# AI4Science-WestlakeU/wdno

Hardware: AMD Instinct MI355X
Metric: diffusion train steps/sec, 2D smoke U-Net (8 samples per GPU per step) (higher is better)
Workload: dtype f32

## Files before the change

### include/wdno_hip.h

```cpp
#ifndef WDNO_HIP_H
#define WDNO_HIP_H
#include <stdint.h>
#include <stddef.h>

#ifdef __cplusplus
extern "C" {
#endif

typedef void* wdno_stream_t;

enum { WDNO_OK = 0, WDNO_EINVAL = -1, WDNO_ELAUNCH = -2, WDNO_EUNSUPPORTED = -3, WDNO_EWORKSPACE = -4 };

#define WDNO_AMAX_SLOTS 64
#define WDNO_AMAX_STRIDE 16
#define WDNO_AMAX_FLOATS (WDNO_AMAX_SLOTS * WDNO_AMAX_STRIDE)
const char* wdno_strerror(int code);
int wdno_version(void);
const char* wdno_last_hip_error(void);
int wdno_set_debug(int mode);

typedef struct {
  int nd;
  int mode;
  int L;
  int n_img;
  int in_dims[3];
  int out_dims[3];
  int64_t cs_img, cs_band, cs0, cs1;
} wdno_dwt_desc;
size_t wdno_dwt_ws_bytes(const wdno_dwt_desc* d);
int wdno_dwt_fwd(const float* x, float* coef, const wdno_dwt_desc* d, const float* filters_host, void* ws, size_t ws_bytes, wdno_stream_t s);
int wdno_dwt_inv(const float* coef, float* x, const wdno_dwt_desc* d, const float* filters_host, void* ws, size_t ws_bytes, wdno_stream_t s);
int wdno_dwt_fwd_adjoint(const float* dcoef, float* dx, const wdno_dwt_desc* d, const float* filters_host, void* ws, size_t ws_bytes, wdno_stream_t s);
int wdno_dwt_inv_adjoint(const float* dx, float* dcoef, const wdno_dwt_desc* d, const float* filters_host, void* ws, size_t ws_bytes, wdno_stream_t s);
int wdno_dwt_fwd_packed(const float* x, float* state, const wdno_dwt_desc* d, const float* filters_host, int img_inner, int64_t cs_outer, int row_w,
                        const float* rescaler, wdno_stream_t s);
int wdno_upsample_coef(const float* in, float* out, int64_t outer, int a, int mid, int b, int c, int fa, int fb, int fc, wdno_stream_t s);
int wdno_pack_smoke_state(const float* coef, int64_t coef_sim_stride, const float* init_coef, int64_t init_sim_stride, const float* smokeout,
                          int64_t so_sim_stride, const int64_t* idx, const float* rescaler, float* state, int64_t B, int F, int nt, int nx,
                          int pad_t, int pad_x, wdno_stream_t s);
int wdno_pack_smoke_fields(const float* coef, int64_t coef_sim_stride, const float* rho0, int64_t rho0_sim_stride, const float* curve,
                           int64_t curve_sim_stride, const float* dec_lo_host, const float* dec_hi_host, int L, const float* rescaler,
                           float* state, int64_t B, int F, int nt, int nx, int pad_t, int pad_x, int H0, int W0, int T0, wdno_stream_t s);

int wdno_nc_to_cl(const float* src, float* dst, int64_t N, int C, int64_t S, int Cp, wdno_stream_t s);
int wdno_cl_to_nc(const float* src, float* dst, int64_t N, int C, int64_t S, int Cp, wdno_stream_t s);
int wdno_concat2_cl_planes(const float* a, int Ca, const float* b, int Cb, const float* rec_a, const float* rec_b, void* hi, void* lo,
                           float* scale_out, int64_t P, wdno_stream_t s);
int wdno_concat2_cl(const float* a, int Ca, const float* b, int Cb, float* out, int64_t P, wdno_stream_t s);
int wdno_concat2_cl_amax(const float* a, int Ca, const float* b, int Cb, float* out, float* amax_rec, int64_t P, wdno_stream_t s);
int wdno_split2_cl(const float* in, float* a, int Ca, float* b, int Cb, int64_t P, wdno_stream_t s);
int wdno_upsample2x_cl_fwd(const float* in, float* out, int64_t N, int H, int W, int C, wdno_stream_t s);
int wdno_upsample2x_cl_bwd(const float* dout, float* din, int64_t N, int H, int W, int C, wdno_stream_t s);

typedef struct {
  int N, D, H, W, C;
  int OD, OH, OW, K;
  int kd, kh, kw;
  int sd, sh, sw;
  int pd, ph, pw;
  int YD, YH, YW;
  int osd, osh, osw, ood, ooh, oow;
} wdno_conv_geom;
int wdno_conv_fwd(const float* x, const float* wp, const float* bias, const float* residual, float* y,
                  const wdno_conv_geom* g, wdno_stream_t s);
int wdno_amax(const float* x, int64_t n, float* amax_zeroed, wdno_stream_t s);
int wdno_amax_record(const float* x, int64_t n, float* rec_zeroed, wdno_stream_t s);
int wdno_split_f16(const float* x, const float* amax_rec, void* hi, void* lo, float* scale_out, int64_t rows, int C, int C8, wdno_stream_t s);
size_t wdno_split_colsum_ws_bytes(int64_t rows, int C8);
int wdno_split_f16_colsum(const float* x, const float* amax_rec, void* hi, void* lo, float* scale_out, float* colsum_out,
                          void* ws, size_t ws_bytes, int64_t rows, int C, int C8, wdno_stream_t s);
int wdno_pack_split_weight(const float* w, const float* amax, void* hi, void* lo, float* scale_out, int K, int C, int kd, int kh, int kw,
                           int A, int B, int mode, wdno_stream_t s);
typedef struct { const void* x; int64_t n; void* out; } wdno_amax_item;
typedef struct {
  const void* w; const void* amax; void* hi; void* lo; void* scale_out;
  int K, C, kd, kh, kw, A, B, mode;
} wdno_wsplit_item;
int wdno_amax_multi(const void* table, int n_items, int blocks_per_item, wdno_stream_t s);
int wdno_pack_split_weight_multi(const void* table, int n_items, int blocks_per_item, wdno_stream_t s);
int wdno_conv_fwd_f16x3(const void* xh, const void* xl, const float* sx, const void* wph, const void* wpl, const float* sw,
                        const float* bias, const float* residual, float* y, const wdno_conv_geom* g, wdno_stream_t s);
int wdno_conv_fwd_f16x3_amax(const void* xh, const void* xl, const float* sx, const void* wph, const void* wpl, const float* sw,
                             const float* bias, const float* residual, float* y, float* amax_rec, const wdno_conv_geom* g,
                             wdno_stream_t s);
typedef struct { int channels, d0, h0, w0; } wdno_zero_box;
int wdno_conv_fwd_f16x3_zbox(const void* xh, const void* xl, const float* sx, const void* wph, const void* wpl, const float* sw,
                             const float* bias, const float* residual, float* y, float* amax_rec, const wdno_conv_geom* g,
                             const wdno_zero_box* zb, wdno_stream_t s);
int wdno_conv_fwd_bf16_ex(const void* x16, const void* wp16, const float* bias, const float* residual, void* y, int y_bf16, float* amax_rec,
                          const wdno_conv_geom* g, const wdno_zero_box* zb, wdno_stream_t s);
int wdno_conv_fwd_f16x3_ws(const void* xh, const void* xl, const float* sx, const void* wph, const void* wpl, const float* sw,
                           const float* bias, const float* residual, float* y, float* amax_rec, const wdno_conv_geom* g,
                           void* ws, size_t ws_bytes, wdno_stream_t s);
size_t wdno_conv_fwd_split_ws_bytes(const wdno_conv_geom* g);
size_t wdno_conv_wgrad_f16x3_ws_bytes(const wdno_conv_geom* g);
int wdno_conv_pixel_table(void* table, const wdno_conv_geom* g, wdno_stream_t s);
int wdno_conv_wgrad_f16x3(const void* xh, const void* xl, const float* sx, const void* dyh, const void* dyl, const float* sdy,
                          const void* pixel_table, float* dwp, void* ws, size_t ws_bytes, const wdno_conv_geom* g, wdno_stream_t s);
int wdno_conv_wgrad_f16x3_param(const void* xh, const void* xl, const float* sx, const void* dyh, const void* dyl, const float* sdy,
                                const void* pixel_table, float* dw, int Kn, int Cn, void* ws, size_t ws_bytes,
                                const wdno_conv_geom* g, wdno_stream_t s);
#define WDNO_WGRAD_REDUCE_MAX 40
typedef struct wdno_wgrad_reduce_item {
  const float* ws; float* dw;
  int n, splits;
  int K8, C8, kw, ntap, Kn, Cn;
  int tiled;
  int reserved;
} wdno_wgrad_reduce_item;
int wdno_conv_wgrad_partials(const void* xh, const void* xl, const float* sx, const void* dyh, const void* dyl, const float* sdy,
                             const void* pixel_table, float* dw, int Kn, int Cn, void* ws, size_t ws_bytes,
                             const wdno_conv_geom* g, wdno_wgrad_reduce_item* item, wdno_stream_t s);
int wdno_wgrad_reduce_multi(const wdno_wgrad_reduce_item* items, int n_items, wdno_stream_t s);
size_t wdno_conv_wgrad_ws_bytes(const wdno_conv_geom* g);
int wdno_conv_wgrad(const float* x, const float* dy, float* dwp, void* ws, size_t ws_bytes,
                    const wdno_conv_geom* g, wdno_stream_t s);
#define WDNO_ROWS_SUM_MAX 64
typedef struct wdno_rows_sum_item {
  const void* part; float* out;
  int rows, stride, col0, ncols;
  int is_double, reserved;
} wdno_rows_sum_item;
int wdno_rows_sum_multi(const wdno_rows_sum_item* items, int n_items, wdno_stream_t s);
size_t wdno_colsum_ws_bytes(int64_t P, int C);
int wdno_colsum(const float* in, float* out, int64_t P, int C, void* ws, size_t ws_bytes, wdno_stream_t s);

int wdno_cast_bf16(const float* x, void* out16, int64_t rows, int C, int C8, wdno_stream_t s);
int wdno_cast_bf16_colsum(const float* x, void* out16, float* colsum_out, void* ws, size_t ws_bytes, int64_t rows, int C, int C8, wdno_stream_t s);
int wdno_conv_fwd_bf16(const void* x16, const void* wp16, const float* bias, const float* residual, float* y, float* amax_rec,
                       const wdno_conv_geom* g, wdno_stream_t s);
int wdno_conv_wgrad_bf16_param(const void* x16, const void* dy16, const void* pixel_table, float* dw, int Kn, int Cn, void* ws,
                               size_t ws_bytes, const wdno_conv_geom* g, wdno_stream_t s);

size_t wdno_groupnorm_ws_bytes(int64_t N, int64_t S, int C, int G);
size_t wdno_groupnorm_stats_floats(int64_t N, int C, int G);
int wdno_groupnorm_act_fwd(const float* x, const float* gamma, const float* beta, const float* ss, float* y,
                           float* stats, int64_t N, int64_t S, int C, int G, float eps, int silu,
                           void* ws, size_t ws_bytes, wdno_stream_t s);
int wdno_groupnorm_act_fwd_amax(const float* x, const float* gamma, const float* beta, const float* ss, float* y,
                                float* stats, float* amax_rec, int64_t N, int64_t S, int C, int G, float eps, int silu,
                                void* ws, size_t ws_bytes, wdno_stream_t s);
int wdno_groupnorm_act_bwd(const float* x, const float* dy, const float* gamma, const float* beta, const float* ss,
                           const float* stats, float* dx, float* dgb_partial, float* dss,
                           int64_t N, int64_t S, int C, int G, int silu, void* ws, size_t ws_bytes, wdno_stream_t s);
int wdno_groupnorm_act_bwd_amax(const float* x, const float* dy, const float* gamma, const float* beta, const float* ss,
                                const float* stats, float* dx, float* dgb_partial, float* dss, float* amax_rec,
                                int64_t N, int64_t S, int C, int G, int silu, void* ws, size_t ws_bytes, wdno_stream_t s);
size_t wdno_groupnorm_bwd_planes_ws_bytes(int64_t N, int64_t S, int C, int G);
size_t wdno_groupnorm_fwd_planes_ws_bytes(int64_t N, int64_t S, int C, int G);
int wdno_groupnorm_act_fwd_planes(const float* x, const float* gamma, const float* beta, const float* ss, void* y_hi, void* y_lo,
                                  float* y_scale, float* stats, float* bound_rec, int64_t N, int64_t S, int C, int G, float eps, int silu,
                                  void* ws, size_t ws_bytes, wdno_stream_t s);
int wdno_groupnorm_act_add_fwd_planes(const float* x, const float* gamma, const float* beta, const float* ss, const float* residual,
                                      const float* res_rec, float* y, void* y_hi, void* y_lo, float* y_scale, float* stats,
                                      float* bound_rec, float* y_amax_rec, int64_t N, int64_t S, int C, int G, float eps, int silu,
                                      void* ws, size_t ws_bytes, wdno_stream_t s);
int wdno_groupnorm_act_bwd_planes(const float* x, const float* dy, const float* gamma, const float* beta, const float* ss,
                                  const float* stats, void* dx_hi, void* dx_lo, float* dx_scale, float* dx_colsum,
                                  float* dgb_partial, float* dgb_sum, float* dss, float* bound_rec, int64_t N, int64_t S, int C, int G, int silu,
                                  void* ws, size_t ws_bytes, wdno_stream_t s);
int wdno_groupnorm_bwd_planes_tail(int64_t N, int64_t S, int C, int G, size_t* csp_offset, int* rows);
int wdno_groupnorm_act_fwd_amax_t(const void* x, int x_bf16, const float* gamma, const float* beta, const float* ss, float* y,
                                  float* stats, float* amax_rec, int64_t N, int64_t S, int C, int G, float eps, int silu,
                                  void* ws, size_t ws_bytes, wdno_stream_t s);
int wdno_groupnorm_act_fwd_planes_t(const void* x, int x_bf16, const float* gamma, const float* beta, const float* ss, void* y_hi, void* y_lo,
                                    float* y_scale, float* stats, float* bound_rec, int64_t N, int64_t S, int C, int G, float eps,
                                    int silu, void* ws, size_t ws_bytes, wdno_stream_t s);
int wdno_groupnorm_act_add_fwd_planes_t(const void* x, int x_bf16, const float* gamma, const float* beta, const float* ss, const float* residual,
                                        const float* res_rec, float* y, void* y_hi, void* y_lo, float* y_scale, float* stats,
                                        float* bound_rec, float* y_amax_rec, int64_t N, int64_t S, int C, int G, float eps, int silu,
                                        void* ws, size_t ws_bytes, wdno_stream_t s);
int wdno_groupnorm_act_bwd_planes_t(const void* x, int x_bf16, const void* dy, int dy_bf16, const float* gamma, const float* beta, const float* ss,
                                    const float* stats, void* dx_hi, void* dx_lo, float* dx_scale, float* dx_colsum,
                                    float* dgb_partial, float* dgb_sum, float* dss, float* bound_rec, int64_t N, int64_t S, int C, int G, int silu,
                                    void* ws, size_t ws_bytes, wdno_stream_t s);
int wdno_layernorm_fwd(const float* x, const float* g, float* y, int64_t P, int C, float eps, wdno_stream_t s);
int wdno_layernorm_fwd_amax(const float* x, const float* g, float* y, float* amax_rec, int64_t P, int C, float eps, wdno_stream_t s);
int wdno_layernorm_fwd_planes(const float* x, const float* g, void* y_hi, void* y_lo, float* y_scale, int64_t P, int C, float eps,
                              wdno_stream_t s);
size_t wdno_layernorm_bwd_ws_bytes(int64_t P, int C);
int wdno_layernorm_bwd(const float* x, const float* g, const float* dy, float* dx, float* dg, int64_t P, int C,
                       float eps, void* ws, size_t ws_bytes, wdno_stream_t s);
int wdno_layernorm_bwd_add(const float* x, const float* g, const float* dy, const float* add_to, float* dx, float* dg, int64_t P, int C,
                           float eps, void* ws, size_t ws_bytes, wdno_stream_t s);
int wdno_layernorm_bwd_add_amax(const float* x, const float* g, const float* dy, const float* add_to, float* dx, float* dg, float* amax_rec,
                                int64_t P, int C, float eps, void* ws, size_t ws_bytes, wdno_stream_t s);

typedef struct {
  int n_uo, n_ui, n_tok, heads;
  int64_t so, si, st;
} wdno_attn_desc;
int wdno_attn_fwd(const float* qkv, const float* rot_cos, const float* rot_sin, const float* bias, float* out,
                  const wdno_attn_desc* d, float scale, wdno_stream_t s);
size_t wdno_attn_bwd_ws_bytes(const wdno_attn_desc* d);
int wdno_attn_bwd(const float* qkv, const float* rot_cos, const float* rot_sin, const float* bias, const float* out,
                  const float* dout, float* dqkv, float* dbias, const wdno_attn_desc* d, float scale, void* ws, size_t ws_bytes,
                  wdno_stream_t s);
int wdno_attn_fwd_amax(const float* qkv, const float* rot_cos, const float* rot_sin, const float* bias, float* out, float* amax_rec,
                       const wdno_attn_desc* d, float scale, wdno_stream_t s);
int wdno_attn_bwd_amax(const float* qkv, const float* rot_cos, const float* rot_sin, const float* bias, const float* out,
                       const float* dout, float* dqkv, float* dbias, float* amax_rec, const wdno_attn_desc* d, float scale,
                       void* ws, size_t ws_bytes, wdno_stream_t s);
int wdno_attn_bwd_planes(const float* qkv, const float* rot_cos, const float* rot_sin, const float* bias, const float* out,
                         const float* dout, void* dqkv_hi, void* dqkv_lo, float* dqkv_scale, float* dbias,
                         const float* rec_qkv, const float* rec_dout, const wdno_attn_desc* d, float scale, void* ws, size_t ws_bytes,
                         wdno_stream_t s);
int wdno_attn_fwd_planes(const float* qkv, const float* rot_cos, const float* rot_sin, const float* bias, float* out, void* out_hi,
                         void* out_lo, float* out_scale, float* amax_rec, const float* rec_qkv, const wdno_attn_desc* d, float scale,
                         wdno_stream_t s);
size_t wdno_linattn_ws_bytes(int64_t units, int heads);
int wdno_linattn_fwd(const float* qkv, float* out, float* kstats , float* ctx ,
                     int64_t units, int n_tok, int heads, float scale, wdno_stream_t s);
int wdno_linattn_bwd(const float* qkv, const float* dout, const float* kstats, const float* ctx, float* dqkv,
                     void* ws, size_t ws_bytes, int64_t units, int n_tok, int heads, float scale, wdno_stream_t s);
int wdno_linattn_fwd_amax(const float* qkv, float* out, float* kstats, float* ctx, float* amax_rec, int64_t units, int n_tok, int heads,
                          float scale, wdno_stream_t s);
int wdno_linattn_bwd_amax(const float* qkv, const float* dout, const float* kstats, const float* ctx, float* dqkv, float* amax_rec,
                          void* ws, size_t ws_bytes, int64_t units, int n_tok, int heads, float scale, wdno_stream_t s);
int wdno_linattn_bwd_planes(const float* qkv, const float* dout, const float* kstats, const float* ctx, void* dqkv_hi, void* dqkv_lo,
                            float* dqkv_scale, const float* rec_qkv, const float* rec_dout, float* rec_dctx, void* ws, size_t ws_bytes,
                            int64_t units, int n_tok, int heads, float scale, wdno_stream_t s);
int wdno_linattn_fwd_planes(const float* qkv, void* out_hi, void* out_lo, float* out_scale, float* kstats, float* ctx,
                            const float* rec_qkv, int64_t units, int n_tok, int heads, float scale, wdno_stream_t s);

int wdno_tattn_fused_takes(int C, int n_tok, int heads);
int wdno_tattn_fused_fwd(const float* x, const float* gamma, float eps, const void* wq_hi, const void* wq_lo, const float* wq_scale,
                         const void* wo_hi, const void* wo_lo, const float* wo_scale, const float* rot_cos, const float* rot_sin,
                         const float* bias, float* y, float* amax_rec, float* qkv_out, float* rec_v,
                         int64_t n_batch, int n_tok, int64_t hw, int C, int heads, float scale, wdno_stream_t s);
size_t wdno_tattn_fused_bwd_ws_bytes(void);
int wdno_tattn_fused_bwd_grads(void);
int wdno_tattn_fused_bwd(const float* x, const float* dy, const float* gamma, float eps, const void* wq_hi, const void* wq_lo,
                         const float* wq_scale, const void* wo_hi, const void* wo_lo, const float* wo_scale, const float* rot_cos,
                         const float* rot_sin, const float* bias, const float* rec_dy, const float* rec_v, float* dx, float* amax_rec,
                         float* grads, void* ws, size_t ws_bytes,
                         int64_t n_batch, int n_tok, int64_t hw, int C, int heads, float scale, wdno_stream_t s);

int wdno_lattn_fused_takes(int C, int heads, int n_tok);
size_t wdno_lattn_fused_ws_bytes(int64_t units, int n_tok);
int wdno_lattn_fused_fwd(const float* x, const float* gamma, float eps, const void* wq_hi, const void* wq_lo, const float* wq_scale,
                         const void* wo_hi, const void* wo_lo, const float* wo_scale, const float* bias_out, float* y, float* amax_rec,
                         float* ctx_out, float* kstat_out, void* ws, size_t ws_bytes, int64_t units, int n_tok, int C, int heads, float scale,
                         wdno_stream_t s);

int wdno_lattn_fused_bwd_grads(void);
size_t wdno_lattn_fused_bwd_ws_bytes(int64_t units, int n_tok);
int wdno_lattn_fused_bwd(const float* x, const float* dy, const float* gamma, float eps, const void* wq_hi, const void* wq_lo,
                         const float* wq_scale, const void* wot_hi, const void* wot_lo, const float* wot_scale, const float* ctx,
                         const float* kstat, const float* rec_dy, float* dx, float* amax_rec, float* grads, void* ws, size_t ws_bytes,
                         int64_t units, int n_tok, int C, int heads, float scale, wdno_stream_t s);

int wdno_relpos_bias_fwd(const float* w, const int64_t* bucket, float* out, int n, int heads, wdno_stream_t s);
int wdno_relpos_bias_bwd(const float* dbias, const int64_t* bucket, float* dw, int n, int heads, int num_buckets, wdno_stream_t s);

int wdno_linear_rows_fwd(const float* x, int x_stride, const float* w, int w_stride, const float* bias, float* y, int P, int C, int K,
                         int Kp, wdno_stream_t s);
int wdno_linear_rows_wgrad(const float* x, int x_stride, const float* dy, int dy_stride, float* dw, float* db, int P, int C, int K,
                           wdno_stream_t s);

typedef struct wdno_linear_item {
  const void* w;
  const void* bias;
  int K, k_start;
} wdno_linear_item;
int wdno_linear_multi_fwd(const void* table, int n_items, int F, const float* x, float* y, int P, int C, wdno_stream_t s);
int wdno_linear_multi_wgrad(const void* table, int n_items, int F, const float* x, const float* dy, float* dw, float* db, int P, int C,
                            wdno_stream_t s);
size_t wdno_linear_multi_dgrad_ws_bytes(int F, int P, int C);
int wdno_linear_multi_dgrad(const void* table, int n_items, int F, const float* dy, float* dx, int P, int C, void* ws, size_t ws_bytes,
                            wdno_stream_t s);

int wdno_act_fwd(const float* x, float* y, int64_t n, int act, wdno_stream_t s);
int wdno_act_bwd(const float* x, const float* dy, float* dx, int64_t n, int act, wdno_stream_t s);
int wdno_add(const float* a, const float* b, float* out, int64_t n, wdno_stream_t s);
int wdno_add_amax(const float* a, const float* b, float* out, float* amax_rec, int64_t n, wdno_stream_t s);
int wdno_sinusoidal_emb(const int64_t* t, const float* freqs, float* out, int B, int dim, wdno_stream_t s);

typedef struct {
  int tree;
  int B, F, C, H, W;
  int cT, cH, cW;
  int cond_pad, cond_a, cond_b, cond_c, cond_low;
  int u_rows, uT_rows;
} wdno_cond_desc;
int wdno_q_sample_cond(const float* x0, const float* noise, const int64_t* t, const float* sqrt_ac, const float* sqrt_1mac,
// ... 39 lines not shown
```

### wdno_amd/_lib.py

```python
import contextlib
import ctypes as C
import os

import torch

HERE = os.path.dirname(os.path.abspath(__file__))
LIB_PATH = os.path.join(HERE, 'libwdno_hip.so')

P = C.c_void_p
I = C.c_int
L = C.c_int64
F = C.c_float
Z = C.c_size_t


class DwtDesc(C.Structure):
    _fields_ = [('nd', I), ('mode', I), ('L', I), ('n_img', I), ('in_dims', I * 3), ('out_dims', I * 3),
                ('cs_img', L), ('cs_band', L), ('cs0', L), ('cs1', L)]


class ConvGeom(C.Structure):
    _fields_ = [(k, I) for k in ('N', 'D', 'H', 'W', 'C', 'OD', 'OH', 'OW', 'K', 'kd', 'kh', 'kw', 'sd', 'sh', 'sw',
                                 'pd', 'ph', 'pw', 'YD', 'YH', 'YW', 'osd', 'osh', 'osw', 'ood', 'ooh', 'oow')]


class AttnDesc(C.Structure):
    _fields_ = [('n_uo', I), ('n_ui', I), ('n_tok', I), ('heads', I), ('so', L), ('si', L), ('st', L)]


class CondDesc(C.Structure):
    _fields_ = [(k, I) for k in ('tree', 'B', 'F', 'C', 'H', 'W', 'cT', 'cH', 'cW', 'cond_pad', 'cond_a', 'cond_b',
                                 'cond_c', 'cond_low', 'u_rows', 'uT_rows')]


class WgradReduceItem(C.Structure):
    _fields_ = [('ws', C.c_void_p), ('dw', C.c_void_p), ('n', I), ('splits', I), ('K8', I), ('C8', I), ('kw', I), ('ntap', I), ('Kn', I), ('Cn', I),
                ('tiled', I), ('reserved', I)]


class RowsSumItem(C.Structure):
    _fields_ = [('part', C.c_void_p), ('out', C.c_void_p), ('rows', I), ('stride', I), ('col0', I), ('ncols', I), ('is_double', I), ('reserved', I)]


class BurgersDesc(C.Structure):
    _fields_ = [(k, I) for k in ('N', 's', 'nx0', 'nt_f', 'nxf', 'steps', 'record_time', 'f_time', 'num_t', 'sub_s', 'out_cols', 'waves',
                                 'points')] + [(k, F) for k in ('c', 'd', 'dm', 'dt')]


PD, PG, PA, PC = C.POINTER(DwtDesc), C.POINTER(ConvGeom), C.POINTER(AttnDesc), C.POINTER(CondDesc)
PF = C.POINTER(C.c_float)

PROTOTYPES = {
    'wdno_strerror': (C.c_char_p, [I]),
    'wdno_version': (I, []),
    'wdno_last_hip_error': (C.c_char_p, []),
    'wdno_set_debug': (I, [I]),
    'wdno_dwt_ws_bytes': (Z, [PD]),
    'wdno_dwt_fwd': (I, [P, P, PD, PF, P, Z, P]),
    'wdno_dwt_fwd_packed': (I, [P, P, PD, PF, I, L, I, P, P]),
    'wdno_dwt_inv': (I, [P, P, PD, PF, P, Z, P]),
    'wdno_dwt_fwd_adjoint': (I, [P, P, PD, PF, P, Z, P]),
    'wdno_dwt_inv_adjoint': (I, [P, P, PD, PF, P, Z, P]),
    'wdno_upsample_coef': (I, [P, P, L, I, I, I, I, I, I, I, P]),
    'wdno_pack_smoke_state': (I, [P, L, P, L, P, L, P, P, P, L, I, I, I, I, I, P]),
    'wdno_pack_smoke_fields': (I, [P, L, P, L, P, L, PF, PF, I, P, P, L, I, I, I, I, I, I, I, I, P]),
    'wdno_nc_to_cl': (I, [P, P, L, I, L, I, P]),
    'wdno_cl_to_nc': (I, [P, P, L, I, L, I, P]),
    'wdno_concat2_cl': (I, [P, I, P, I, P, L, P]),
    'wdno_concat2_cl_planes': (I, [P, I, P, I, P, P, P, P, P, L, P]),
    'wdno_concat2_cl_amax': (I, [P, I, P, I, P, P, L, P]),
    'wdno_split2_cl': (I, [P, P, I, P, I, L, P]),
    'wdno_upsample2x_cl_fwd': (I, [P, P, L, I, I, I, P]),
    'wdno_upsample2x_cl_bwd': (I, [P, P, L, I, I, I, P]),
    'wdno_conv_fwd': (I, [P, P, P, P, P, PG, P]),
    'wdno_amax': (I, [P, L, P, P]),
    'wdno_amax_record': (I, [P, L, P, P]),
    'wdno_split_f16': (I, [P, P, P, P, P, L, I, I, P]),
    'wdno_split_colsum_ws_bytes': (Z, [L, I]),
    'wdno_split_f16_colsum': (I, [P, P, P, P, P, P, P, Z, L, I, I, P]),
    'wdno_pack_split_weight': (I, [P, P, P, P, P, I, I, I, I, I, I, I, I, P]),
    'wdno_amax_multi': (I, [P, I, I, P]),
    'wdno_pack_split_weight_multi': (I, [P, I, I, P]),
    'wdno_conv_fwd_f16x3': (I, [P, P, P, P, P, P, P, P, P, PG, P]),
    'wdno_conv_fwd_f16x3_amax': (I, [P, P, P, P, P, P, P, P, P, P, PG, P]),
    'wdno_conv_fwd_f16x3_ws': (I, [P, P, P, P, P, P, P, P, P, P, PG, P, Z, P]),
    'wdno_conv_fwd_split_ws_bytes': (Z, [PG]),
    'wdno_conv_wgrad_f16x3_ws_bytes': (Z, [PG]),
    'wdno_conv_pixel_table': (I, [P, PG, P]),
    'wdno_conv_wgrad_f16x3': (I, [P, P, P, P, P, P, P, P, P, Z, PG, P]),
    'wdno_conv_wgrad_f16x3_param': (I, [P, P, P, P, P, P, P, P, I, I, P, Z, PG, P]),
    'wdno_conv_wgrad_partials': (I, [P, P, P, P, P, P, P, P, I, I, P, Z, PG, P, P]),
    'wdno_wgrad_reduce_multi': (I, [P, I, P]),
    'wdno_rows_sum_multi': (I, [P, I, P]),
    'wdno_cast_bf16': (I, [P, P, L, I, I, P]),
    'wdno_cast_bf16_colsum': (I, [P, P, P, P, Z, L, I, I, P]),
    'wdno_conv_fwd_bf16': (I, [P, P, P, P, P, P, PG, P]),
    'wdno_conv_fwd_f16x3_zbox': (I, [P, P, P, P, P, P, P, P, P, P, PG, P, P]),
    'wdno_conv_fwd_bf16_ex': (I, [P, P, P, P, P, I, P, PG, P, P]),
    'wdno_conv_wgrad_bf16_param': (I, [P, P, P, P, I, I, P, Z, PG, P]),
    'wdno_conv_wgrad_ws_bytes': (Z, [PG]),
    'wdno_conv_wgrad': (I, [P, P, P, P, Z, PG, P]),
    'wdno_colsum_ws_bytes': (Z, [L, I]),
    'wdno_colsum': (I, [P, P, L, I, P, Z, P]),
    'wdno_groupnorm_ws_bytes': (Z, [L, L, I, I]),
    'wdno_groupnorm_stats_floats': (Z, [L, I, I]),
    'wdno_groupnorm_act_fwd': (I, [P, P, P, P, P, P, L, L, I, I, F, I, P, Z, P]),
    'wdno_groupnorm_act_fwd_amax': (I, [P, P, P, P, P, P, P, L, L, I, I, F, I, P, Z, P]),
    'wdno_groupnorm_act_bwd': (I, [P, P, P, P, P, P, P, P, P, L, L, I, I, I, P, Z, P]),
    'wdno_groupnorm_act_bwd_amax': (I, [P, P, P, P, P, P, P, P, P, P, L, L, I, I, I, P, Z, P]),
    'wdno_groupnorm_bwd_planes_ws_bytes': (Z, [L, L, I, I]),
    'wdno_groupnorm_bwd_planes_tail': (I, [L, L, I, I, C.POINTER(Z), C.POINTER(I)]),
    'wdno_groupnorm_fwd_planes_ws_bytes': (Z, [L, L, I, I]),
    'wdno_groupnorm_act_fwd_planes': (I, [P, P, P, P, P, P, P, P, P, L, L, I, I, F, I, P, Z, P]),
    'wdno_groupnorm_act_add_fwd_planes': (I, [P, P, P, P, P, P, P, P, P, P, P, P, P, L, L, I, I, F, I, P, Z, P]),
    'wdno_layernorm_fwd_planes': (I, [P, P, P, P, P, L, I, F, P]),
    'wdno_groupnorm_act_bwd_planes': (I, [P, P, P, P, P, P, P, P, P, P, P, P, P, P, L, L, I, I, I, P, Z, P]),
    'wdno_groupnorm_act_fwd_amax_t': (I, [P, I, P, P, P, P, P, P, L, L, I, I, F, I, P, Z, P]),
    'wdno_groupnorm_act_fwd_planes_t': (I, [P, I, P, P, P, P, P, P, P, P, L, L, I, I, F, I, P, Z, P]),
    'wdno_groupnorm_act_add_fwd_planes_t': (I, [P, I, P, P, P, P, P, P, P, P, P, P, P, P, L, L, I, I, F, I, P, Z, P]),
    'wdno_groupnorm_act_bwd_planes_t': (I, [P, I, P, I, P, P, P, P, P, P, P, P, P, P, P, P, L, L, I, I, I, P, Z, P]),
    'wdno_layernorm_fwd': (I, [P, P, P, L, I, F, P]),
    'wdno_layernorm_fwd_amax': (I, [P, P, P, P, L, I, F, P]),
    'wdno_layernorm_bwd_ws_bytes': (Z, [L, I]),
    'wdno_layernorm_bwd': (I, [P, P, P, P, P, L, I, F, P, Z, P]),
    'wdno_layernorm_bwd_add': (I, [P, P, P, P, P, P, L, I, F, P, Z, P]),
    'wdno_layernorm_bwd_add_amax': (I, [P, P, P, P, P, P, P, L, I, F, P, Z, P]),
    'wdno_attn_fwd': (I, [P, P, P, P, P, PA, F, P]),
    'wdno_attn_bwd_ws_bytes': (Z, [PA]),
    'wdno_attn_bwd': (I, [P, P, P, P, P, P, P, P, PA, F, P, Z, P]),
    'wdno_attn_fwd_amax': (I, [P, P, P, P, P, P, PA, F, P]),
    'wdno_attn_bwd_amax': (I, [P, P, P, P, P, P, P, P, P, PA, F, P, Z, P]),
    'wdno_attn_fwd_planes': (I, [P, P, P, P, P, P, P, P, P, P, PA, F, P]),
    'wdno_linattn_fwd_planes': (I, [P, P, P, P, P, P, P, L, I, I, F, P]),
    'wdno_attn_bwd_planes': (I, [P, P, P, P, P, P, P, P, P, P, P, P, PA, F, P, Z, P]),
    'wdno_tattn_fused_takes': (I, [I, I, I]),
    'wdno_tattn_fused_fwd': (I, [P, P, F, P, P, P, P, P, P, P, P, P, P, P, P, P, L, I, L, I, I, F, P]),
    'wdno_lattn_fused_takes': (I, [I, I, I]),
    'wdno_lattn_fused_ws_bytes': (Z, [L, I]),
    'wdno_lattn_fused_fwd': (I, [P, P, F, P, P, P, P, P, P, P, P, P, P, P, P, Z, L, I, I, I, F, P]),
    'wdno_lattn_fused_bwd_grads': (I, []),
    'wdno_lattn_fused_bwd_ws_bytes': (Z, [L, I]),
    'wdno_lattn_fused_bwd': (I, [P, P, P, F, P, P, P, P, P, P, P, P, P, P, P, P, P, Z, L, I, I, I, F, P]),
    'wdno_tattn_fused_bwd_ws_bytes': (Z, []),
    'wdno_tattn_fused_bwd_grads': (I, []),
    'wdno_tattn_fused_bwd': (I, [P, P, P, F, P, P, P, P, P, P, P, P, P, P, P, P, P, P, P, Z, L, I, L, I, I, F, P]),
    'wdno_linattn_ws_bytes': (Z, [L, I]),
    'wdno_linattn_fwd': (I, [P, P, P, P, L, I, I, F, P]),
    'wdno_linattn_bwd': (I, [P, P, P, P, P, P, Z, L, I, I, F, P]),
    'wdno_linattn_fwd_amax': (I, [P, P, P, P, P, L, I, I, F, P]),
    'wdno_linattn_bwd_amax': (I, [P, P, P, P, P, P, P, Z, L, I, I, F, P]),
    'wdno_linattn_bwd_planes': (I, [P, P, P, P, P, P, P, P, P, P, P, Z, L, I, I, F, P]),
    'wdno_act_fwd': (I, [P, P, L, I, P]),
    'wdno_act_bwd': (I, [P, P, P, L, I, P]),
    'wdno_linear_rows_fwd': (I, [P, I, P, I, P, P, I, I, I, I, P]),
    'wdno_linear_rows_wgrad': (I, [P, I, P, I, P, P, I, I, I, P]),
    'wdno_linear_multi_fwd': (I, [P, I, I, P, P, I, I, P]),
    'wdno_linear_multi_wgrad': (I, [P, I, I, P, P, P, P, I, I, P]),
    'wdno_linear_multi_dgrad_ws_bytes': (Z, [I, I, I]),
    'wdno_linear_multi_dgrad': (I, [P, I, I, P, P, I, I, P, Z, P]),
    'wdno_add': (I, [P, P, P, L, P]),
    'wdno_add_amax': (I, [P, P, P, P, L, P]),
    'wdno_sinusoidal_emb': (I, [P, P, P, I, I, P]),
    'wdno_q_sample_cond': (I, [P, P, P, P, P, P, P, PC, P]),
    'wdno_apply_cond': (I, [P, P, PC, P]),
    'wdno_weighted_mse_ws_bytes': (Z, [L]),
    'wdno_weighted_mse': (I, [P, P, P, P, F, P, P, L, L, I, L, P, Z, P]),
    'wdno_weighted_mse_bwd': (I, [P, P, P, P, F, P, P, L, L, I, L, P]),
    'wdno_p_sample_update': (I, [P, P, P, P, P, P, P, P, P, P, P, L, L, I, P]),
    'wdno_ddim_update': (I, [P, P, P, P, P, P, F, F, F, P, P, L, L, P]),
    'wdno_ddim_update_dev': (I, [P, P, P, P, P, P, P, P, P, L, L, P]),
    'wdno_sumsq_ws_bytes': (Z, [L]),
    'wdno_sumsq': (I, [P, L, P, P, Z, P]),
    'wdno_adam_clip_step': (I, [P, P, P, P, L, P, F, F, F, F, F, F, I, P]),
    'wdno_ema_update': (I, [P, P, L, F, P]),
    'wdno_gather_items': (I, [P, I, I, P]),
    'wdno_relpos_bias_fwd': (I, [P, P, P, I, I, P]),
    'wdno_relpos_bias_bwd': (I, [P, P, P, I, I, I, P]),
    'wdno_burgers_solve': (I, [P, P, P, C.POINTER(BurgersDesc), P]),
}

_lib = None


def load():
    global _lib
    if _lib is not None:
        return _lib
    if not os.path.exists(LIB_PATH):
        raise RuntimeError(f'{LIB_PATH} is missing: run `python -c "import __graft_entry__ as g; g.build()"` '
                           '(there is no CPU / eager fallback for the wdno_amd hot path)')
    lib = C.CDLL(LIB_PATH)
    for name, (res, args) in PROTOTYPES.items():
        fn = getattr(lib, name)
        fn.restype = res
        fn.argtypes = args
    _lib = lib
    if os.environ.get('WDNO_DEBUG'):
        try:
            check(lib.wdno_set_debug(int(os.environ['WDNO_DEBUG'])), f"WDNO_DEBUG={os.environ['WDNO_DEBUG']}")
        except RuntimeError:
            _lib = None
            raise
    return lib


def check(code, what):
    if code != 0:
        lib = load()
        msg = lib.wdno_strerror(code).decode()
        hip = lib.wdno_last_hip_error().decode() if code == -2 else ''
        raise RuntimeError(f'{what} failed: {msg} ({code}) {hip}')


@contextlib.contextmanager
def debug_mode(mode):
    lib = load()
    check(lib.wdno_set_debug(mode), f'wdno_set_debug({mode})')
    try:
        yield
    finally:
        lib.wdno_set_debug(0)
```

### wdno_amd/csrc/conv_common.h

```cpp
#pragma once
#include "common.h"

typedef float f32x16 __attribute__((ext_vector_type(16)));

#define BK 32
#define LDS_STRIDE 36

struct ConvP {
  wdno_conv_geom g;
  int R;
  int nchunk;
  int nsteps;
  int64_t P;
  int identity_out;
  int debug;
  int tiles_n;
  int ntiles;
  int ksplit;
  float* amax_rec;
  int tsplit;
  float* split_ws;
  size_t split_ws_bytes;
  int zb_blocks, zb_d, zb_h;
  int out_bf16;
};

__device__ __forceinline__ int xcd_swizzle(int bid, int nwg) {
  int q = nwg >> 3, r = nwg & 7;
  int xcd = bid & 7, idx = bid >> 3;
  int start = xcd < r ? xcd * (q + 1) : r * (q + 1) + (xcd - r) * q;
  return start + idx;
}

__device__ __forceinline__ int64_t out_row(const wdno_conv_geom& g, int64_t p) {
  int ow = (int)(p % g.OW); int64_t t = p / g.OW;
  int oh = (int)(t % g.OH); t /= g.OH;
  int od = (int)(t % g.OD);
  int64_t n = t / g.OD;
  return ((n * g.YD + (od * g.osd + g.ood)) * g.YH + (oh * g.osh + g.ooh)) * g.YW + (ow * g.osw + g.oow);
}

static inline int check_geom(const wdno_conv_geom* g) {
  if (!g) return WDNO_EINVAL;
  if (g->N <= 0 || g->D <= 0 || g->H <= 0 || g->W <= 0 || g->C <= 0 || g->K <= 0) return WDNO_EINVAL;
  if (g->OD <= 0 || g->OH <= 0 || g->OW <= 0 || g->kd <= 0 || g->kh <= 0 || g->kw <= 0) return WDNO_EINVAL;
  if (g->sd <= 0 || g->sh <= 0 || g->sw <= 0 || g->osd <= 0 || g->osh <= 0 || g->osw <= 0) return WDNO_EINVAL;
  if ((g->C & 3) || (g->K & 3)) return WDNO_EUNSUPPORTED;
  if ((g->OD - 1) * g->osd + g->ood >= g->YD || (g->OH - 1) * g->osh + g->ooh >= g->YH || (g->OW - 1) * g->osw + g->oow >= g->YW)
    return WDNO_EINVAL;
  return WDNO_OK;
}
#include "debug_modes.h"
void wdno_wgrad_h3d_plan(const wdno_conv_geom* g, int* bm, int* bn, int* splits, int* pix_per_split, int* splitpair = nullptr);
int wdno_conv_wgrad_h3_dma(const void* xh, const void* xl, const void* dyh, const void* dyl, const float* sx, const float* sdy,
                           const void* table, float* wsf, const wdno_conv_geom* g, hipStream_t st);
int wdno_conv_fwd_h3_dma(const void* xh, const void* xl, const void* wh, const void* wl, const float* sx, const float* sw,
                         const float* bias, const float* residual, float* y, ConvP& p, hipStream_t st, int stages);
bool wdno_conv_h3t_takes(const wdno_conv_geom& g);
int wdno_conv_h3t_split(const wdno_conv_geom& g, int64_t P, int cus);
int wdno_conv_fwd_h3_tap(int shape, const void* xh, const void* xl, const void* wh, const void* wl, const float* sx, const float* sw,
                         const float* bias, const float* residual, float* y, ConvP& p, hipStream_t st);
#ifdef __HIPCC__
__device__ __forceinline__ uint4 bf16x8_from_runs(float4 va, float4 vb) {
  const uint2 A = bf16x4_pack(va), B = bf16x4_pack(vb);
  const auto sx = __builtin_amdgcn_permlane32_swap(A.x, B.x, false, false);
  const auto sy = __builtin_amdgcn_permlane32_swap(A.y, B.y, false, false);
  return make_uint4(sx[0], sy[0], sx[1], sy[1]);
}
__device__ __forceinline__ void lgkm0_barrier() {
  __builtin_amdgcn_s_waitcnt(0xc07f);
  asm volatile("s_barrier" : : : "memory");
}
#endif
static inline void fill_params(ConvP& p, const wdno_conv_geom* g) {
  p.g = *g;
  p.amax_rec = nullptr;
  p.ksplit = 1;
  p.tsplit = 1;
  p.split_ws = nullptr;
  p.split_ws_bytes = 0;
  p.zb_blocks = 0; p.zb_d = 0; p.zb_h = 0;
  p.out_bf16 = 0;
  p.debug = wdno_debug_mode;
  p.R = g->kw * g->C;
  p.nchunk = cdiv(p.R, BK);
  p.nsteps = g->kd * g->kh * p.nchunk;
  p.P = (int64_t)g->N * g->OD * g->OH * g->OW;
  p.identity_out = (g->YD == g->OD && g->YH == g->OH && g->YW == g->OW && g->osd == 1 && g->osh == 1 && g->osw == 1 &&
                    g->ood == 0 && g->ooh == 0 && g->oow == 0) ? 1 : 0;
}
```

### wdno_amd/csrc/conv_h3.hip

```cpp
#include "conv_common.h"
#include <type_traits>
#include <algorithm>

typedef _Float16 half8 __attribute__((ext_vector_type(8)));
typedef __bf16 bf16x8 __attribute__((ext_vector_type(8)));
template <bool LP>
__device__ __forceinline__ f32x16 mfma_16(half8 a, half8 b, f32x16 c) {
  if constexpr (LP) return __builtin_amdgcn_mfma_f32_32x32x16_bf16(__builtin_bit_cast(bf16x8, a), __builtin_bit_cast(bf16x8, b), c, 0, 0, 0);
  else return __builtin_amdgcn_mfma_f32_32x32x16_f16(a, b, c, 0, 0, 0);
}

#define HBK 32
#define HST 40

template <bool RECORD>
__global__ __launch_bounds__(256) void amax_kernel(const float* __restrict__ x, int64_t n, unsigned* __restrict__ out) {
  __shared__ float red[4];
  const int64_t n4 = n >> 2;
  const float4* x4 = reinterpret_cast<const float4*>(x);
  float m = 0.f;
  const int64_t stride = (int64_t)gridDim.x * 1024;
  for (int64_t k0 = (int64_t)blockIdx.x * 1024 + threadIdx.x; k0 < n4; k0 += stride) {
    float4 v[4];
#pragma unroll
// ... 703 lines not shown
  const int wave = tid >> 6, lane = tid & 63;
  const int wm = wave / WN, wn = wave - wm * WN;
  const int li = lane & 31, hh = lane >> 5;
  const int m_base = wm * (TM * 32), n_base = wn * (TN * 32);
  f32x16 acc[TM][TN];
#pragma unroll
  for (int a = 0; a < TM; ++a)
#pragma unroll
    for (int bb = 0; bb < TN; ++bb)
#pragma unroll
      for (int e = 0; e < 16; ++e) acc[a][bb][e] = 0.f;

  if (nsteps > 0) {
    put_rec(0, fetch_rec(0));
    put_rec(1, fetch_rec(1));
    put_rec(2, fetch_rec(2));
    int4v rec = fetch_rec(3);
    __syncthreads();
    load_tile(0);
    store_tile(0);
    __syncthreads();
    if (nsteps > 1) load_tile(1);
    for (int step = 0; step < nsteps; ++step) {
      const _Float16* Ah = hsm + (step & 1) * STAGE;
      const _Float16* Al = Ah + WH_BKP * SA;
      const _Float16* Bh = Ah + NPL * WH_BKP * SA;
      const _Float16* Bl = Bh + WH_BKP * SB;
      put_rec(step + 3, rec);
      rec = fetch_rec(step + 4);
#pragma unroll
      for (int ks = 0; ks < WH_BKP / 16; ++ks) {
        half8 fah[TM], fal[TM], fbh[TN], fbl[TN];
#pragma unroll
        for (int a = 0; a < TM; ++a) {
          fah[a] = tr_frag(Ah, SA, ks * 16, m_base + a * 32, lane);
          if (!LP) fal[a] = tr_frag(Al, SA, ks * 16, m_base + a * 32, lane);
        }
#pragma unroll
        for (int bb = 0; bb < TN; ++bb) {
          fbh[bb] = tr_frag(Bh, SB, ks * 16, n_base + bb * 32, lane);
          if (!LP) fbl[bb] = tr_frag(Bl, SB, ks * 16, n_base + bb * 32, lane);
        }
        if constexpr (!LP) {
#pragma unroll
          for (int a = 0; a < TM; ++a)
#pragma unroll
            for (int bb = 0; bb < TN; ++bb) acc[a][bb] = mfma_16<false>(fal[a], fbh[bb], acc[a][bb]);
#pragma unroll
          for (int a = 0; a < TM; ++a)
#pragma unroll
            for (int bb = 0; bb < TN; ++bb) acc[a][bb] = mfma_16<false>(fah[a], fbl[bb], acc[a][bb]);
        }
#pragma unroll
        for (int a = 0; a < TM; ++a)
#pragma unroll
          for (int bb = 0; bb < TN; ++bb) acc[a][bb] = mfma_16<LP>(fah[a], fbh[bb], acc[a][bb]);
      }
      if (step + 1 < nsteps) store_tile((step + 1) & 1);
      __syncthreads();
      if (step + 2 < nsteps) load_tile(step + 2);
    }
  }

  const float inv = LP ? 1.0f : 1.0f / (sx[0] * sdy[0]);
  float* out = ws + ((int64_t)split * (g.kd * g.kh) + tap) * (int64_t)g.K * p.R;
#pragma unroll
  for (int a = 0; a < TM; ++a)
#pragma unroll
    for (int e = 0; e < 16; ++e) {
      int kk = k0 + m_base + a * 32 + (e & 3) + 8 * (e >> 2) + 4 * hh;
      if (kk >= g.K) continue;
#pragma unroll
      for (int bb = 0; bb < TN; ++bb) {
        int rr = r0 + n_base + bb * 32 + li;
        if (rr < p.R) out[(int64_t)kk * p.R + rr] = acc[a][bb][e] * inv;
      }
    }
}

__global__ __launch_bounds__(256) void wgrad_h3_reduce_kernel(const float* __restrict__ ws, float* __restrict__ out, int64_t n, int splits) {
  const int64_t n4 = n >> 2;
  const int64_t stride = (int64_t)gridDim.x * 256;
  for (int64_t i = (int64_t)blockIdx.x * 256 + threadIdx.x; i < n4; i += stride) {
    float4 a[4];
#pragma unroll
    for (int u = 0; u < 4; ++u) a[u] = make_float4(0.f, 0.f, 0.f, 0.f);
    int s = 0;
    for (; s + 3 < splits; s += 4) {
#pragma unroll
      for (int u = 0; u < 4; ++u) {
        const float4 v = *reinterpret_cast<const float4*>(ws + (int64_t)(s + u) * n + 4 * i);
        a[u].x += v.x; a[u].y += v.y; a[u].z += v.z; a[u].w += v.w;
      }
    }
    for (; s < splits; ++s) {
      const float4 v = *reinterpret_cast<const float4*>(ws + (int64_t)s * n + 4 * i);
      a[0].x += v.x; a[0].y += v.y; a[0].z += v.z; a[0].w += v.w;
    }
    *reinterpret_cast<float4*>(out + 4 * i) = make_float4((a[0].x + a[1].x) + (a[2].x + a[3].x), (a[0].y + a[1].y) + (a[2].y + a[3].y),
                                                          (a[0].z + a[1].z) + (a[2].z + a[3].z), (a[0].w + a[1].w) + (a[2].w + a[3].w));
  }
  if (blockIdx.x == 0)
    for (int64_t i = (n4 << 2) + threadIdx.x; i < n; i += 256) {
      float acc = 0.f;
      for (int s = 0; s < splits; ++s) acc += ws[(int64_t)s * n + i];
      out[i] = acc;
    }
}

static void wgrad_h3_plan(WgradHP& w, const wdno_conv_geom* g) {
  fill_params(w.c, g);
  w.xcd_group = wdno_debug_mode != WDNO_DBG_WGRAD_NO_XCD_GROUPING;
  const int BM = g->K > 64 ? 128 : 64;
  w.tiles_k = cdiv(g->K, BM);
  w.bn = (g->K > 64 || (w.c.R % 128 != 0 && w.c.R % 192 == 0)) ? 192 : 128;
  w.tiles_r = cdiv(w.c.R, w.bn);
  int64_t tiles = (int64_t)w.tiles_k * w.tiles_r * g->kd * g->kh;
  int64_t want = 512 / tiles;
  if (want < 1) want = 1;
  int64_t max_splits = cdiv64(w.c.P, 16 * WH_BKP);
  if (want > max_splits) want = max_splits;
  if (want < 1) want = 1;
  if (want > 4096) want = 4096;
  int64_t pps = cdiv64(cdiv64(w.c.P, want), WH_BKP) * WH_BKP;
  w.pix_per_split = pps;
  w.splits = (int)cdiv64(w.c.P, pps);
}
extern "C" size_t wdno_conv_wgrad_f16x3_ws_bytes(const wdno_conv_geom* g) {
  if (check_geom(g) != WDNO_OK) return 0;
  WgradHP w;
  wgrad_h3_plan(w, g);
  int bm, bn, splits, pps, sp_mode;
  wdno_wgrad_h3d_plan(g, &bm, &bn, &splits, &pps, &sp_mode);
  if (splits > w.splits) w.splits = splits;
  return (size_t)w.splits * g->kd * g->kh * (size_t)g->K * w.c.R * sizeof(float);
}
template <int BM, int BN, int WM, int WN, bool LP>
static void launch_wgrad_h3(const void* xh, const void* xl, const void* dyh, const void* dyl, const float* sx, const float* sdy,
                            const void* table, float* wsf, const WgradHP& w, dim3 grid, hipStream_t st) {
  const wdno_conv_geom& g = w.c.g;
  const unsigned x_bytes = (unsigned)((int64_t)g.N * g.D * g.H * g.W * g.C * 2);
  const unsigned dy_bytes = (unsigned)((int64_t)g.N * g.YD * g.YH * g.YW * g.K * 2);
  size_t lds = (size_t)2 * (LP ? 1 : 2) * WH_BKP * (BM + WH_PAD + BN + WH_PAD) * sizeof(_Float16) + WH_RING * WH_BKP * sizeof(int4v);
  static bool attr_done = false;
  if (!attr_done) {
    (void)hipFuncSetAttribute((const void*)conv_wgrad_h3_kernel<BM, BN, WM, WN, LP>, hipFuncAttributeMaxDynamicSharedMemorySize, (int)lds);
    attr_done = true;
  }
  conv_wgrad_h3_kernel<BM, BN, WM, WN, LP><<<grid, 256, lds, st>>>((const _Float16*)xh, (const _Float16*)xl, (const _Float16*)dyh,
                                                            (const _Float16*)dyl, sx, sdy, (const int4v*)table, wsf, w, x_bytes, dy_bytes);
}
static int wgrad_h3_partials(const void* xh, const void* xl, const float* sx, const void* dyh, const void* dyl, const float* sdy,
                             const void* pixel_table, float* single, void* ws, size_t ws_bytes, const wdno_conv_geom* g, hipStream_t st,
                             int* splits_out) {
  int rc = check_geom(g);
  if (rc) return rc;
  if ((g->C & 7) || (g->K & 7) || !pixel_table) return WDNO_EUNSUPPORTED;
  if ((int64_t)g->N * g->D * g->H * g->W * g->C * 2 >= OOB_OFFSET || (int64_t)g->N * g->YD * g->YH * g->YW * g->K * 2 >= OOB_OFFSET)
    return WDNO_EUNSUPPORTED;
  WgradHP w;
  wgrad_h3_plan(w, g);
  if (wdno_debug_mode != WDNO_DBG_ROW_ATTN_AND_REG_STAGED_CONV) {
    int bm, bn, splits, pps, sp_mode;
    wdno_wgrad_h3d_plan(g, &bm, &bn, &splits, &pps, &sp_mode);
    size_t need_d = (size_t)splits * g->kd * g->kh * (size_t)g->K * w.c.R * sizeof(float);
    float* dst = (splits == 1 && single) ? single : (float*)ws;
    if (dst == (float*)ws && ws_bytes < need_d) return WDNO_EWORKSPACE;
    rc = wdno_conv_wgrad_h3_dma(xh, xl, dyh, dyl, sx, sdy, pixel_table, dst, g, st);
    if (rc == WDNO_OK) { *splits_out = splits; return WDNO_OK; }
    if (rc != WDNO_EUNSUPPORTED) return rc;
  }
  size_t need = (size_t)w.splits * g->kd * g->kh * (size_t)g->K * w.c.R * sizeof(float);
  float* wsf = (w.splits == 1 && single) ? single : (float*)ws;
  if (wsf == (float*)ws && ws_bytes < need) return WDNO_EWORKSPACE;
  if (w.splits > 65535) return WDNO_EUNSUPPORTED;
  dim3 grid((unsigned)(w.tiles_k * g->kd * g->kh * w.tiles_r), (unsigned)w.splits);
  if (xl == nullptr) {
    if (g->K > 64) launch_wgrad_h3<128, 192, 2, 2, true>(xh, xh, dyh, dyh, sx, sdy, pixel_table, wsf, w, grid, st);
    else if (w.bn == 192) launch_wgrad_h3<64, 192, 2, 2, true>(xh, xh, dyh, dyh, sx, sdy, pixel_table, wsf, w, grid, st);
    else launch_wgrad_h3<64, 128, 1, 4, true>(xh, xh, dyh, dyh, sx, sdy, pixel_table, wsf, w, grid, st);
  } else if (g->K > 64) launch_wgrad_h3<128, 192, 2, 2, false>(xh, xl, dyh, dyl, sx, sdy, pixel_table, wsf, w, grid, st);
  else if (w.bn == 192) launch_wgrad_h3<64, 192, 2, 2, false>(xh, xl, dyh, dyl, sx, sdy, pixel_table, wsf, w, grid, st);
  else launch_wgrad_h3<64, 128, 1, 4, false>(xh, xl, dyh, dyl, sx, sdy, pixel_table, wsf, w, grid, st);
  *splits_out = w.splits;
  return WDNO_OK;
}
extern "C" int wdno_conv_wgrad_f16x3(const void* xh, const void* xl, const float* sx, const void* dyh, const void* dyl, const float* sdy,
                                     const void* pixel_table, float* dwp, void* ws, size_t ws_bytes, const wdno_conv_geom* g, wdno_stream_t s) {
  hipStream_t st = as_stream(s);
  int splits = 0;
  int rc = wgrad_h3_partials(xh, xl, sx, dyh, dyl, sdy, pixel_table, dwp, ws, ws_bytes, g, st, &splits);
  if (rc) return rc;
  if (splits > 1) {
    int64_t n = (int64_t)g->kd * g->kh * g->K * (int64_t)g->kw * g->C;
    wgrad_h3_reduce_kernel<<<stream_grid(n / 4 + 1, 256), 256, 0, st>>>((const float*)ws, dwp, n, splits);
  }
  return wdno_check_launch();
}
__device__ __forceinline__ void wgrad_h3_reduce_nat_body(const float* __restrict__ ws, float* __restrict__ dw, int64_t n, int splits,
                                                         int K8, int C8, int kw, int ntap, int Kn, int Cn, float4 (*part)[33], int bid, int nb) {
  const int R = kw * C8;
  const int j = threadIdx.x & 31, q = threadIdx.x >> 5;
  const int64_t n4 = n >> 2;
  for (int64_t i4 = (int64_t)bid * 32 + j; i4 - j < n4; i4 += (int64_t)nb * 32) {
    float4 a = make_float4(0.f, 0.f, 0.f, 0.f), b = a;
    if (i4 < n4) {
      const float4* src = reinterpret_cast<const float4*>(ws) + i4;
      int sidx = q;
      for (; sidx + 8 < splits; sidx += 16) {
        const float4 u = src[(int64_t)sidx * n4], v = src[(int64_t)(sidx + 8) * n4];
        a.x += u.x; a.y += u.y; a.z += u.z; a.w += u.w;
        b.x += v.x; b.y += v.y; b.z += v.z; b.w += v.w;
      }
      if (sidx < splits) {
        const float4 u = src[(int64_t)sidx * n4];
        a.x += u.x; a.y += u.y; a.z += u.z; a.w += u.w;
      }
    }
    part[q][j] = make_float4(a.x + b.x, a.y + b.y, a.z + b.z, a.w + b.w);
    __syncthreads();
    if (q < 4 && i4 < n4) {
      float t = 0.f;
#pragma unroll
      for (int g = 0; g < 8; ++g) {
        const float4 v = part[g][j];
        t += q == 0 ? v.x : q == 1 ? v.y : q == 2 ? v.z : v.w;
      }
      const int64_t i = i4 * 4 + q;
      const int r = (int)(i % R);
      int64_t tt = i / R;
      const int k = (int)(tt % K8);
      const int tap = (int)(tt / K8);
      const int dx = r / C8, c = r - dx * C8;
      if (k < Kn && c < Cn) dw[(((int64_t)k * Cn + c) * ntap + tap) * kw + dx] = t;
    }
    __syncthreads();
  }
}
__global__ __launch_bounds__(256) void wgrad_h3_reduce_nat_kernel(const float* __restrict__ ws, float* __restrict__ dw, int64_t n, int splits,
                                                                   int K8, int C8, int kw, int ntap, int Kn, int Cn) {
  __shared__ float4 part[8][33];
  wgrad_h3_reduce_nat_body(ws, dw, n, splits, K8, C8, kw, ntap, Kn, Cn, part, (int)blockIdx.x, (int)gridDim.x);
}
__device__ __forceinline__ void wgrad_h3_reduce_tile_body(const float* __restrict__ ws, float* __restrict__ dw, int64_t n, int splits,
                                                          int K8, int C8, int kw, int ntap, int Kn, int Cn, float (*tile)[65], int bx, int by) {
  const int T = ntap * kw, R = kw * C8;
  const int k = by, c0 = bx * 64;
  const int wave = threadIdx.x >> 6, lane = threadIdx.x & 63;
  for (int sgm = wave; sgm < T; sgm += 4) {
    const int t = sgm / kw, dx = sgm - t * kw;
    float a = 0.f, b = 0.f;
    if (c0 + lane < C8) {
      const float* src = ws + ((int64_t)t * K8 + k) * R + dx * C8 + c0 + lane;
      int sp = 0;
      for (; sp + 1 < splits; sp += 2) { a += src[(int64_t)sp * n]; b += src[(int64_t)(sp + 1) * n]; }
      if (sp < splits) a += src[(int64_t)sp * n];
    }
    tile[lane][sgm] = a + b;
  }
  __syncthreads();
  const int cn = min(64, Cn - c0);
  float* out = dw + ((int64_t)k * Cn + c0) * T;
  for (int e = threadIdx.x; e < cn * T; e += 256) {
    const int c = e / T, sgm = e - c * T;
    out[e] = tile[c][sgm];
  }
}
__global__ __launch_bounds__(256) void wgrad_h3_reduce_tile_kernel(const float* __restrict__ ws, float* __restrict__ dw, int64_t n, int splits,
                                                                    int K8, int C8, int kw, int ntap, int Kn, int Cn) {
  __shared__ float tile[64][65];
  wgrad_h3_reduce_tile_body(ws, dw, n, splits, K8, C8, kw, ntap, Kn, Cn, tile, (int)blockIdx.x, (int)blockIdx.y);
}
static bool wgrad_h3_reduce_tiled(int splits, const wdno_conv_geom* g, int Kn, int Cn) {
  const int T = g->kd * g->kh * g->kw;
  const bool big = (int64_t)Kn * cdiv(Cn, 64) >= 512 && splits <= 8;
  return T <= 64 && (splits <= 2 || big);
}

struct WgradReduceArgs {
  wdno_wgrad_reduce_item it[WDNO_WGRAD_REDUCE_MAX];
  int first[WDNO_WGRAD_REDUCE_MAX + 1];
  int n;
};
__global__ __launch_bounds__(256) void wgrad_h3_reduce_multi_kernel(const WgradReduceArgs a) {
  __shared__ __attribute__((aligned(16))) float smem[64 * 65];
  int lo = 0, hi = a.n - 1;
  while (lo < hi) {
    const int mid = (lo + hi + 1) >> 1;
    if (a.first[mid] <= (int)blockIdx.x) lo = mid; else hi = mid - 1;
  }
  const wdno_wgrad_reduce_item& w = a.it[lo];
  const int bid = (int)blockIdx.x - a.first[lo], nb = a.first[lo + 1] - a.first[lo];
  if (w.tiled) {
    const int bxn = (w.Cn + 63) >> 6;
    wgrad_h3_reduce_tile_body(w.ws, w.dw, w.n, w.splits, w.K8, w.C8, w.kw, w.ntap, w.Kn, w.Cn, reinterpret_cast<float (*)[65]>(smem), bid % bxn, bid / bxn);
  } else {
    wgrad_h3_reduce_nat_body(w.ws, w.dw, w.n, w.splits, w.K8, w.C8, w.kw, w.ntap, w.Kn, w.Cn, reinterpret_cast<float4 (*)[33]>(smem), bid, nb);
  }
}
extern "C" int wdno_wgrad_reduce_multi(const wdno_wgrad_reduce_item* items, int n_items, wdno_stream_t s) {
  WDNO_REQUIRE(items && n_items >= 0);
  hipStream_t st = as_stream(s);
  for (int base = 0; base < n_items; base += WDNO_WGRAD_REDUCE_MAX) {
    WgradReduceArgs a;
    a.n = n_items - base < WDNO_WGRAD_REDUCE_MAX ? n_items - base : WDNO_WGRAD_REDUCE_MAX;
    int grid = 0;
    for (int i = 0; i < a.n; ++i) {
      a.it[i] = items[base + i];
      const wdno_wgrad_reduce_item& w = a.it[i];
      WDNO_REQUIRE(w.ws && w.dw && w.n > 0 && w.splits >= 1 && w.Kn > 0 && w.Cn > 0 && w.Kn <= w.K8 && w.Cn <= w.C8);
      a.first[i] = grid;
      grid += w.tiled ? cdiv(w.Cn, 64) * w.Kn : stream_grid(w.n / 4, 32);
    }
    a.first[a.n] = grid;
    if (grid > 0) wgrad_h3_reduce_multi_kernel<<<grid, 256, 0, st>>>(a);
  }
  return wdno_check_launch();
}

static void wgrad_h3_reduce_launch(const float* ws, float* dw, int64_t n, int splits, const wdno_conv_geom* g, int Kn, int Cn, hipStream_t st) {
  if (wgrad_h3_reduce_tiled(splits, g, Kn, Cn)) {
    wgrad_h3_reduce_tile_kernel<<<dim3(cdiv(Cn, 64), Kn), 256, 0, st>>>(ws, dw, n, splits, g->K, g->C, g->kw, g->kd * g->kh, Kn, Cn);
    return;
  }
  wgrad_h3_reduce_nat_kernel<<<stream_grid(n / 4, 32), 256, 0, st>>>(ws, dw, n, splits, g->K, g->C, g->kw, g->kd * g->kh, Kn, Cn);
}
extern "C" int wdno_conv_wgrad_f16x3_param(const void* xh, const void* xl, const float* sx, const void* dyh, const void* dyl, const float* sdy,
                                           const void* pixel_table, float* dw, int Kn, int Cn, void* ws, size_t ws_bytes,
                                           const wdno_conv_geom* g, wdno_stream_t s) {
  WDNO_REQUIRE(g && Kn > 0 && Cn > 0 && Kn <= g->K && Cn <= g->C);
  hipStream_t st = as_stream(s);
  int splits = 0;
  int rc = wgrad_h3_partials(xh, xl, sx, dyh, dyl, sdy, pixel_table, nullptr, ws, ws_bytes, g, st, &splits);
  if (rc) return rc;
  const int64_t n = (int64_t)g->kd * g->kh * g->K * (int64_t)g->kw * g->C;
  wgrad_h3_reduce_launch((const float*)ws, dw, n, splits, g, Kn, Cn, st);
  return wdno_check_launch();
}

extern "C" int wdno_conv_wgrad_partials(const void* xh, const void* xl, const float* sx, const void* dyh, const void* dyl, const float* sdy,
                                        const void* pixel_table, float* dw, int Kn, int Cn, void* ws, size_t ws_bytes,
                                        const wdno_conv_geom* g, wdno_wgrad_reduce_item* item, wdno_stream_t s) {
  WDNO_REQUIRE(g && item && dw && Kn > 0 && Cn > 0 && Kn <= g->K && Cn <= g->C);
  int splits = 0;
  int rc = wgrad_h3_partials(xh, xl, sx, dyh, dyl, sdy, pixel_table, nullptr, ws, ws_bytes, g, as_stream(s), &splits);
  if (rc) return rc;
  const int64_t n = (int64_t)g->kd * g->kh * g->K * (int64_t)g->kw * g->C;
  if (n >= 0x7fffffff) return WDNO_EUNSUPPORTED;
  item->ws = (const float*)ws; item->dw = dw; item->n = (int)n; item->splits = splits; item->K8 = g->K; item->C8 = g->C; item->kw = g->kw;
  item->ntap = g->kd * g->kh; item->Kn = Kn; item->Cn = Cn; item->tiled = wgrad_h3_reduce_tiled(splits, g, Kn, Cn) ? 1 : 0;
  return wdno_check_launch();
}

extern "C" int wdno_conv_wgrad_bf16_param(const void* x16, const void* dy16, const void* pixel_table, float* dw, int Kn, int Cn, void* ws,
                                          size_t ws_bytes, const wdno_conv_geom* g, wdno_stream_t s) {
  WDNO_REQUIRE(g && Kn > 0 && Cn > 0 && Kn <= g->K && Cn <= g->C);
  hipStream_t st = as_stream(s);
  int splits = 0;
  int rc = wgrad_h3_partials(x16, nullptr, nullptr, dy16, nullptr, nullptr, pixel_table, nullptr, ws, ws_bytes, g, st, &splits);
  if (rc) return rc;
  const int64_t n = (int64_t)g->kd * g->kh * g->K * (int64_t)g->kw * g->C;
  wgrad_h3_reduce_launch((const float*)ws, dw, n, splits, g, Kn, Cn, st);
  return wdno_check_launch();
}

#define PS_LDS_FLOATS 10240
struct PackTile { int KT, CT, CTp, tiles_k, tiles_c; };
__host__ __device__ static inline PackTile pack_tile(int T, int A, int B, int mode) {
  PackTile t;
  auto need = [&](int longd, int shortd) { return (int64_t)T * (mode ? (int64_t)longd * (shortd + 1) : (int64_t)shortd * (longd + 1)); };
  int longd = 128, shortd = 8;
  while (longd > 8 && need(longd, shortd) > PS_LDS_FLOATS) longd >>= 1;
  while (shortd > 1 && need(longd, shortd) > PS_LDS_FLOATS) shortd >>= 1;
  t.KT = mode ? longd : shortd;
  t.CT = mode ? shortd : longd;
  t.CTp = t.CT + 1;
  const int kext = mode ? B : A, cext = mode ? A : B;
  t.tiles_k = (kext + t.KT - 1) / t.KT;
  t.tiles_c = (cext + t.CT - 1) / t.CT;
  return t;
}
__device__ __forceinline__ unsigned ps_magic(unsigned d) { return d > 1 ? (unsigned)((1ull << 32) / d) + 1u : 0u; }
__device__ __forceinline__ int ps_div(int n, int d, unsigned m) { return d == 1 ? n : (int)__umulhi((unsigned)n, m); }
__device__ __forceinline__ void pack_split_body(const float* __restrict__ w, const float* __restrict__ amax,
                                                _Float16* __restrict__ hi, _Float16* __restrict__ lo,
                                                float* __restrict__ scale_out, int K, int C, int kd, int kh, int kw,
                                                int A, int B, int mode_in, int block, int nblocks) {
  __shared__ float tile[PS_LDS_FLOATS + 16];
  const int frag = mode_in >= 10 ? mode_in - 9 : 0;
  const int parity = mode_in >= 2 && mode_in < 6 ? mode_in - 2 : -1;
  const int patch = mode_in >= 6 && mode_in < 10 ? mode_in - 6 : -1;
  const int mode = mode_in == 1 || patch >= 0 ? 1 : 0;
  const bool lp = lo == nullptr;
  const float s = lp ? 1.0f : scale_from_amax(amax[0]);
  if (!lp && block == 0 && threadIdx.x == 0) scale_out[0] = s;
  const int b8 = B >> 3;
  const int T = kd * kh * kw, khw = kh * kw;
  const PackTile pt = pack_tile(T, A, B, mode);
  if ((int64_t)T * pt.KT * pt.CTp > PS_LDS_FLOATS + 16) return;
  const int ntiles = pt.tiles_k * pt.tiles_c;
  const int run = pt.CT * T;
  const int bt8 = (mode ? pt.KT : pt.CT) >> 3;
  const int at = mode ? pt.CT : pt.KT;
  const unsigned m_run = ps_magic(run), m_T = ps_magic(T), m_bt8 = ps_magic(bt8), m_at = ps_magic(at), m_khw = ps_magic(khw), m_kw = ps_magic(kw);
  for (int tl = block; tl < ntiles; tl += nblocks) {
    const int tk = ps_div(tl, pt.tiles_c, ps_magic(pt.tiles_c)), tc = tl - tk * pt.tiles_c;
    const int k0 = tk * pt.KT, c0 = tc * pt.CT;
    __syncthreads();
    const int cvalid = min(pt.CT, C - c0);
    const int nload = pt.KT * run;
    for (int idx0 = threadIdx.x; idx0 < nload; idx0 += 256 * 8) {
      float v[8];
      int dst[8];
#pragma unroll
      for (int u = 0; u < 8; ++u) {
        const int idx = min(idx0 + 256 * u, nload - 1);
        const int kk = ps_div(idx, run, m_run), r = idx - kk * run;
        const int cl = ps_div(r, T, m_T), tap = r - cl * T;
        const bool ok = k0 + kk < K && cl < cvalid;
        const int64_t off = !ok ? 0 : patch >= 0 ? (((int64_t)(k0 + kk) * C + c0 + cl) * 4 + patch) : parity < 0 ? ((int64_t)(k0 + kk) * C + c0) * T + r
                            : ((int64_t)(c0 + cl) * K + (k0 + kk)) * 16 + (3 - (parity >> 1) - 2 * (tap >> 1)) * 4 + (3 - (parity & 1) - 2 * (tap & 1));
        v[u] = w[off];
        if (!ok) v[u] = 0.f;
        dst[u] = idx0 + 256 * u < nload ? (tap * pt.KT + kk) * pt.CTp + cl : -1;
      }
#pragma unroll
      for (int u = 0; u < 8; ++u)
        if (dst[u] >= 0) tile[dst[u]] = v[u];
    }
    __syncthreads();
    const int nitems = T * at * bt8;
    for (int idx = threadIdx.x; idx < nitems; idx += 256) {
      int q = ps_div(idx, bt8, m_bt8);
      const int g = idx - q * bt8;
      const int tap = ps_div(q, at, m_at), al = q - tap * at;
      const int dz = ps_div(tap, khw, m_khw), rr = tap - dz * khw;
      const int dy = ps_div(rr, kw, m_kw), dx = rr - dy * kw;
      const int ts = mode ? T - 1 - tap : tap;
      const int a = (mode ? c0 : k0) + al;
      const int bg = ((mode ? k0 : c0) >> 3) + g;
      if (a >= A || bg >= b8) continue;
      const float* src = mode ? tile + (ts * pt.KT + g * 8) * pt.CTp + al : tile + (ts * pt.KT + al) * pt.CTp + g * 8;
      const int step = mode ? pt.CTp : 1;
      half8 h, l;
      typedef unsigned short us8 __attribute__((ext_vector_type(8)));
      us8 bq;
#pragma unroll
      for (int e = 0; e < 8; ++e) {
        const float v = src[e * step];
        const float tv = v * s;
        const _Float16 th = (_Float16)tv;
        h[e] = th;
        l[e] = (_Float16)(tv - (float)th);
        bq[e] = bf16_rne(v);
      }
      int64_t i = ((((int64_t)dz * kh + dy) * A + a) * kw + dx) * b8 + bg;
      if (frag) {
        const int li = a & 31, t = bg >> 2, hh2 = (bg >> 1) & 1, s2 = bg & 1;
        if (frag == 1) { const int ti = a >> 7, hd = (a >> 5) & 3; i = ((((hd * 3 + ti) * (B >> 5) + t) * 2 + s2) * 64 + hh2 * 32 + li); }
        else { const int q4 = A >> 2, wv = a / q4, mt = (a - wv * q4) >> 5; i = ((((wv * (A >> 7) + mt) * 4 + t) * 2 + s2) * 64 + hh2 * 32 + li); }
      }
      if (lp) { *reinterpret_cast<us8*>(hi + i * 8) = bq; continue; }
      *reinterpret_cast<half8*>(hi + i * 8) = h;
      *reinterpret_cast<half8*>(lo + i * 8) = l;
    }
  }
}
__global__ __launch_bounds__(256) void pack_split_weight_kernel(const float* __restrict__ w, const float* __restrict__ amax,
                                                                 _Float16* __restrict__ hi, _Float16* __restrict__ lo,
                                                                 float* __restrict__ scale_out, int K, int C, int kd, int kh, int kw,
                                                                 int A, int B, int mode) {
  pack_split_body(w, amax, hi, lo, scale_out, K, C, kd, kh, kw, A, B, mode, (int)blockIdx.x, (int)gridDim.x);
}
__global__ __launch_bounds__(256) void amax_multi_kernel(const wdno_amax_item* __restrict__ tab) {
  __shared__ float red[4];
  const wdno_amax_item it = tab[blockIdx.y];
  const float* x = (const float*)it.x;
  const int64_t n = it.n;
  float m = 0.f;
  int64_t head = (int64_t)(((16 - (reinterpret_cast<uintptr_t>(x) & 15)) & 15) >> 2);
  if (head > n) head = n;
  const int64_t n4 = (n - head) >> 2, tail0 = head + 4 * n4;
  if (blockIdx.x == 0) {
    if ((int64_t)threadIdx.x < head) m = fabsf(x[threadIdx.x]);
    if (tail0 + (int64_t)threadIdx.x < n) m = fmaxf(m, fabsf(x[tail0 + threadIdx.x]));
  }
  const float4* x4 = reinterpret_cast<const float4*>(x + head);
  const int64_t stride = (int64_t)gridDim.x * 256;
  int64_t k = (int64_t)blockIdx.x * 256 + threadIdx.x;
  for (; k + 3 * stride < n4; k += 4 * stride) {
    const float4 a = x4[k], b = x4[k + stride], c = x4[k + 2 * stride], d = x4[k + 3 * stride];
    m = amax4(amax4(m, a), b);
    m = amax4(amax4(m, c), d);
  }
  for (; k < n4; k += stride) m = amax4(m, x4[k]);
  m = wave_max(m);
  if ((threadIdx.x & 63) == 0) red[threadIdx.x >> 6] = m;
  __syncthreads();
  if (threadIdx.x == 0) {
    m = fmaxf(fmaxf(red[0], red[1]), fmaxf(red[2], red[3]));
    if (m > 0.f) atomicMax((unsigned*)it.out, __float_as_uint(m));
  }
}
extern "C" int wdno_amax_multi(const void* table, int n_items, int blocks_per_item, wdno_stream_t s) {
  WDNO_REQUIRE(table && n_items > 0 && n_items <= 65535 && blocks_per_item > 0);
  amax_multi_kernel<<<dim3((unsigned)blocks_per_item, (unsigned)n_items), 256, 0, as_stream(s)>>>((const wdno_amax_item*)table);
  return wdno_check_launch();
}
__global__ __launch_bounds__(256) void pack_split_weight_multi_kernel(const wdno_wsplit_item* __restrict__ tab) {
  const wdno_wsplit_item it = tab[blockIdx.y];
  pack_split_body((const float*)it.w, (const float*)it.amax, (_Float16*)it.hi, (_Float16*)it.lo, (float*)it.scale_out, it.K, it.C, it.kd, it.kh,
                  it.kw, it.A, it.B, it.mode, (int)blockIdx.x, (int)gridDim.x);
}
extern "C" int wdno_pack_split_weight_multi(const void* table, int n_items, int blocks_per_item, wdno_stream_t s) {
  WDNO_REQUIRE(table && n_items > 0 && n_items <= 65535 && blocks_per_item > 0);
  pack_split_weight_multi_kernel<<<dim3((unsigned)blocks_per_item, (unsigned)n_items), 256, 0, as_stream(s)>>>((const wdno_wsplit_item*)table);
// ... 20 lines not shown
```

### wdno_amd/csrc/conv_wgrad_h3d.hip

```cpp
#include "conv_common.h"
#include <type_traits>

typedef _Float16 half8 __attribute__((ext_vector_type(8)));
typedef __bf16 bf16x8 __attribute__((ext_vector_type(8)));
typedef int int4v __attribute__((ext_vector_type(4)));
#define WD_OOB 0x7ffffff0
template <bool LP>
__device__ __forceinline__ f32x16 mfma_16(half8 a, half8 b, f32x16 c) {
  if constexpr (LP) return __builtin_amdgcn_mfma_f32_32x32x16_bf16(__builtin_bit_cast(bf16x8, a), __builtin_bit_cast(bf16x8, b), c, 0, 0, 0);
  else return __builtin_amdgcn_mfma_f32_32x32x16_f16(a, b, c, 0, 0, 0);
}

struct WgradDP {
  ConvP c;
  int tiles_k, tiles_r, splits, nsteps;
  int items;
  int pix_per_split;
  int xcd_chunk;
  int splitpair, n_a;
};

__device__ __forceinline__ int4v wd_rsrc(const void* ptr, unsigned bytes) {
  uint64_t a = reinterpret_cast<uint64_t>(ptr);
  int4v r;
  r.x = __builtin_amdgcn_readfirstlane((int)(unsigned)a);
  r.y = __builtin_amdgcn_readfirstlane((int)(unsigned)((a >> 32) & 0xffffu));
  r.z = __builtin_amdgcn_readfirstlane((int)bytes);
  r.w = 0x00020000;
  return r;
}
__device__ __forceinline__ void wd_piece(int4v rsrc, int off, unsigned lds_dst) {
  asm volatile("s_mov_b32 m0, %1\n\ts_nop 0\n\tbuffer_load_dwordx4 %0, %2, 0 offen lds" : : "v"(off), "s"(lds_dst), "s"(rsrc) : "memory");
}
__device__ __forceinline__ int4v wd_load_rec(int4v rsrc, int off) {
  int4v v;
  asm volatile("buffer_load_dwordx4 %0, %1, %2, 0 offen" : "=v"(v) : "v"(off), "s"(rsrc) : "memory");
  return v;
}
template <int NCH>
__device__ __forceinline__ half8 wd_frag(const char* plane, int lane_off, int pix0, int ch0) {
  typedef short short4v __attribute__((ext_vector_type(4)));
  typedef short4v __attribute__((address_space(3))) * lds_s4;
  const char* p0 = plane + lane_off + (pix0 / 4) * (NCH * 64) + (ch0 / 32) * 256;
  short4v a = __builtin_amdgcn_ds_read_tr16_b64_v4i16((lds_s4)(p0));
  short4v b = __builtin_amdgcn_ds_read_tr16_b64_v4i16((lds_s4)(p0 + NCH * 64));
  typedef short short8v __attribute__((ext_vector_type(8)));
  short8v c = __builtin_shufflevector(a, b, 0, 1, 2, 3, 4, 5, 6, 7);
  return __builtin_bit_cast(half8, c);
}

template <int BM, int BN, int NS, bool LP>
__global__ __launch_bounds__(512) void conv_wgrad_h3d_kernel(const _Float16* __restrict__ xh, const _Float16* __restrict__ xl,
                                                              const _Float16* __restrict__ dyh, const _Float16* __restrict__ dyl,
                                                              const float* __restrict__ sx, const float* __restrict__ sdy,
                                                              const int4v* __restrict__ table, float* __restrict__ ws, WgradDP wp,
                                                              unsigned x_bytes, unsigned dy_bytes, unsigned tbl_bytes) {
  constexpr int TM = BM / 64, TN = BN / 64;
  constexpr int ACH = BM / 8, BCH = BN / 8;
  constexpr int A_PLANE = 32 * ACH * 16, B_PLANE = 32 * BCH * 16;
  constexpr int NPL = LP ? 1 : 2;
  constexpr int A_LO = A_PLANE, B_HI = NPL * A_PLANE, B_LO = B_HI + B_PLANE;
  constexpr int STAGE = NPL * (A_PLANE + B_PLANE);
  constexpr int APC = A_PLANE / 1024, BPC = B_PLANE / 1024;
  constexpr int NPAIR = APC + BPC;
  static_assert(NPAIR % 4 == 0, "pieces are dealt to four producer waves");
  constexpr int R = NPAIR / 4;
  constexpr int PW = NPL * R;
  constexpr int LA = 2;
  static_assert(R + (NS - 2) * (R + PW) <= 63, "vmcnt is a 6-bit counter");
  extern __shared__ __attribute__((aligned(1024))) char smem[];
  const ConvP& p = wp.c;
  const wdno_conv_geom& g = p.g;
  const int tid = threadIdx.x;
  const int wave = __builtin_amdgcn_readfirstlane(tid >> 6), lane = tid & 63;
  int it_first, it_stride, my_items;
  if (wp.xcd_chunk > 0) {
    const int xcd = (int)blockIdx.x & 7, idx = (int)blockIdx.x >> 3;
    const int beg = xcd * wp.xcd_chunk, end = min(beg + wp.xcd_chunk, wp.items);
    it_stride = (int)gridDim.x >> 3;
    it_first = beg + idx;
    my_items = it_first < end ? (end - it_first + it_stride - 1) / it_stride : 0;
  } else {
    it_first = (int)blockIdx.x; it_stride = (int)gridDim.x;
    my_items = (wp.items - it_first + it_stride - 1) / it_stride;
  }
  const int ntap = g.kd * g.kh;
  auto decode_item = [&](int t, int& tile_k, int& tap, int& tile_r, int& split) {
    int id = it_first + t * it_stride;
    tile_r = id % wp.tiles_r; id /= wp.tiles_r;
    tap = id % ntap; id /= ntap;
    tile_k = id % wp.tiles_k;
    split = id / wp.tiles_k;
  };

  if (wave >= 4) {
    const int pq = wave - 4;
    int4v rxh = wd_rsrc(xh, x_bytes), rxl = wd_rsrc(xl, x_bytes), rdh = wd_rsrc(dyh, dy_bytes), rdl = wd_rsrc(dyl, dy_bytes);
    int4v rtb = wd_rsrc(table, tbl_bytes);
    asm volatile("s_nop 4" : "+s"(rxh), "+s"(rxl), "+s"(rdh), "+s"(rdl), "+s"(rtb));
    const unsigned lds0 = __builtin_amdgcn_readfirstlane((unsigned)(size_t)(__attribute__((address_space(3))) char*)smem);
    int row[R], chk[R];
#pragma unroll
    for (int j = 0; j < R; ++j) {
      const int gp = pq + 4 * j;
      const bool isA = gp < APC;
      const int f = 64 * (isA ? gp : gp - APC) + lane;
      const int nch = isA ? ACH : BCH;
      const int nu = nch / 4;
      row[j] = 4 * (f / (16 * nu)) + ((f >> 2) & 3);
      chk[j] = (((f >> 4) % nu) * 4 + (f & 3)) * 8;
    }
    struct Cur { int t, s; };
    Cur rc{0, 0}, pc{0, 0};
    int r_pbeg = 0;
    int c_dz = 0, c_dy = 0, c_tapoff = 0;
    int i_off[R], i_dx[R];
    bool i_ok[R];
    auto load_item_r = [&]() {
      int tk, tap, tr, sp;
      decode_item(rc.t, tk, tap, tr, sp);
      r_pbeg = sp * wp.pix_per_split;
    };
    auto load_item_p = [&]() {
      int tk, tap, tr, sp;
      decode_item(pc.t, tk, tap, tr, sp);
      c_dz = tap / g.kh; c_dy = tap - c_dz * g.kh;
      c_tapoff = (c_dz * g.H + c_dy) * g.W * g.C;
#pragma unroll
      for (int j = 0; j < R; ++j) {
        if (pq + 4 * j < APC) {
          const int k = tk * BM + chk[j];
          i_ok[j] = k < g.K;
          i_off[j] = k * 2;
          i_dx[j] = 0;
        } else {
          const int r = tr * BN + chk[j];
          i_ok[j] = r < p.R;
          i_off[j] = r;
          i_dx[j] = r / g.C;
        }
      }
    };
    if (my_items > 0) { load_item_r(); load_item_p(); }
    int4v rec[LA + 1][R];
    bool rok[LA + 1][R];
    auto fetch = [&](auto SLOT) {
      constexpr int S = decltype(SLOT)::value;
      const bool live = rc.t < my_items;
#pragma unroll
      for (int j = 0; j < R; ++j) {
        const int pm = r_pbeg + rc.s * 32 + row[j];
        rok[S][j] = live && pm < (int)p.P;
        rec[S][j] = wd_load_rec(rtb, rok[S][j] ? pm * 16 : WD_OOB);
      }
// ... 390 lines not shown

  const int wslot = wave >> 1, whalf = wave & 1;
  const int li = lane & 31;
  const int gq = lane >> 4, xq = lane & 15;
  const int offA = (2 * (gq >> 1)) * (ACH * 64) + (xq >> 2) * 64 + (gq & 1) * 32 + (xq & 3) * 8 + (kind_b ? wslot * A_PLANE : 0);
  const int chan = (gq & 1) * 32 + (xq & 3) * 8;
  const int pix_l = 8 * (gq >> 1) + (xq >> 2);
  typedef short short4v __attribute__((ext_vector_type(4)));
  typedef short short8v __attribute__((ext_vector_type(8)));
  typedef short4v __attribute__((address_space(3))) * lds_s4;
  auto x_addr = [&](int wrow, int unit) { return (wrow >> 2) * (XCH * 64) + unit * 256 + (wrow & 3) * 64 + chan; };
  const float inv = LP ? 1.0f : 1.0f / (sx[0] * sdy[0]);
  const int hh = lane >> 5;
  const int step_ow = 32 % g.W;
  const int wbase = B_HI + wslot * W_PLANE;

  auto run = [&](auto HC) {
    constexpr int HV = decltype(HC)::value;
    constexpr int DX[3] = {(3 * HV) >> 1, (3 * HV + 1) >> 1, (3 * HV + 2) >> 1};
    constexpr int UH[3] = {(3 * HV) & 1, (3 * HV + 1) & 1, (3 * HV + 2) & 1};
    int base[TN][4], rd[TN][4], ow[4];
#pragma unroll
    for (int c = 0; c < 4; ++c)
#pragma unroll
      for (int b = 0; b < TN; ++b) base[b][c] = x_addr(16 * (c >> 1) + 4 * (c & 1) + pix_l + DX[b], UH[b]);
    auto select = [&](int c) {
#pragma unroll
      for (int b = 0; b < TN; ++b) {
        if (DX[b] == 1) rd[b][c] = base[b][c];
        else rd[b][c] = (unsigned)(ow[c] - g.pw + DX[b]) < (unsigned)g.W ? base[b][c] : (base[b][c] & (XCH * 64 - 1)) + ZROWS;
      }
    };
    auto advance = [&](int c) {
      ow[c] += step_ow;
      if (ow[c] >= g.W) ow[c] -= g.W;
    };
    half8 fah[2][TM], fal[2][TM], fbh[2][TN], fbl[2][TN];
    auto read_frags = [&](auto SET, int stage, int ks) {
      constexpr int B = decltype(SET)::value;
      const char* st = smem + stage * STAGE;
#pragma unroll
      for (int a = 0; a < TM; ++a) {
        fah[B][a] = wd_frag<ACH>(st, offA, ks * 16, a * 32);
        if (!LP) fal[B][a] = wd_frag<ACH>(st + A_LO, offA, ks * 16, a * 32);
      }
#pragma unroll
      for (int b = 0; b < TN; ++b) {
        const short4v h0 = __builtin_amdgcn_ds_read_tr16_b64_v4i16((lds_s4)(st + wbase + rd[b][2 * ks]));
        const short4v h1 = __builtin_amdgcn_ds_read_tr16_b64_v4i16((lds_s4)(st + wbase + rd[b][2 * ks + 1]));
        fbh[B][b] = __builtin_bit_cast(half8, (short8v)__builtin_shufflevector(h0, h1, 0, 1, 2, 3, 4, 5, 6, 7));
        if (!LP) {
          const short4v l0 = __builtin_amdgcn_ds_read_tr16_b64_v4i16((lds_s4)(st + wbase + B_PLANE + rd[b][2 * ks]));
          const short4v l1 = __builtin_amdgcn_ds_read_tr16_b64_v4i16((lds_s4)(st + wbase + B_PLANE + rd[b][2 * ks + 1]));
          fbl[B][b] = __builtin_bit_cast(half8, (short8v)__builtin_shufflevector(l0, l1, 0, 1, 2, 3, 4, 5, 6, 7));
        }
      }
    };
    f32x16 acc[TM][TN];
    auto mfma_set = [&](auto SET) {
      constexpr int B = decltype(SET)::value;
      if constexpr (!LP) {
#pragma unroll
        for (int a = 0; a < TM; ++a)
#pragma unroll
          for (int b = 0; b < TN; ++b) acc[a][b] = mfma_16<false>(fbh[B][b], fal[B][a], acc[a][b]);
#pragma unroll
        for (int a = 0; a < TM; ++a)
#pragma unroll
          for (int b = 0; b < TN; ++b) acc[a][b] = mfma_16<false>(fbl[B][b], fah[B][a], acc[a][b]);
      }
#pragma unroll
      for (int a = 0; a < TM; ++a)
#pragma unroll
        for (int b = 0; b < TN; ++b) acc[a][b] = mfma_16<LP>(fbh[B][b], fah[B][a], acc[a][b]);
    };
    constexpr int NRD = NPL * 2 * (TM + TN), NMF = (LP ? 1 : 3) * TM * TN, RPM = (NRD + NMF - 1) / NMF;
    auto interleave = [&]() {
#pragma unroll
      for (int i = 0; i < NMF; ++i) {
        __builtin_amdgcn_sched_group_barrier(0x008, 1, 0);
        if (i * RPM < NRD) __builtin_amdgcn_sched_group_barrier(0x100, RPM, 0);
      }
    };
    using B0 = std::integral_constant<int, 0>;
    using B1 = std::integral_constant<int, 1>;
    int stage = 0;
    for (int t = 0; t < my_items; ++t) {
      int tile_k, tile_c, tps[2], sps[2];
      decode_item(t, tile_k, tile_c, tps, sps);
      const int tap = wslot ? tps[1] : tps[0], split = wslot ? sps[1] : sps[0];
      const int pbeg = split * wp.pix_per_split;
#pragma unroll
      for (int c = 0; c < 4; ++c) ow[c] = (pbeg + 16 * (c >> 1) + 4 * (c & 1) + pix_l) % g.OW;
#pragma unroll
      for (int a = 0; a < TM; ++a)
#pragma unroll
        for (int b = 0; b < TN; ++b)
#pragma unroll
          for (int e = 0; e < 16; ++e) acc[a][b][e] = 0.f;
      select(0); select(1);
      lgkm0_barrier();
      read_frags(B0{}, stage, 0);
      advance(0); advance(1);
      for (int step = 0; step + 1 < wp.nsteps; ++step) {
        select(2); select(3);
        read_frags(B1{}, stage, 1);
        advance(2); advance(3);
        mfma_set(B0{});
        interleave();
        __builtin_amdgcn_sched_barrier(0);
        stage = stage + 1 == NS ? 0 : stage + 1;
        select(0); select(1);
        lgkm0_barrier();
        read_frags(B0{}, stage, 0);
        advance(0); advance(1);
        mfma_set(B1{});
        interleave();
        __builtin_amdgcn_sched_barrier(0);
      }
      select(2); select(3);
      read_frags(B1{}, stage, 1);
      mfma_set(B0{});
      interleave();
      __builtin_amdgcn_sched_barrier(0);
      stage = stage + 1 == NS ? 0 : stage + 1;
      mfma_set(B1{});
      __builtin_amdgcn_sched_barrier(0);
      if (tap < ntap && split < wp.splits) {
        float* out = ws + ((int64_t)split * ntap + tap) * (int64_t)g.K * p.R;
#pragma unroll
        for (int a = 0; a < TM; ++a) {
          const int kk = tile_k * BM + a * 32 + li;
          if (kk >= g.K) continue;
          float* orow = out + (int64_t)kk * p.R;
#pragma unroll
          for (int b = 0; b < TN; ++b) {
#pragma unroll
            for (int e4 = 0; e4 < 4; ++e4) {
              const int rr = DX[b] * g.C + tile_c * CT + UH[b] * 32 + 8 * e4 + 4 * hh;
              *reinterpret_cast<float4*>(orow + rr) = make_float4(acc[a][b][4 * e4] * inv, acc[a][b][4 * e4 + 1] * inv, acc[a][b][4 * e4 + 2] * inv, acc[a][b][4 * e4 + 3] * inv);
            }
          }
        }
      }
    }
  };
  if (whalf == 0) run(std::integral_constant<int, 0>{});
  else run(std::integral_constant<int, 1>{});
}

#ifndef WDNO_H3S_STAGES
#define WDNO_H3S_STAGES 4
#endif
template <bool LP>
__global__ __launch_bounds__(512) void conv_wgrad_h3s_kernel(const _Float16* __restrict__ xh, const _Float16* __restrict__ xl,
                                                              const _Float16* __restrict__ dyh, const _Float16* __restrict__ dyl,
                                                              const float* __restrict__ sx, const float* __restrict__ sdy,
                                                              float* __restrict__ ws, WgradDP wp, unsigned x_bytes, unsigned dy_bytes) {
  constexpr int KW = 7, CX = 48, NS = WDNO_H3S_STAGES, TM = 2;
  constexpr int ROWB = CX * 2, XROWS = 32 + KW - 1, X_DATA = XROWS * ROWB;
  constexpr int A_PLANE = 4096, X_PLANE = 4096, ZADDR = X_DATA;
  constexpr int NPL = LP ? 1 : 2;
  constexpr int A_LO = A_PLANE, B_HI = NPL * A_PLANE, B_LO = B_HI + X_PLANE;
  constexpr int STAGE = NPL * (A_PLANE + X_PLANE);
  constexpr int PER = 2 * NPL;
  extern __shared__ __attribute__((aligned(1024))) char smem[];
  const ConvP& p = wp.c;
  const wdno_conv_geom& g = p.g;
  const int tid = threadIdx.x;
  const int wave = __builtin_amdgcn_readfirstlane(tid >> 6), lane = tid & 63;
  int it_first, it_stride, my_items;
  if (wp.xcd_chunk > 0) {
    const int xcd = (int)blockIdx.x & 7, idx = (int)blockIdx.x >> 3;
    const int beg = xcd * wp.xcd_chunk, end = min(beg + wp.xcd_chunk, wp.items);
    it_stride = (int)gridDim.x >> 3;
    it_first = beg + idx;
    my_items = it_first < end ? (end - it_first + it_stride - 1) / it_stride : 0;
  } else {
    it_first = (int)blockIdx.x; it_stride = (int)gridDim.x;
    my_items = (wp.items - it_first + it_stride - 1) / it_stride;
  }
  const int ntap = g.kd * g.kh;
  const int total = my_items * wp.nsteps;

  if (wave >= 4) {
    const int pq = wave - 4;
    int4v rxh = wd_rsrc(xh, x_bytes), rxl = wd_rsrc(xl, x_bytes), rdh = wd_rsrc(dyh, dy_bytes), rdl = wd_rsrc(dyl, dy_bytes);
    asm volatile("s_nop 4" : "+s"(rxh), "+s"(rxl), "+s"(rdh), "+s"(rdl));
    const unsigned lds0 = __builtin_amdgcn_readfirstlane((unsigned)(size_t)(__attribute__((address_space(3))) char*)smem);
    const int f = 64 * pq + lane;
    const int xr = f / (ROWB / 16), xc = f - xr * (ROWB / 16);
    const bool x_slot = xr < XROWS;
    const int gi = f >> 5, du = (f >> 4) & 1, dj = (f >> 2) & 3, dc = f & 3;
    const int dpix = 16 * (gi >> 2) + 8 * ((gi >> 1) & 1) + (gi & 1) + 2 * dj;
    const bool d_slot = du * 32 + dc * 8 < g.K;
    int it = 0, st = 0;
    int q = 0, qw = 0, qh = 0, qd = 0, x_off = 0, dp = 0, d_off = 0, vdz = 0, vdy = 0;
    auto setup_item = [&]() {
      const int id = it_first + it * it_stride;
      const int tap = id % ntap, split = id / ntap;
      const int dz = tap / g.kh, dy = tap - dz * g.kh;
      vdz = dz - g.pd; vdy = dy - g.ph;
      const int pbeg = split * wp.pix_per_split;
      q = pbeg + xr - g.pw;
      const int whd = g.W * g.H * g.D;
      int qq = q + whd;
      qw = qq % g.W; qq /= g.W;
      qh = qq % g.H; qq /= g.H;
      qd = qq % g.D;
      x_off = ((q + (vdz * g.H + vdy) * g.W) * g.C + xc * 8) * 2;
      dp = pbeg + dpix;
      d_off = (dp * g.K + du * 32 + dc * 8) * 2;
    };
    const bool no_dma = p.debug == WDNO_DBG_NO_DMA;
    auto issue_next = [&](int buf) {
      const unsigned sb = lds0 + buf * STAGE + pq * 1024;
      const bool xv = x_slot && q >= 0 && q < (int)p.P && (unsigned)(qd + vdz) < (unsigned)g.D && (unsigned)(qh + vdy) < (unsigned)g.H;
      const int xo = xv && !no_dma ? x_off : WD_OOB;
      const int d_o = d_slot && dp < (int)p.P && !no_dma ? d_off : WD_OOB;
      wd_piece(rdh, d_o, sb);
      if (!LP) wd_piece(rdl, d_o, sb + A_LO);
      wd_piece(rxh, xo, sb + B_HI);
      if (!LP) wd_piece(rxl, xo, sb + B_LO);
      q += 32; x_off += 32 * g.C * 2; dp += 32; d_off += 32 * g.K * 2;
      qw += 32;
      while (qw >= g.W) { qw -= g.W; if (++qh == g.H) { qh = 0; if (++qd == g.D) qd = 0; } }
      if (++st == wp.nsteps) { st = 0; if (++it < my_items) setup_item(); }
    };
    if (total > 0) setup_item();
    int nbuf = 0;
    for (int a = 0; a < NS - 1 && a < total; ++a) { issue_next(nbuf); nbuf = nbuf + 1 == NS ? 0 : nbuf + 1; }
    for (int gs = 0; gs < total; ++gs) {
      if (gs + NS - 2 < total) asm volatile("s_waitcnt vmcnt(%0)\n\ts_barrier" : : "n"((NS - 2) * PER) : "memory");
      else asm volatile("s_waitcnt vmcnt(0)\n\ts_barrier" : : : "memory");
      if (gs + NS - 1 < total) { issue_next(nbuf); nbuf = nbuf + 1 == NS ? 0 : nbuf + 1; }
    }
    asm volatile("s_waitcnt vmcnt(0)" : : : "memory");
    return;
  }

  const int li = lane & 31, hh = lane >> 5, g1 = (lane >> 4) & 1, xq = lane & 15;
  const int fj = xq >> 2, c4 = xq & 3;
  typedef short short4v __attribute__((ext_vector_type(4)));
  typedef short short8v __attribute__((ext_vector_type(8)));
  typedef short4v __attribute__((address_space(3))) * lds_s4;
  const float inv = LP ? 1.0f : 1.0f / (sx[0] * sdy[0]);
  const int step_ow = 32 % g.W;
  const int a_base = hh * 1024 + fj * 64 + g1 * 32 + c4 * 8;

  auto run = [&](auto TNC) {
    constexpr int TN = decltype(TNC)::value;
    const int tb0 = 3 * wave;
    int xbase[TN][4], rd[TN][4], dlo[TN], ow[4];
#pragma unroll
    for (int b = 0; b < TN; ++b) {
      const int r = 32 * (tb0 + b) + 16 * g1 + 4 * c4;
      const int dx = r / CX;
      dlo[b] = dx < KW ? g.pw - dx : (1 << 20);
#pragma unroll
      for (int c = 0; c < 4; ++c) xbase[b][c] = (16 * (c >> 1) + 8 * hh + (c & 1) + 2 * fj) * ROWB + 2 * r;
    }
    auto select = [&](int c) {
#pragma unroll
      for (int b = 0; b < TN; ++b) rd[b][c] = (unsigned)(ow[c] - dlo[b]) < (unsigned)g.W ? xbase[b][c] : 3840 + (xbase[b][c] & 255);
    };
    auto advance = [&](int c) {
      ow[c] += step_ow;
      if (ow[c] >= g.W) ow[c] -= g.W;
    };
    half8 fah[2][TM], fal[2][TM], fbh[2][TN], fbl[2][TN];
    auto tr2 = [&](const char* a0, const char* a1) {
      const short4v h0 = __builtin_amdgcn_ds_read_tr16_b64_v4i16((lds_s4)a0);
      const short4v h1 = __builtin_amdgcn_ds_read_tr16_b64_v4i16((lds_s4)a1);
      return __builtin_bit_cast(half8, (short8v)__builtin_shufflevector(h0, h1, 0, 1, 2, 3, 4, 5, 6, 7));
    };
    auto read_frags = [&](auto SET, int stage, int ks) {
      constexpr int B = decltype(SET)::value;
      const char* st = smem + stage * STAGE;
#pragma unroll
      for (int a = 0; a < TM; ++a) {
        const char* pa = st + a_base + ks * 2048 + a * 256;
        fah[B][a] = tr2(pa, pa + 512);
        if (!LP) fal[B][a] = tr2(pa + A_LO, pa + A_LO + 512);
      }
#pragma unroll
      for (int b = 0; b < TN; ++b) {
        fbh[B][b] = tr2(st + B_HI + rd[b][2 * ks], st + B_HI + rd[b][2 * ks + 1]);
        if (!LP) fbl[B][b] = tr2(st + B_LO + rd[b][2 * ks], st + B_LO + rd[b][2 * ks + 1]);
      }
    };
    f32x16 acc[TM][TN];
    auto mfma_set = [&](auto SET) {
      constexpr int B = decltype(SET)::value;
      if constexpr (!LP) {
#pragma unroll
        for (int a = 0; a < TM; ++a)
#pragma unroll
          for (int b = 0; b < TN; ++b) acc[a][b] = mfma_16<false>(fbh[B][b], fal[B][a], acc[a][b]);
#pragma unroll
        for (int a = 0; a < TM; ++a)
#pragma unroll
          for (int b = 0; b < TN; ++b) acc[a][b] = mfma_16<false>(fbl[B][b], fah[B][a], acc[a][b]);
      }
#pragma unroll
      for (int a = 0; a < TM; ++a)
#pragma unroll
        for (int b = 0; b < TN; ++b) acc[a][b] = mfma_16<LP>(fbh[B][b], fah[B][a], acc[a][b]);
    };
    constexpr int NRD = NPL * 2 * (TM + TN), NMF = (LP ? 1 : 3) * TM * TN, RPM = (NRD + NMF - 1) / NMF;
    auto interleave = [&]() {
#pragma unroll
      for (int i = 0; i < NMF; ++i) {
        __builtin_amdgcn_sched_group_barrier(0x008, 1, 0);
        if (i * RPM < NRD) __builtin_amdgcn_sched_group_barrier(0x100, RPM, 0);
      }
    };
    using B0 = std::integral_constant<int, 0>;
    using B1 = std::integral_constant<int, 1>;
    int stage = 0;
    for (int t = 0; t < my_items; ++t) {
      const int id = it_first + t * it_stride;
      const int tap = id % ntap, split = id / ntap;
      const int pbeg = split * wp.pix_per_split;
#pragma unroll
      for (int c = 0; c < 4; ++c) ow[c] = (pbeg + 16 * (c >> 1) + 8 * hh + (c & 1) + 2 * fj) % g.OW;
#pragma unroll
      for (int a = 0; a < TM; ++a)
#pragma unroll
        for (int b = 0; b < TN; ++b)
#pragma unroll
          for (int e = 0; e < 16; ++e) acc[a][b][e] = 0.f;
      select(0); select(1);
      lgkm0_barrier();
      read_frags(B0{}, stage, 0);
      advance(0); advance(1);
      for (int step = 0; step + 1 < wp.nsteps; ++step) {
        select(2); select(3);
        read_frags(B1{}, stage, 1);
        advance(2); advance(3);
        mfma_set(B0{});
        interleave();
        __builtin_amdgcn_sched_barrier(0);
        stage = stage + 1 == NS ? 0 : stage + 1;
        select(0); select(1);
        lgkm0_barrier();
        read_frags(B0{}, stage, 0);
        advance(0); advance(1);
        mfma_set(B1{});
        interleave();
        __builtin_amdgcn_sched_barrier(0);
      }
      select(2); select(3);
      read_frags(B1{}, stage, 1);
      mfma_set(B0{});
      interleave();
      __builtin_amdgcn_sched_barrier(0);
      stage = stage + 1 == NS ? 0 : stage + 1;
      mfma_set(B1{});
      __builtin_amdgcn_sched_barrier(0);
      float* out = ws + ((int64_t)split * ntap + tap) * (int64_t)g.K * p.R;
#pragma unroll
      for (int a = 0; a < TM; ++a) {
        const int kk = a * 32 + li;
        if (kk >= g.K) continue;
        float* orow = out + (int64_t)kk * p.R;
#pragma unroll
        for (int b = 0; b < TN; ++b) {
#pragma unroll
          for (int e4 = 0; e4 < 4; ++e4) {
            const int rr = 32 * (tb0 + b) + 8 * e4 + 4 * hh;
            if (rr < p.R)
              *reinterpret_cast<float4*>(orow + rr) = make_float4(acc[a][b][4 * e4] * inv, acc[a][b][4 * e4 + 1] * inv, acc[a][b][4 * e4 + 2] * inv, acc[a][b][4 * e4 + 3] * inv);
          }
        }
      }
    }
  };
  if (wave < 3) run(std::integral_constant<int, 3>{});
  else run(std::integral_constant<int, 2>{});
}

static int wd_num_cus() {
  static int n = 0;
  if (!n) {
    int dev = 0;
    hipDeviceProp_t prop;
    if (hipGetDevice(&dev) != hipSuccess || hipGetDeviceProperties(&prop, dev) != hipSuccess) return 256;
    n = prop.multiProcessorCount > 0 ? prop.multiProcessorCount : 256;
  }
  return n;
}

static bool wd_window_takes(const wdno_conv_geom* g) {
  if (wdno_debug_mode == WDNO_DBG_CHUNKED_DMA_CONV || (wdno_debug_mode == WDNO_DBG_PER_AXIS_DWT_AND_WGRAD_WINDOW_K64 && g->K > 64)) return false;
  return g->sd == 1 && g->sh == 1 && g->sw == 1 && g->OD == g->D && g->OH == g->H && g->OW == g->W && g->kw == 3 && g->pw == 1 &&
         (g->C % 64) == 0 && (g->K % 8) == 0;
}
static bool wd_stem_takes(const wdno_conv_geom* g) {
  if (wdno_debug_mode == WDNO_DBG_CHUNKED_DMA_CONV) return false;
  return g->sd == 1 && g->sh == 1 && g->sw == 1 && g->OD == g->D && g->OH == g->H && g->OW == g->W && g->kw == 7 && g->pw == 3 &&
         g->C == 48 && (g->K % 8) == 0 && g->K <= 64 && g->kd <= 8 && g->kh <= 8;
}
void wdno_wgrad_h3d_plan(const wdno_conv_geom* g, int* bm, int* bn, int* splits, int* pix_per_split, int* splitpair) {
  ConvP c;
  fill_params(c, g);
  if (splitpair) *splitpair = 0;
  if (wd_stem_takes(g)) {
    *bm = 64; *bn = 352;
    int64_t want = 256 / (g->kd * g->kh);
    int64_t max_splits = cdiv64(c.P, 16 * 32);
    if (want > max_splits) want = max_splits;
    if (want < 1) want = 1;
    int64_t pps = cdiv64(cdiv64(c.P, want), 32) * 32;
    *pix_per_split = (int)pps;
    *splits = (int)cdiv64(c.P, pps);
    return;
  }
  if (wd_window_takes(g)) {
    *bm = 64; *bn = 192;
    const int ntap = g->kd * g->kh, tkc = cdiv(g->K, 64) * (g->C / 64);
    const int tiles = tkc * ((ntap + 1) / 2);
    int64_t want = 256 / tiles;
    int64_t max_splits = cdiv64(c.P, 16 * 32);
    if (want > max_splits) want = max_splits;
    if (want < 1) want = 1;
    int64_t pps = cdiv64(cdiv64(c.P, want), 32) * 32;
    *pix_per_split = (int)pps;
    *splits = (int)cdiv64(c.P, pps);
    if (splitpair) *splitpair = 0;
    if (splitpair && (ntap & 1) && wdno_debug_mode != WDNO_DBG_WGRAD_NO_SPLIT_PAIR) {
      const int blocks = wd_num_cus() >= 256 ? 256 : (wd_num_cus() & ~7);
      int64_t S = max_splits < 256 ? max_splits : 256;
      while (S >= 2 && (int64_t)tkc * (ntap / 2) * S + (int64_t)tkc * ((S + 1) / 2) > blocks) --S;
      if (S >= 2) {
        const int64_t pps2 = cdiv64(cdiv64(c.P, S), 32) * 32;
        const int64_t s2 = cdiv64(c.P, pps2);
        if (s2 >= 2 && pps2 < pps) { *pix_per_split = (int)pps2; *splits = (int)s2; *splitpair = 1; }
      }
    }
    return;
  }
  *bm = g->K > 64 ? 128 : 64;
  *bn = cdiv(c.R, 192) * 192 <= cdiv(c.R, 128) * 128 ? 192 : 128;
  const int tiles = cdiv(g->K, *bm) * cdiv(c.R, *bn) * g->kd * g->kh;
  int64_t want = 512 / tiles;
  int64_t max_splits = cdiv64(c.P, 16 * 32);
  if (want > max_splits) want = max_splits;
  if (want < 1) want = 1;
  int64_t pps = cdiv64(cdiv64(c.P, want), 32) * 32;
  *pix_per_split = (int)pps;
  *splits = (int)cdiv64(c.P, pps);
}

template <int BM, int BN, bool LP>
static void launch_wd(const void* xh, const void* xl, const void* dyh, const void* dyl, const float* sx, const float* sdy,
                      const void* table, float* wsf, const WgradDP& w, hipStream_t st) {
  const wdno_conv_geom& g = w.c.g;
  const unsigned x_bytes = (unsigned)((int64_t)g.N * g.D * g.H * g.W * g.C * 2);
  const unsigned dy_bytes = (unsigned)((int64_t)g.N * g.YD * g.YH * g.YW * g.K * 2);
  const unsigned tbl_bytes = (unsigned)(w.c.P * 16);
  constexpr int NS = 3;
  const size_t lds = (size_t)NS * (LP ? 1 : 2) * (32 * (BM / 8) * 16 + 32 * (BN / 8) * 16);
  static bool done = false;
  if (!done) { (void)hipFuncSetAttribute((const void*)conv_wgrad_h3d_kernel<BM, BN, NS, LP>, hipFuncAttributeMaxDynamicSharedMemorySize, (int)lds); done = true; }
  int grid = wd_num_cus();
  if (w.items < grid) grid = w.items;
  WgradDP wl = w;
  wl.xcd_chunk = 0;
  if (grid >= 64 && wdno_debug_mode != WDNO_DBG_WGRAD_NO_XCD_GROUPING) {
    wl.xcd_chunk = cdiv(w.items, 8);
    grid = wd_num_cus() & ~7;
    if (8 * wl.xcd_chunk < grid) grid = 8 * wl.xcd_chunk;
  }
  conv_wgrad_h3d_kernel<BM, BN, NS, LP><<<grid, 512, lds, st>>>((const _Float16*)xh, (const _Float16*)xl, (const _Float16*)dyh, (const _Float16*)dyl,
                                                         sx, sdy, (const int4v*)table, wsf, wl, x_bytes, dy_bytes, tbl_bytes);
}

template <bool LP>
static void launch_ww(const void* xh, const void* xl, const void* dyh, const void* dyl, const float* sx, const float* sdy,
                      const void* table, float* wsf, const WgradDP& w, hipStream_t st) {
  const wdno_conv_geom& g = w.c.g;
  const unsigned x_bytes = (unsigned)((int64_t)g.N * g.D * g.H * g.W * g.C * 2);
  const unsigned dy_bytes = (unsigned)((int64_t)g.N * g.YD * g.YH * g.YW * g.K * 2);
  const unsigned tbl_bytes = (unsigned)(w.c.P * 16);
  constexpr int NS = 3;
  const size_t lds = (size_t)NS * (LP ? 1 : 2) * (2 * 4096 + 2 * 5120);
  static bool done = false;
  if (!done) { (void)hipFuncSetAttribute((const void*)conv_wgrad_h3w_kernel<NS, LP>, hipFuncAttributeMaxDynamicSharedMemorySize, (int)lds); done = true; }
  int grid = wd_num_cus();
  if (w.items < grid) grid = w.items;
  WgradDP wl = w;
  wl.xcd_chunk = 0;
  if (grid >= 64 && wdno_debug_mode != WDNO_DBG_WGRAD_NO_XCD_GROUPING) {
    wl.xcd_chunk = cdiv(w.items, 8);
    grid = wd_num_cus() & ~7;
    if (8 * wl.xcd_chunk < grid) grid = 8 * wl.xcd_chunk;
  }
  conv_wgrad_h3w_kernel<NS, LP><<<grid, 512, lds, st>>>((const _Float16*)xh, (const _Float16*)xl, (const _Float16*)dyh, (const _Float16*)dyl,
                                                       sx, sdy, (const int4v*)table, wsf, wl, x_bytes, dy_bytes, tbl_bytes);
}

template <bool LP>
static void launch_ws(const void* xh, const void* xl, const void* dyh, const void* dyl, const float* sx, const float* sdy,
                      float* wsf, const WgradDP& w, hipStream_t st) {
  const wdno_conv_geom& g = w.c.g;
  const unsigned x_bytes = (unsigned)((int64_t)g.N * g.D * g.H * g.W * g.C * 2);
  const unsigned dy_bytes = (unsigned)((int64_t)g.N * g.YD * g.YH * g.YW * g.K * 2);
  const size_t lds = (size_t)WDNO_H3S_STAGES * (LP ? 1 : 2) * (4096 + 4096);
  int grid = wd_num_cus();
  if (w.items < grid) grid = w.items;
  WgradDP wl = w;
  wl.xcd_chunk = 0;
  if (grid >= 64 && wdno_debug_mode != WDNO_DBG_WGRAD_NO_XCD_GROUPING) {
    wl.xcd_chunk = cdiv(w.items, 8);
    grid = wd_num_cus() & ~7;
    if (8 * wl.xcd_chunk < grid) grid = 8 * wl.xcd_chunk;
  }
  conv_wgrad_h3s_kernel<LP><<<grid, 512, lds, st>>>((const _Float16*)xh, (const _Float16*)xl, (const _Float16*)dyh, (const _Float16*)dyl,
                                                   sx, sdy, wsf, wl, x_bytes, dy_bytes);
}

int wdno_conv_wgrad_h3_dma(const void* xh, const void* xl, const void* dyh, const void* dyl, const float* sx, const float* sdy,
                           const void* table, float* wsf, const wdno_conv_geom* g, hipStream_t st) {
  WgradDP w;
  fill_params(w.c, g);
  int bm, bn;
  wdno_wgrad_h3d_plan(g, &bm, &bn, &w.splits, &w.pix_per_split, &w.splitpair);
  w.n_a = 0x7fffffff;
  if (w.c.P * 16 >= WD_OOB) return WDNO_EUNSUPPORTED;
  w.tiles_k = cdiv(g->K, bm);
  w.tiles_r = cdiv(w.c.R, bn);
  w.nsteps = w.pix_per_split / 32;
  w.items = w.tiles_k * w.tiles_r * g->kd * g->kh * w.splits;
  if (wd_stem_takes(g)) {
    if ((int64_t)g->N * g->D * g->H * g->W * g->C * 2 >= WD_OOB || w.c.P * g->K * 2 >= WD_OOB) return WDNO_EUNSUPPORTED;
    w.tiles_k = w.tiles_r = 1;
    w.items = g->kd * g->kh * w.splits;
    if (xl == nullptr) launch_ws<true>(xh, xh, dyh, dyh, sx, sdy, wsf, w, st);
    else launch_ws<false>(xh, xl, dyh, dyl, sx, sdy, wsf, w, st);
    return WDNO_OK;
  }
  if (wd_window_takes(g)) {
    w.items = w.tiles_k * w.tiles_r * ((g->kd * g->kh + 1) / 2) * w.splits;
    if (w.splitpair) {
      w.n_a = w.tiles_k * w.tiles_r * ((g->kd * g->kh) / 2) * w.splits;
      w.items = w.n_a + w.tiles_k * w.tiles_r * ((w.splits + 1) / 2);
    }
    if (xl == nullptr) launch_ww<true>(xh, xh, dyh, dyh, sx, sdy, table, wsf, w, st);
    else launch_ww<false>(xh, xl, dyh, dyl, sx, sdy, table, wsf, w, st);
    return WDNO_OK;
  }
  if (xl == nullptr) {
    if (bm == 128 && bn == 192) launch_wd<128, 192, true>(xh, xh, dyh, dyh, sx, sdy, table, wsf, w, st);
    else if (bm == 128) launch_wd<128, 128, true>(xh, xh, dyh, dyh, sx, sdy, table, wsf, w, st);
    else if (bn == 192) launch_wd<64, 192, true>(xh, xh, dyh, dyh, sx, sdy, table, wsf, w, st);
    else launch_wd<64, 128, true>(xh, xh, dyh, dyh, sx, sdy, table, wsf, w, st);
    return WDNO_OK;
  }
  if (bm == 128 && bn == 192) launch_wd<128, 192, false>(xh, xl, dyh, dyl, sx, sdy, table, wsf, w, st);
  else if (bm == 128) launch_wd<128, 128, false>(xh, xl, dyh, dyl, sx, sdy, table, wsf, w, st);
  else if (bn == 192) launch_wd<64, 192, false>(xh, xl, dyh, dyl, sx, sdy, table, wsf, w, st);
  else launch_wd<64, 128, false>(xh, xl, dyh, dyl, sx, sdy, table, wsf, w, st);
  return WDNO_OK;
}
```

### wdno_amd/csrc/debug_modes.h

```cpp
#pragma once

#define WDNO_DEBUG_MODES(X)                                                                                                                       \
  X(WDNO_DBG_OFF, 0)                                                                                                               \
                                \
  X(WDNO_DBG_ROW_ATTN_AND_REG_STAGED_CONV, 5)                                                                                                      \
  X(WDNO_DBG_WGRAD_NO_XCD_GROUPING, 6)   \
  X(WDNO_DBG_FORCE_DMA_CONV, 7)                     \
       \
  X(WDNO_DBG_CHUNKED_DMA_CONV, 8)                                                                                                                  \
                                                                                                               \
  X(WDNO_DBG_PER_AXIS_DWT_AND_WGRAD_WINDOW_K64, 11)                                                                                                \
  X(WDNO_DBG_DWT_SKIP_W_PASS, 12)                                        \
  X(WDNO_DBG_DWT_SKIP_H_PASS, 13)                                                    \
  X(WDNO_DBG_DWT_SKIP_T_PASS, 14)                                     \
     \
  X(WDNO_DBG_NO_DMA, 21)                                                                                                                           \
  X(WDNO_DBG_WGRAD_NO_DMA_NO_PIECE, 22)                  \
            \
  X(WDNO_DBG_STAMP_CYCLES, 23)                                                         \
  X(WDNO_DBG_STAMP_EPILOGUE, 24)                                                                          \
  X(WDNO_DBG_STAMP_REALTIME, 26)                                          \
  X(WDNO_DBG_FORCE_TILES_160, 30)           \
  X(WDNO_DBG_FORCE_TILES_320, 31)                                   \
  X(WDNO_DBG_ATTN_GENERIC_NTOK, 44)      \
  X(WDNO_DBG_DWT3_SYNTH_LDS, 45)              \
  X(WDNO_DBG_CONV_NO_RUN_SPLIT, 56)      \
  X(WDNO_DBG_STEM_EVERY_STAGE, 57)                  \
  X(WDNO_DBG_ATTN_FWD_ROWS, 67)          \
  X(WDNO_DBG_ATTN_BWD_ROWS, 68)                                              \
  X(WDNO_DBG_WGRAD_NO_SPLIT_PAIR, 70)    \
  X(WDNO_DBG_STEM_TILES_256, 72)                             \
                               \
  X(WDNO_DBG_NO_DMA_STAMP_CYCLES, 123)                                                                                                             \
  X(WDNO_DBG_NO_DMA_STAMP_EPILOGUE, 124)                                                                                                           \
  X(WDNO_DBG_NO_DMA_STAMP_REALTIME, 126)

enum wdno_debug : int {
#define WDNO_DBG_ENUM(name, value) name = value,
  WDNO_DEBUG_MODES(WDNO_DBG_ENUM)
#undef WDNO_DBG_ENUM
  WDNO_DBG_NO_DMA_OFFSET = 100
};

extern int wdno_debug_mode;
```

### wdno_amd/ops.py

```python
import contextlib
import ctypes as C
import math
import os

import torch

from . import _lib
from ._lib import AttnDesc, CondDesc, ConvGeom, DwtDesc

WEIGHT_EPOCH = 0
_pack_cache = {}


PROFILE = None


class _timed:

    def __init__(self, key, flops):
        self.key, self.flops = key, flops

    def __enter__(self):
        if PROFILE is not None:
            self.e0 = torch.cuda.Event(enable_timing=True)
# ... 679 lines not shown
        key = (n, d, h, ww, cp8, kp, tuple(ks), tuple(osp)) if tap and ks[2] == 3 else None
        wsb = 0
        if key is not None:
            wsb = _split_ws_bytes.get(key)
            if wsb is None:
                wsb = _split_ws_bytes[key] = int(_lib_().wdno_conv_fwd_split_ws_bytes(C.byref(g)))
        if wsb:
            ws = torch.empty(wsb // 4, device=xh.device, dtype=torch.float32)
            _lib.check(_lib_().wdno_conv_fwd_f16x3_ws(_p(xh), _p(xl), _p(sx), _p(wh), _p(wl), _p(sw), _p(bias_p), _p(residual), _p(y),
                                                      _p(amax_rec), C.byref(g), _p(ws), wsb, _stream()), 'conv_fwd_f16x3_ws')
            return y
        _lib.check(_lib_().wdno_conv_fwd_f16x3_amax(_p(xh), _p(xl), _p(sx), _p(wh), _p(wl), _p(sw), _p(bias_p), _p(residual), _p(y),
                                                    _p(amax_rec), C.byref(g), _stream()), 'conv_fwd_f16x3')
    return y


_split_ws_bytes = {}


_pixel_tables = {}


def _fwd_h3_kernel_name(pixels, k, ks, tap=False, c=None):
    cdiv = lambda a, b: -(-a // b)
    tiles = cdiv(pixels, 128) * cdiv(k, 128) if k > 64 else cdiv(pixels, 256)
    small_tap = tap and ks[2] == 3 and cdiv(pixels, 64) * cdiv(k, 64) >= 64
    if (tiles >= 100 or small_tap) and max(ks) <= 8:
        cus = 256
        cost = lambda bm, bn, wgt: cdiv(cdiv(pixels, bm) * cdiv(k, bn), cus) * bm * bn * wgt
        shapes = [(256, 64, 1.04), (192, 64, 1.08)] if k <= 64 else [(128, 128, 1.0), (192, 128, 1.0), (256, 64, 1.04), (192, 64, 1.08)]
        best = shapes[0]
        for sh in shapes[1:]:
            if cost(*sh) < cost(*best):
                best = sh
        if tap and ks[2] == 3:
            c_best = cost(*best)
            if k > 64 and cost(160, 128, 1.02) < c_best:
                best, c_best = (160, 128, 1.02), cost(160, 128, 1.02)
            if cost(320, 64, 1.05) < c_best:
                best, c_best = (320, 64, 1.05), cost(320, 64, 1.05)
            if cost(128, 64, 1.15) < c_best:
                best, c_best = (128, 64, 1.15), cost(128, 64, 1.15)
            if cost(64, 64, 1.35) < c_best:
                best = (64, 64, 1.35)
            if best[:2] == (64, 64) and c is not None and c % 32 == 0 and k >= 128:
                t128, nst = cdiv(pixels, 128) * cdiv(k, 128), ks[0] * ks[1] * (c // 32)
                if t128 * 4 <= cus and nst % 4 == 0 and nst // 4 >= 8:
                    return 'conv_fwd_h3t_kernel<128,128>/4'
        if tap and _lp() and k > 64 and cdiv(pixels, 256) * cdiv(k, 128) >= 2 * cus:
            best = (256, 128)
        if tap and ks[2] == 7:
            best = (256, 64)
            if not _lp() and cdiv(pixels, 256) < cus and cdiv(pixels, 256) < cdiv(pixels, 192) <= cus:
                best = (192, 64)
        return f'conv_fwd_h3{"t" if tap else "d"}_kernel<{best[0]},{best[1]}>'
    return 'conv_fwd_h3_kernel<..,128>' if k > 64 else 'conv_fwd_h3_kernel<..,64>'


def _wgrad_h3_kernel_name(k, run, window=False):
    if window == 'stem':
        return 'conv_wgrad_h3s_kernel<64,352>'
    if window:
        return 'conv_wgrad_h3w_kernel<64,384>'
    cdiv = lambda a, b: -(-a // b)
    bn = 192 if cdiv(run, 192) * 192 <= cdiv(run, 128) * 128 else 128
    return f'conv_wgrad_h3d_kernel<{128 if k > 64 else 64},{bn}>'


FLAT_WGRAD = True
_FLAT_ARMED = False
DEFER_WGRAD_REDUCE = True
_WGRAD_PENDING = None
WGRAD_FLUSH_BYTES = int(os.environ.get('WDNO_WGRAD_FLUSH_MB', '0')) << 20
DEFER_ROW_SUMS = True
_ROWSUM_PENDING = []
_DEFERRED_DSTS = set()


def flush_wgrad_reduces():
    global _WGRAD_PENDING, _ROWSUM_PENDING
    pend, rows = _WGRAD_PENDING, _ROWSUM_PENDING
    if rows:
        _ROWSUM_PENDING = []
        ritems = (_lib.RowsSumItem * len(rows))(*[it for it, _ in rows])
        _lib.check(_lib_().wdno_rows_sum_multi(C.cast(ritems, C.c_void_p), len(rows), _stream()), 'rows_sum_multi')
        _DEFERRED_DSTS.update(int(it.out) for it, _ in rows)
    if not pend:
        return
    _WGRAD_PENDING = [] if _FLAT_ARMED else None
    items = (_lib.WgradReduceItem * len(pend))(*[it for it, _ in pend])
    _lib.check(_lib_().wdno_wgrad_reduce_multi(C.cast(items, C.c_void_p), len(pend), _stream()), 'wgrad_reduce_multi')
    _DEFERRED_DSTS.update(int(it.dw) for it, _ in pend)


class _RowsJob:
    __slots__ = ('keep', 'ptr', 'rows', 'stride', 'col0', 'ncols', 'is_double')

    def __init__(self, keep, ptr, rows, stride, col0, ncols, is_double):
        self.keep, self.ptr, self.rows, self.stride, self.col0, self.ncols, self.is_double = keep, ptr, rows, stride, col0, ncols, is_double

    def item(self, out, ncols=None):
        it = _lib.RowsSumItem()
        it.part, it.out, it.rows, it.stride, it.col0 = self.ptr, out.data_ptr(), self.rows, self.stride, self.col0
        it.ncols, it.is_double, it.reserved = self.ncols if ncols is None else ncols, self.is_double, 0
        return it


def rows_sum_for_param(job, param, ncols=None, out=None):
    n = job.ncols if ncols is None else ncols
    if out is None and DEFER_ROW_SUMS and _WGRAD_PENDING is not None and param is not None:
        out = _flat_grad_out(param, (n,))
    if out is not None:
        _ROWSUM_PENDING.append((job.item(out, n), job.keep))
        return out
    dev = job.keep.device
    out = torch.empty((n,), device=dev, dtype=torch.float32)
    items = (_lib.RowsSumItem * 1)(job.item(out, n))
    _lib.check(_lib_().wdno_rows_sum_multi(C.cast(items, C.c_void_p), 1, _stream()), 'rows_sum_multi')
    return out


def take_deferred_dsts():
    global _DEFERRED_DSTS
    d, _DEFERRED_DSTS = _DEFERRED_DSTS, set()
    return d


@contextlib.contextmanager
def flat_wgrad_scope():
    global _FLAT_ARMED, _WGRAD_PENDING
    prev, _FLAT_ARMED = _FLAT_ARMED, True
    outer = _WGRAD_PENDING
    if DEFER_WGRAD_REDUCE and outer is None:
        _WGRAD_PENDING = []
    try:
        yield
    finally:
        _FLAT_ARMED = prev
        if outer is None:
            try:
                flush_wgrad_reduces()
            finally:
                _WGRAD_PENDING = None


def _flat_grad_out(w, shape):
    v = getattr(w, '_wdno_flat_grad', None)
    if v is None or not FLAT_WGRAD or not _FLAT_ARMED or w.grad is not None or getattr(w, '_wdno_flat_busy', True) or v.numel() != math.prod(shape) or v.device != w.device:
        return None
    w._wdno_flat_busy = True
    return v.view(shape)


def conv_wgrad_h3(xplanes, shape4, gyplanes, osp, ks, st, pd, param_kc=None, out=None):
    xh, xl, sx = xplanes
    gh, gl, sg = gyplanes
    n, d, h, ww = shape4
    c8, k8 = xh.shape[-1], gh.shape[-1]
    g = _geom((n, d, h, ww), c8, k8, ks, st, pd, osp)
    lib = _lib_()
    nb = lib.wdno_conv_wgrad_f16x3_ws_bytes(C.byref(g))
    ws = _ws(nb, xh.device)
    tkey = (str(xh.device), n, d, h, ww, c8, tuple(osp), tuple(ks), tuple(st), tuple(pd))
    table = _pixel_tables.get(tkey)
    if table is None:
        table = torch.empty((n * osp[0] * osp[1] * osp[2], 4), device=xh.device, dtype=torch.int32)
        _lib.check(lib.wdno_conv_pixel_table(_p(table), C.byref(g), _stream()), 'conv_pixel_table')
        _pixel_tables[tkey] = table
    flops = 2.0 * n * osp[0] * osp[1] * osp[2] * k8 * ks[0] * ks[1] * ks[2] * c8
    window = tuple(st) == (1, 1, 1) and tuple(osp) == (d, h, ww) and ks[2] == 3 and pd[2] == 1 and c8 % 64 == 0
    if tuple(st) == (1, 1, 1) and tuple(osp) == (d, h, ww) and ks[2] == 7 and pd[2] == 3 and c8 == 48 and k8 <= 64 and max(ks) <= 8:
        window = 'stem'
    if param_kc is not None and out is not None and _WGRAD_PENDING is not None:
        kn, cn = param_kc
        dw = out
        item = _lib.WgradReduceItem()
        with _timed(_wgrad_h3_kernel_name(k8, ks[2] * c8, window), flops):
            _lib.check(lib.wdno_conv_wgrad_partials(_p(xh), _p(xl), _p(sx), _p(gh), _p(gl), _p(sg), _p(table), _p(dw), kn, cn, _p(ws), nb, C.byref(g),
                                                    C.byref(item), _stream()), 'conv_wgrad_partials')
        _WGRAD_PENDING.append((item, ws))
        if WGRAD_FLUSH_BYTES and sum(w.numel() for _, w in _WGRAD_PENDING) > WGRAD_FLUSH_BYTES:
            flush_wgrad_reduces()
        return dw
    if xl is None:
        assert param_kc is not None
        kn, cn = param_kc
        dw = out if out is not None else torch.empty((kn, cn, *ks), device=xh.device, dtype=torch.float32)
        with _timed(_wgrad_h3_kernel_name(k8, ks[2] * c8, window), flops):
            _lib.check(lib.wdno_conv_wgrad_bf16_param(_p(xh), _p(gh), _p(table), _p(dw), kn, cn, _p(ws), nb, C.byref(g), _stream()), 'conv_wgrad_bf16_param')
        return dw
    if param_kc is not None:
        kn, cn = param_kc
        dw = out if out is not None else torch.empty((kn, cn, *ks), device=xh.device, dtype=torch.float32)
        with _timed(_wgrad_h3_kernel_name(k8, ks[2] * c8, window), flops):
            _lib.check(lib.wdno_conv_wgrad_f16x3_param(_p(xh), _p(xl), _p(sx), _p(gh), _p(gl), _p(sg), _p(table), _p(dw), kn, cn, _p(ws), nb,
                                                       C.byref(g), _stream()), 'conv_wgrad_f16x3_param')
        return dw
    dwp = torch.empty((ks[0], ks[1], k8, ks[2], c8), device=xh.device, dtype=torch.float32)
    with _timed(_wgrad_h3_kernel_name(k8, ks[2] * c8, window), flops):
        _lib.check(lib.wdno_conv_wgrad_f16x3(_p(xh), _p(xl), _p(sx), _p(gh), _p(gl), _p(sg), _p(table), _p(dwp), _p(ws), nb, C.byref(g), _stream()),
                   'conv_wgrad_f16x3')
    return dwp


def _use_h3(pixels, reduction):
    return CONV_MATH in ('f16x3', 'bf16') and pixels >= H3_MIN_PIXELS and reduction >= H3_MIN_REDUCTION


def conv_reads_planes(pixels, weight):
    if not PLANES_FWD or CONV_MATH not in ('f16x3', 'bf16') or weight.dim() < 2:
        return False
    k, c = weight.shape[0], weight.shape[1]
    vol = 1
    for v in weight.shape[2:]:
        vol *= v
    if pixels <= LINEAR_ROWS_MAX and weight.dim() == 2:
        return False
    return pad4(c) % 8 == 0 and _use_h3(pixels, pad4(c) * vol)


POISON = os.environ.get('WDNO_POISON', '0') == '1'


def _poison(t):
    if POISON:
        t.fill_(float('nan'))
    return t


def _planes_only(t, planes):
    _poison(t)
    t._wdno_planes = (planes, t._version, CONV_MATH)
    t._wdno_unwritten = True
    return t


def _out_size(n, k, s, p):
    return (n + 2 * p - k) // s + 1


def conv_fwd_raw(x, wp, bias_p, residual, ks, st, pd, kp):
    n, d, h, w, cp = x.shape
    osp = tuple(_out_size(a, k, s, p) for a, k, s, p in zip((d, h, w), ks, st, pd))
    y = torch.empty((n, *osp, kp), device=x.device, dtype=torch.float32)
    g = _geom((n, d, h, w), cp, kp, ks, st, pd, osp)
    flops = 2.0 * n * osp[0] * osp[1] * osp[2] * kp * ks[0] * ks[1] * ks[2] * cp
    with _timed('conv_fwd_kernel<128,2,2>' if kp > 64 else 'conv_fwd_kernel<64,4,1>', flops):
        _lib.check(_lib_().wdno_conv_fwd(_p(x), _p(wp), _p(bias_p), _p(residual), _p(y), C.byref(g), _stream()), 'conv_fwd')
    return y


def conv_wgrad_raw(x, dy, ks, st, pd):
    n, d, h, w, cp = x.shape
    kp = dy.shape[-1]
    osp = tuple(dy.shape[1:4])
    g = _geom((n, d, h, w), cp, kp, ks, st, pd, osp)
    lib = _lib_()
    nb = lib.wdno_conv_wgrad_ws_bytes(C.byref(g))
    ws = _ws(nb, x.device)
    dwp = torch.empty((ks[0], ks[1], kp, ks[2], cp), device=x.device, dtype=torch.float32)
    flops = 2.0 * n * osp[0] * osp[1] * osp[2] * kp * ks[0] * ks[1] * ks[2] * cp
    with _timed('conv_wgrad_kernel<128,2,2>' if kp > 64 else 'conv_wgrad_kernel<64,1,4>', flops):
        _lib.check(lib.wdno_conv_wgrad(_p(x), _p(dy), _p(dwp), _p(ws), nb, C.byref(g), _stream()), 'conv_wgrad')
    return dwp


def conv_transpose_raw(x, wt, bias_p, cout_p):
    n, d, h, w, cp = x.shape
    y = torch.empty((n, d, 2 * h, 2 * w, cout_p), device=x.device, dtype=torch.float32)
    lib = _lib_()
    for py in range(2):
        for px in range(2):
            g = _geom((n, d, h, w), cp, cout_p, (1, 2, 2), (1, 1, 1), (0, 1 - py, 1 - px), (d, h, w),
                      y_sp=(d, 2 * h, 2 * w), ostride=(1, 2, 2), ooff=(0, py, px))
            _lib.check(lib.wdno_conv_fwd(_p(x), _p(wt[py, px]), _p(bias_p), None, _p(y), C.byref(g), _stream()), 'conv_transpose')
    return y


def colsum(x2d):
    p, c = x2d.shape
    lib = _lib_()
    nb = lib.wdno_colsum_ws_bytes(p, c)
    ws = _ws(nb, x2d.device)
    out = torch.empty((c,), device=x2d.device, dtype=torch.float32)
    _lib.check(lib.wdno_colsum(_p(x2d), _p(out), p, c, _p(ws), nb, _stream()), 'colsum')
    return out


def _pad_vec(v, n):
    if v is None or v.shape[0] == n:
        return v
    out = v.new_zeros((n,))
    out[:v.shape[0]] = v
    return out


LINEAR_MULTI_ROWS_MAX = 256
LINEAR_ROWS_MAX = 64


def _linear_rows_backward(ctx, gy):
    x, weight = ctx.saved_tensors
    _, _, _, k, c, cp, kp, has_bias, _, _, _ = ctx.meta
    gy = _chk(gy, 'grad')
    rows = x.shape[0]
    lib = _lib_()
    gx = gw = gb = None
    if ctx.needs_input_grad[0]:
        wt = _cached(weight, 'lin_t', 0, 0, lambda: weight.detach().t())
        gx = torch.empty((rows, cp), device=x.device, dtype=torch.float32)
        _lib.check(lib.wdno_linear_rows_fwd(_p(gy), kp, _p(wt), k, None, _p(gx), rows, k, c, cp, _stream()), 'linear_rows_dgrad')
    if ctx.needs_input_grad[1] or (has_bias and ctx.needs_input_grad[2]):
        gw = torch.empty((k, c), device=x.device, dtype=torch.float32)
        gb = torch.empty((k,), device=x.device, dtype=torch.float32) if has_bias else None
        _lib.check(lib.wdno_linear_rows_wgrad(_p(x), cp, _p(gy), kp, _p(gw), _p(gb), rows, c, k, _stream()), 'linear_rows_wgrad')
        gw = gw.reshape(weight.shape)
        if not ctx.needs_input_grad[1]:
            gw = None
        if not (has_bias and ctx.needs_input_grad[2]):
            gb = None
    return gx, gw, gb, None, None, None


class _Conv(torch.autograd.Function):

    @staticmethod
    def forward(ctx, x, weight, bias, residual, stride, padding, with_skip=False, grad_planes=False, to_norm=False):
        ctx.with_skip = with_skip
        ctx.to_norm = to_norm and grad_planes
        ctx.bias_ref = bias
        y = _Conv._forward(ctx, x, weight, bias, residual, stride, padding)
        if grad_planes and not ctx.rows and ctx.h3 and y.dim() in (4, 5) and residual is None:
            ks, st = ctx.meta[0], ctx.meta[1]
            n_, d_, h_, w_, _ = ctx.xshape
            if not ctx.needs_input_grad[0] or (st == (1, 1, 1) and _use_h3(n_ * d_ * h_ * w_, ctx.meta[6] * ks[0] * ks[1] * ks[2])):
                y._wdno_grad_planes = True
        if with_skip:
            return y, _alias_of(x)
        return y

    @staticmethod
    def _forward(ctx, x, weight, bias, residual, stride, padding):
        xrec = _known_amax(x)
        x_in = x
        ctx.x16 = x.dtype == torch.bfloat16
        if ctx.x16:
            if not (getattr(x, '_wdno_unwritten', False) and x.is_cuda):
                raise RuntimeError('wdno_amd: a bf16 tensor that is not a planes-only placeholder reached a convolution')
            x = x if x.is_contiguous() else x.contiguous()
        else:
            x = _chk(x, 'x')
        lead = None
        if x.dim() != 5:
            lead = x.shape[:-1]
            x5 = x.reshape(1, 1, 1, -1, x.shape[-1]) if x.dim() != 4 else x.unsqueeze(1)
        else:
            x5 = x
        w5 = _as5(weight)
        k, c = w5.shape[0], w5.shape[1]
        cp, kp = x5.shape[-1], pad4(k)
        assert cp == pad4(c), f'channel mismatch: tensor has {cp}, weight expects {c}'
        ks = tuple(w5.shape[2:])
        if x.dim() == 2 and x.shape[0] <= LINEAR_ROWS_MAX and weight.dim() == 2 and residual is None and c % 4 == 0 and k % 4 == 0:
            wc = weight.detach()
            wc = wc if wc.is_contiguous() else wc.contiguous()
            rows = x.shape[0]
            y = torch.empty((rows, kp), device=x.device, dtype=torch.float32)
            _lib.check(_lib_().wdno_linear_rows_fwd(_p(x), cp, _p(wc), c, _p(None if bias is None else bias.detach()), _p(y), rows, c, k, kp,
                                                    _stream()), 'linear_rows_fwd')
            ctx.save_for_backward(x, weight)
            ctx.h3 = False
            ctx.rows = True
            ctx.meta = (ks, stride, padding, k, c, cp, kp, bias is not None, False, lead, 2)
            return y
        ctx.rows = False
        with torch.no_grad():
            bias_p = _pad_vec(bias.detach() if bias is not None else None, kp)
        res5 = None
        if residual is not None:
            residual = _chk(residual, 'residual')
            res5 = residual
        osp_ = tuple(_out_size(a, kk, s_, p_) for a, kk, s_, p_ in zip(x5.shape[1:4], ks, stride, padding))
        h3 = _use_h3(x5.shape[0] * osp_[0] * osp_[1] * osp_[2], cp * ks[0] * ks[1] * ks[2])
        if getattr(x_in, '_wdno_unwritten', False):
            hp = getattr(x_in, '_wdno_planes', None)
            if not (h3 and hp is not None and hp[1] == x_in._version and hp[2] == CONV_MATH):
                raise RuntimeError('wdno_amd: a planes-only tensor reached a convolution that reads fp32')
        if h3:
            c8w = pad8(cp) + 8 if (ks[2] == 7 and kp <= 64 and tuple(stride) == (1, 1, 1) and pad8(cp) % 16) else None
            planes = split_f16_of(x_in, x5.reshape(-1, cp), xrec, c8w)
            yrec = _new_amax_record(x5.device)
            nx_, dx_, hx_, wx_ = x5.shape[:4]
            out16 = (ACT16 and _lp() and getattr(ctx, 'to_norm', False) and GRAD_PLANES and residual is None and x.dim() in (4, 5) and kp % 8 == 0
                     and kp // 8 <= 256 and (kp // 8) & (kp // 8 - 1) == 0
                     and (not ctx.needs_input_grad[0] or (tuple(stride) == (1, 1, 1) and _use_h3(nx_ * dx_ * hx_ * wx_, kp * ks[0] * ks[1] * ks[2]))))
            y = _leave_amax(conv_fwd_h3(planes, tuple(x5.shape[:4]), weight, pack_fwd, 'f', bias_p, res5, ks, stride, padding, kp,
                                        amax_rec=yrec, zero_box=zero_box_of(x_in) if x_in.dim() == 5 else None, out16=out16), yrec)
            ctx.save_for_backward(planes[0], planes[1], planes[2], weight)
        else:
            y = conv_fwd_raw(x5, pack_fwd(weight, cp, kp), bias_p, res5, ks, stride, padding, kp)
            ctx.save_for_backward(x5, weight)
        ctx.h3 = h3
        ctx.xshape = tuple(x5.shape)
        ctx.meta = (ks, stride, padding, k, c, cp, kp, bias is not None, residual is not None, lead, x.dim())
        if lead is not None:
            y = y.reshape(*lead, kp) if x.dim() != 4 else y.squeeze(1)
        return y

    @staticmethod
    def backward(ctx, gy, gskip=None):
        if ctx.rows:
            return _linear_rows_backward(ctx, gy) + (None, None, None)
        return _Conv._backward(ctx, gy, gskip) + (None, None, None)

    @staticmethod
    def _backward(ctx, gy, gskip):
        if ctx.h3:
            xh, xl, sx, weight = ctx.saved_tensors
            x5 = None
        else:
            x5, weight = ctx.saved_tensors
        ks, stride, padding, k, c, cp, kp, has_bias, has_res, lead, xdim = ctx.meta
        grec = _known_amax(gy)
        po = getattr(gy, '_wdno_planes_only', None)
        if po is not None and gy.dtype == torch.bfloat16:
            gy = gy if gy.is_contiguous() else gy.contiguous()
        else:
            gy = _chk(gy, 'grad')
        n, d, h, w, _ = ctx.xshape
        gyplanes = None
        gb_given = None
        if po is not None:
            if not (ctx.h3 and po[2] == gy._version and po[3] == CONV_MATH and not has_res):
                raise RuntimeError('wdno_amd: a planes-only gradient reached a convolution that cannot take it')
            gyplanes, gb_given = po[0], po[1]
        osp = tuple(_out_size(a, kk, s, p) for a, kk, s, p in zip((d, h, w), ks, stride, padding))
        gy5 = gy.reshape(n, *osp, kp)
        gx = gw = gb = gr = None
        want_gb = has_bias and ctx.needs_input_grad[2]
        will_split = (ctx.needs_input_grad[1] and ctx.h3) or (ctx.needs_input_grad[0] and stride == (1, 1, 1)
                                                              and _use_h3(n * d * h * w, kp * ks[0] * ks[1] * ks[2]))
        if po is not None:
            if not (will_split and (not ctx.needs_input_grad[0] or (stride == (1, 1, 1) and _use_h3(n * d * h * w, kp * ks[0] * ks[1] * ks[2])))):
                raise RuntimeError('wdno_amd: a planes-only gradient reached a convolution whose backward needs fp32 dy')
            if want_gb:
                gb = rows_sum_for_param(gb_given, getattr(ctx, 'bias_ref', None), k) if isinstance(gb_given, _RowsJob) else gb_given[:k].contiguous()
        elif want_gb and will_split:
            gyplanes, gbs = split_f16_colsum(gy5.reshape(-1, kp), grec, bias=getattr(ctx, 'bias_ref', None), k=k)
            gb = gbs[:k].contiguous()
        if ctx.needs_input_grad[0]:
            gs5 = None if gskip is None else _chk(gskip, 'skip gradient').reshape(n, d, h, w, cp)
            if stride == (1, 1, 1):
                pd = tuple(kk - 1 - p for kk, p in zip(ks, padding))
                if _use_h3(n * d * h * w, kp * ks[0] * ks[1] * ks[2]):
                    if gyplanes is None:
                        gyplanes = split_f16(gy5.reshape(-1, kp), grec)
                    drec = _new_amax_record(gy5.device)
                    gx5 = _leave_amax(conv_fwd_h3(gyplanes, tuple(gy5.shape[:4]), weight, lambda w_, c8_, k_: pack_dgrad(w_, k_, c8_), 'd', None, gs5,
                                                  ks, (1, 1, 1), pd, cp, amax_rec=drec, out16=getattr(ctx, 'x16', False) and gs5 is None), drec)
                else:
                    wd = pack_dgrad(weight, cp, kp)
                    gx5 = conv_fwd_raw(gy5, wd, None, gs5, ks, (1, 1, 1), pd, cp)
                gs5 = None
            elif ks == (1, 4, 4) and stride == (1, 2, 2) and padding == (0, 1, 1):
                oh_, ow_ = gy5.shape[2], gy5.shape[3]
                if ctx.h3 and _use_h3(n * d * oh_ * ow_, kp * 4) and _as5(weight).is_contiguous():
                    if gyplanes is None:
                        gyplanes = split_f16(gy5.reshape(-1, kp), grec)
                    drec = _new_amax_record(gy5.device)
                    gx5 = _leave_amax(conv_transpose_h3(gyplanes, tuple(gy5.shape[:4]), _as5(weight), None, cp, amax_rec=drec), drec)
                else:
                    wt = pack_transposed(_as5(weight), kp, cp)
                    gx5 = conv_transpose_raw(gy5, wt, None, cp)
            elif ks == (1, 2, 2) and stride == (1, 2, 2) and padding == (0, 0, 0):
                if ctx.h3 and _use_h3(n * d * gy5.shape[2] * gy5.shape[3], kp) and _as5(weight).is_contiguous() and PATCH_DGRAD_H3:
                    if gyplanes is None:
                        gyplanes = split_f16(gy5.reshape(-1, kp), grec)
                    drec = _new_amax_record(gy5.device)
                    gx5 = _leave_amax(_patch2_dgrad(gy5, weight, cp, kp, gyplanes, drec), drec)
                else:
                    gx5 = _patch2_dgrad(gy5, weight, cp, kp)
            else:
                raise RuntimeError(f'wdno_amd: unsupported convolution geometry for dgrad {ks} {stride} {padding}')
            if gs5 is not None:
                gx5 = gx5 + gs5
            if getattr(ctx, 'x16', False) and gx5.dtype != torch.bfloat16:
                gx5 = gx5.to(torch.bfloat16)
            gx = gx5
            if lead is not None:
                gx = gx5.reshape(*lead, cp) if xdim != 4 else gx5.squeeze(1)
        if ctx.needs_input_grad[1]:
            if ctx.h3:
                if gyplanes is None:
                    gyplanes = split_f16(gy5.reshape(-1, kp), grec)
                gw = conv_wgrad_h3((xh, xl, sx), (n, d, h, w), gyplanes, osp, ks, stride, padding, param_kc=(k, c),
                                   out=_flat_grad_out(weight, (k, c, *ks))).reshape(weight.shape)
            else:
                dwp = conv_wgrad_raw(x5, gy5, ks, stride, padding)
                gw = dwp[:, :, :k, :, :c].permute(2, 4, 0, 1, 3).reshape(weight.shape).contiguous()
        if want_gb and gb is None:
            gb = colsum(gy5.reshape(-1, kp))[:k].contiguous()
        if has_res and ctx.needs_input_grad[3]:
            gr = gy
        return gx, gw, gb, gr, None, None


def _patch2_dgrad(gy5, weight, cp, kp, gyplanes=None, amax_rec=None):
    n, d, oh, ow, _ = gy5.shape
    w5 = _as5(weight)
    gx = torch.empty((n, d, 2 * oh, 2 * ow, cp), device=gy5.device, dtype=torch.float32)
    lib = _lib_()
    if gyplanes is not None:
        for py in range(2):
            for px in range(2):
                conv_fwd_h3(gyplanes, (n, d, oh, ow), w5, None, f'q{py}{px}', None, None, (1, 1, 1), (1, 1, 1), (0, 0, 0), cp, out=gx,
                            osp=(d, oh, ow), ostride=(1, 2, 2), ooff=(0, py, px), amax_rec=amax_rec)
        return gx

    def build():
        wz = _padded(w5.detach(), kp, cp)
        return wz.permute(3, 4, 1, 0, 2).reshape(2, 2, cp, kp)
    wq = _cached(weight, 'p2', cp, kp, build)
    for py in range(2):
        for px in range(2):
            g = _geom((n, d, oh, ow), kp, cp, (1, 1, 1), (1, 1, 1), (0, 0, 0), (d, oh, ow),
                      y_sp=(d, 2 * oh, 2 * ow), ostride=(1, 2, 2), ooff=(0, py, px))
            _lib.check(lib.wdno_conv_fwd(_p(gy5), _p(wq[py, px]), None, None, _p(gx), C.byref(g), _stream()), 'patch2_dgrad')
    return gx


def conv_cl(x, weight, bias=None, stride=1, padding=0, residual=None, with_skip=False, grad_planes=False, to_norm=False):
    nd = weight.dim() - 2

    def trip(v, fill):
        if nd == 0:
            return (fill,) * 3
        v = (v,) * nd if isinstance(v, int) else tuple(v)
        return (fill,) * (3 - nd) + v
    return _Conv.apply(x, weight, bias, residual, trip(stride, 1), trip(padding, 0) if nd else (0, 0, 0), with_skip, grad_planes, to_norm)


def conv_cl_skip(x, weight, bias=None, stride=1, padding=0, grad_planes=False, to_norm=False):
    return conv_cl(x, weight, bias, stride, padding, None, True, grad_planes, to_norm)


class _ConvT(torch.autograd.Function):

    @staticmethod
    def forward(ctx, x, weight, bias):
        xrec = _known_amax(x)
        x = _chk(x, 'x')
        cin, cout = weight.shape[0], weight.shape[1]
        cin_p, cout_p = x.shape[-1], pad4(cout)
        assert cin_p == pad4(cin) and tuple(weight.shape[2:]) == (1, 4, 4)
        with torch.no_grad():
            bias_p = _pad_vec(bias.detach() if bias is not None else None, cout_p)
        n, d, h, w = x.shape[:4]
        h3 = _use_h3(n * d * h * w, 4 * cin_p) and cout_p % 8 == 0
        if h3:
            planes = split_f16(x.reshape(-1, cin_p), xrec)
            yrec = _new_amax_record(x.device)
            y = _leave_amax(conv_transpose_h3(planes, (n, d, h, w), weight, bias_p, cout_p, yrec), yrec)
            ctx.save_for_backward(weight, *planes)
        else:
            y = conv_transpose_raw(x, pack_transposed(weight, cin_p, cout_p), bias_p, cout_p)
            ctx.save_for_backward(x, weight)
        ctx.meta = (cin, cout, cin_p, cout_p, bias is not None, h3, (n, d, h, w))
        return y

    @staticmethod
    def backward(ctx, gy):
        cin, cout, cin_p, cout_p, has_bias, h3, xshape4 = ctx.meta
        grec = _known_amax(gy)
        gy = _chk(gy, 'grad')
        ks, st, pd = (1, 4, 4), (1, 2, 2), (0, 1, 1)
        gx = gw = gb = None
        if h3:
            weight, xh, xl, sx = ctx.saved_tensors
            gyplanes = split_f16(gy.reshape(-1, cout_p), grec)
            gshape4 = tuple(gy.shape[:4])
            if ctx.needs_input_grad[0]:
                gx = conv_fwd_h3(gyplanes, gshape4, weight, pack_fwd, 'f', None, None, ks, st, pd, cin_p)
            if ctx.needs_input_grad[1]:
                gw = conv_wgrad_h3(gyplanes, gshape4, (xh, xl, sx), xshape4[1:], ks, st, pd, param_kc=(cin, cout),
                                   out=_flat_grad_out(weight, (cin, cout, 1, 4, 4)))
            if has_bias and ctx.needs_input_grad[2]:
                gb = colsum(gy.reshape(-1, cout_p))[:cout].contiguous()
            return gx, gw, gb
        x, weight = ctx.saved_tensors
        if ctx.needs_input_grad[0]:
            wp = pack_fwd(weight, cout_p, cin_p)
            gx = conv_fwd_raw(gy, wp, None, None, ks, st, pd, cin_p)
        if ctx.needs_input_grad[1]:
            dwp = conv_wgrad_raw(gy, x, ks, st, pd)
            gw = dwp[:, :, :cin, :, :cout].permute(2, 4, 0, 1, 3).contiguous()
        if has_bias and ctx.needs_input_grad[2]:
            gb = colsum(gy.reshape(-1, cout_p))[:cout].contiguous()
        return gx, gw, gb


class _LinearItem(C.Structure):
    _fields_ = [('w', C.c_void_p), ('bias', C.c_void_p), ('K', C.c_int), ('k_start', C.c_int)]


_lin_tables = {}


def _linear_table(weights, biases, c):
    key = (tuple(w.data_ptr() for w in weights), tuple(0 if b is None else b.data_ptr() for b in biases), c)
    tab = _lin_tables.get(key)
    if tab is None:
        if len(_lin_tables) > 64:
            _lin_tables.clear()
        items = (_LinearItem * len(weights))()
        ks, start = [], 0
        for i, (w, b) in enumerate(zip(weights, biases)):
            items[i] = _LinearItem(w.data_ptr(), None if b is None else b.data_ptr(), w.shape[0], start)
            ks.append((w.shape[0], start))
            start += w.shape[0]
        dev = torch.frombuffer(bytearray(bytes(items)), dtype=torch.uint8).to(weights[0].device)
        tab = (dev, ks, start)
        _lin_tables[key] = tab
    return tab


class _LinearMulti(torch.autograd.Function):
    @staticmethod
    def forward(ctx, x, n, *wb):
        weights, biases = wb[:n], wb[n:]
        x = _chk(x, 'x')
        p, c = x.shape
        tab, ks, f = _linear_table(weights, biases, c)
        ybuf = torch.empty((p * f,), device=x.device, dtype=torch.float32)
        _lib.check(_lib_().wdno_linear_multi_fwd(_p(tab), len(ks), f, _p(x), _p(ybuf), p, c, _stream()), 'linear_multi_fwd')
        gbuf = torch.empty_like(ybuf)
        outs = []
        for k, start in ks:
            o = ybuf[p * start:p * (start + k)].view(p, k)
            o._wdno_grad_slot = gbuf[p * start:p * (start + k)].view(p, k)
            outs.append(o)
        ctx.save_for_backward(x, *[w for w in weights])
        ctx.meta = (tab, ks, f, p, c, [b is not None for b in biases])
        ctx.gbuf = gbuf
        return tuple(outs)

    @staticmethod
    def backward(ctx, *gys):
        x = ctx.saved_tensors[0]
        tab, ks, f, p, c, has_bias = ctx.meta
# ... 683 lines not shown
```

Before: 33.51.

## Skip zero-box regions in stem wgrad via host-planned item schedule

```diff
diff --git a/include/wdno_hip.h b/include/wdno_hip.h
--- a/include/wdno_hip.h
+++ b/include/wdno_hip.h
@@ -113,6 +113,13 @@
                              const void* pixel_table, float* dw, int Kn, int Cn, void* ws, size_t ws_bytes,
                              const wdno_conv_geom* g, wdno_wgrad_reduce_item* item, wdno_stream_t s);
 int wdno_wgrad_reduce_multi(const wdno_wgrad_reduce_item* items, int n_items, wdno_stream_t s);
+int wdno_conv_wgrad_f16x3_param_zbox(const void* xh, const void* xl, const float* sx, const void* dyh, const void* dyl, const float* sdy,
+                                     const void* pixel_table, float* dw, int Kn, int Cn, void* ws, size_t ws_bytes,
+                                     const wdno_conv_geom* g, const wdno_zero_box* zb, wdno_stream_t s);
+int wdno_conv_wgrad_partials_zbox(const void* xh, const void* xl, const float* sx, const void* dyh, const void* dyl, const float* sdy,
+                                  const void* pixel_table, float* dw, int Kn, int Cn, void* ws, size_t ws_bytes,
+                                  const wdno_conv_geom* g, const wdno_zero_box* zb, wdno_wgrad_reduce_item* item, wdno_stream_t s);
+int wdno_stem_wgrad_plan(const wdno_conv_geom* g, const wdno_zero_box* zb, int64_t* grid_live, int64_t* box_live, int* splits);
 size_t wdno_conv_wgrad_ws_bytes(const wdno_conv_geom* g);
 int wdno_conv_wgrad(const float* x, const float* dy, float* dwp, void* ws, size_t ws_bytes,
                     const wdno_conv_geom* g, wdno_stream_t s);
@@ -132,6 +139,8 @@
                        const wdno_conv_geom* g, wdno_stream_t s);
 int wdno_conv_wgrad_bf16_param(const void* x16, const void* dy16, const void* pixel_table, float* dw, int Kn, int Cn, void* ws,
                                size_t ws_bytes, const wdno_conv_geom* g, wdno_stream_t s);
+int wdno_conv_wgrad_bf16_param_zbox(const void* x16, const void* dy16, const void* pixel_table, float* dw, int Kn, int Cn, void* ws,
+                                    size_t ws_bytes, const wdno_conv_geom* g, const wdno_zero_box* zb, wdno_stream_t s);
 
 size_t wdno_groupnorm_ws_bytes(int64_t N, int64_t S, int C, int G);
 size_t wdno_groupnorm_stats_floats(int64_t N, int C, int G);
diff --git a/wdno_amd/_lib.py b/wdno_amd/_lib.py
--- a/wdno_amd/_lib.py
+++ b/wdno_amd/_lib.py
@@ -91,6 +91,9 @@
     'wdno_conv_wgrad_f16x3_param': (I, [P, P, P, P, P, P, P, P, I, I, P, Z, PG, P]),
     'wdno_conv_wgrad_partials': (I, [P, P, P, P, P, P, P, P, I, I, P, Z, PG, P, P]),
     'wdno_wgrad_reduce_multi': (I, [P, I, P]),
+    'wdno_conv_wgrad_f16x3_param_zbox': (I, [P, P, P, P, P, P, P, P, I, I, P, Z, PG, P, P]),
+    'wdno_conv_wgrad_partials_zbox': (I, [P, P, P, P, P, P, P, P, I, I, P, Z, PG, P, P, P]),
+    'wdno_stem_wgrad_plan': (I, [PG, P, P, P, P]),
     'wdno_rows_sum_multi': (I, [P, I, P]),
     'wdno_cast_bf16': (I, [P, P, L, I, I, P]),
     'wdno_cast_bf16_colsum': (I, [P, P, P, P, Z, L, I, I, P]),
@@ -98,6 +101,7 @@
     'wdno_conv_fwd_f16x3_zbox': (I, [P, P, P, P, P, P, P, P, P, P, PG, P, P]),
     'wdno_conv_fwd_bf16_ex': (I, [P, P, P, P, P, I, P, PG, P, P]),
     'wdno_conv_wgrad_bf16_param': (I, [P, P, P, P, I, I, P, Z, PG, P]),
+    'wdno_conv_wgrad_bf16_param_zbox': (I, [P, P, P, P, I, I, P, Z, PG, P, P]),
     'wdno_conv_wgrad_ws_bytes': (Z, [PG]),
     'wdno_conv_wgrad': (I, [P, P, P, P, Z, PG, P]),
     'wdno_colsum_ws_bytes': (Z, [L, I]),
diff --git a/wdno_amd/csrc/conv_common.h b/wdno_amd/csrc/conv_common.h
--- a/wdno_amd/csrc/conv_common.h
+++ b/wdno_amd/csrc/conv_common.h
@@ -53,7 +53,7 @@
 #include "debug_modes.h"
 void wdno_wgrad_h3d_plan(const wdno_conv_geom* g, int* bm, int* bn, int* splits, int* pix_per_split, int* splitpair = nullptr);
 int wdno_conv_wgrad_h3_dma(const void* xh, const void* xl, const void* dyh, const void* dyl, const float* sx, const float* sdy,
-                           const void* table, float* wsf, const wdno_conv_geom* g, hipStream_t st);
+                           const void* table, float* wsf, const wdno_conv_geom* g, hipStream_t st, const wdno_zero_box* zb = nullptr);
 int wdno_conv_fwd_h3_dma(const void* xh, const void* xl, const void* wh, const void* wl, const float* sx, const float* sw,
                          const float* bias, const float* residual, float* y, ConvP& p, hipStream_t st, int stages);
 bool wdno_conv_h3t_takes(const wdno_conv_geom& g);
diff --git a/wdno_amd/csrc/conv_h3.hip b/wdno_amd/csrc/conv_h3.hip
--- a/wdno_amd/csrc/conv_h3.hip
+++ b/wdno_amd/csrc/conv_h3.hip
@@ -879,7 +879,7 @@
 }
 static int wgrad_h3_partials(const void* xh, const void* xl, const float* sx, const void* dyh, const void* dyl, const float* sdy,
                              const void* pixel_table, float* single, void* ws, size_t ws_bytes, const wdno_conv_geom* g, hipStream_t st,
-                             int* splits_out) {
+                             int* splits_out, const wdno_zero_box* zb = nullptr) {
   int rc = check_geom(g);
   if (rc) return rc;
   if ((g->C & 7) || (g->K & 7) || !pixel_table) return WDNO_EUNSUPPORTED;
@@ -893,7 +893,7 @@
     size_t need_d = (size_t)splits * g->kd * g->kh * (size_t)g->K * w.c.R * sizeof(float);
     float* dst = (splits == 1 && single) ? single : (float*)ws;
     if (dst == (float*)ws && ws_bytes < need_d) return WDNO_EWORKSPACE;
-    rc = wdno_conv_wgrad_h3_dma(xh, xl, dyh, dyl, sx, sdy, pixel_table, dst, g, st);
+    rc = wdno_conv_wgrad_h3_dma(xh, xl, dyh, dyl, sx, sdy, pixel_table, dst, g, st, zb);
     if (rc == WDNO_OK) { *splits_out = splits; return WDNO_OK; }
     if (rc != WDNO_EUNSUPPORTED) return rc;
   }
@@ -1052,25 +1052,31 @@
   }
   wgrad_h3_reduce_nat_kernel<<<stream_grid(n / 4, 32), 256, 0, st>>>(ws, dw, n, splits, g->K, g->C, g->kw, g->kd * g->kh, Kn, Cn);
 }
+extern "C" int wdno_conv_wgrad_f16x3_param_zbox(const void* xh, const void* xl, const float* sx, const void* dyh, const void* dyl, const float* sdy,
+                                                const void* pixel_table, float* dw, int Kn, int Cn, void* ws, size_t ws_bytes,
+                                                const wdno_conv_geom* g, const wdno_zero_box* zb, wdno_stream_t s) {
+  WDNO_REQUIRE(g && Kn > 0 && Cn > 0 && Kn <= g->K && Cn <= g->C);
+  hipStream_t st = as_stream(s);
+  int splits = 0;
+  int rc = wgrad_h3_partials(xh, xl, sx, dyh, dyl, sdy, pixel_table, nullptr, ws, ws_bytes, g, st, &splits, zb);
+  if (rc) return rc;
+  const int64_t n = (int64_t)g->kd * g->kh * g->K * (int64_t)g->kw * g->C;
+  wgrad_h3_reduce_launch((const float*)ws, dw, n, splits, g, Kn, Cn, st);
+  return wdno_check_launch();
+}
+
 extern "C" int wdno_conv_wgrad_f16x3_param(const void* xh, const void* xl, const float* sx, const void* dyh, const void* dyl, const float* sdy,
                                            const void* pixel_table, float* dw, int Kn, int Cn, void* ws, size_t ws_bytes,
                                            const wdno_conv_geom* g, wdno_stream_t s) {
-  WDNO_REQUIRE(g && Kn > 0 && Cn > 0 && Kn <= g->K && Cn <= g->C);
-  hipStream_t st = as_stream(s);
-  int splits = 0;
-  int rc = wgrad_h3_partials(xh, xl, sx, dyh, dyl, sdy, pixel_table, nullptr, ws, ws_bytes, g, st, &splits);
-  if (rc) return rc;
-  const int64_t n = (int64_t)g->kd * g->kh * g->K * (int64_t)g->kw * g->C;
-  wgrad_h3_reduce_launch((const float*)ws, dw, n, splits, g, Kn, Cn, st);
-  return wdno_check_launch();
-}
-
-extern "C" int wdno_conv_wgrad_partials(const void* xh, const void* xl, const float* sx, const void* dyh, const void* dyl, const float* sdy,
-                                        const void* pixel_table, float* dw, int Kn, int Cn, void* ws, size_t ws_bytes,
-                                        const wdno_conv_geom* g, wdno_wgrad_reduce_item* item, wdno_stream_t s) {
+  return wdno_conv_wgrad_f16x3_param_zbox(xh, xl, sx, dyh, dyl, sdy, pixel_table, dw, Kn, Cn, ws, ws_bytes, g, nullptr, s);
+}
+
+extern "C" int wdno_conv_wgrad_partials_zbox(const void* xh, const void* xl, const float* sx, const void* dyh, const void* dyl, const float* sdy,
+                                             const void* pixel_table, float* dw, int Kn, int Cn, void* ws, size_t ws_bytes,
+                                             const wdno_conv_geom* g, const wdno_zero_box* zb, wdno_wgrad_reduce_item* item, wdno_stream_t s) {
   WDNO_REQUIRE(g && item && dw && Kn > 0 && Cn > 0 && Kn <= g->K && Cn <= g->C);
   int splits = 0;
-  int rc = wgrad_h3_partials(xh, xl, sx, dyh, dyl, sdy, pixel_table, nullptr, ws, ws_bytes, g, as_stream(s), &splits);
+  int rc = wgrad_h3_partials(xh, xl, sx, dyh, dyl, sdy, pixel_table, nullptr, ws, ws_bytes, g, as_stream(s), &splits, zb);
   if (rc) return rc;
   const int64_t n = (int64_t)g->kd * g->kh * g->K * (int64_t)g->kw * g->C;
   if (n >= 0x7fffffff) return WDNO_EUNSUPPORTED;
@@ -1079,16 +1085,26 @@
   return wdno_check_launch();
 }
 
-extern "C" int wdno_conv_wgrad_bf16_param(const void* x16, const void* dy16, const void* pixel_table, float* dw, int Kn, int Cn, void* ws,
-                                          size_t ws_bytes, const wdno_conv_geom* g, wdno_stream_t s) {
+extern "C" int wdno_conv_wgrad_partials(const void* xh, const void* xl, const float* sx, const void* dyh, const void* dyl, const float* sdy,
+                                        const void* pixel_table, float* dw, int Kn, int Cn, void* ws, size_t ws_bytes,
+                                        const wdno_conv_geom* g, wdno_wgrad_reduce_item* item, wdno_stream_t s) {
+  return wdno_conv_wgrad_partials_zbox(xh, xl, sx, dyh, dyl, sdy, pixel_table, dw, Kn, Cn, ws, ws_bytes, g, nullptr, item, s);
+}
+
+extern "C" int wdno_conv_wgrad_bf16_param_zbox(const void* x16, const void* dy16, const void* pixel_table, float* dw, int Kn, int Cn, void* ws,
+                                               size_t ws_bytes, const wdno_conv_geom* g, const wdno_zero_box* zb, wdno_stream_t s) {
   WDNO_REQUIRE(g && Kn > 0 && Cn > 0 && Kn <= g->K && Cn <= g->C);
   hipStream_t st = as_stream(s);
   int splits = 0;
-  int rc = wgrad_h3_partials(x16, nullptr, nullptr, dy16, nullptr, nullptr, pixel_table, nullptr, ws, ws_bytes, g, st, &splits);
+  int rc = wgrad_h3_partials(x16, nullptr, nullptr, dy16, nullptr, nullptr, pixel_table, nullptr, ws, ws_bytes, g, st, &splits, zb);
   if (rc) return rc;
   const int64_t n = (int64_t)g->kd * g->kh * g->K * (int64_t)g->kw * g->C;
   wgrad_h3_reduce_launch((const float*)ws, dw, n, splits, g, Kn, Cn, st);
   return wdno_check_launch();
+}
+extern "C" int wdno_conv_wgrad_bf16_param(const void* x16, const void* dy16, const void* pixel_table, float* dw, int Kn, int Cn, void* ws,
+                                          size_t ws_bytes, const wdno_conv_geom* g, wdno_stream_t s) {
+  return wdno_conv_wgrad_bf16_param_zbox(x16, dy16, pixel_table, dw, Kn, Cn, ws, ws_bytes, g, nullptr, s);
 }
 
 #define PS_LDS_FLOATS 10240
diff --git a/wdno_amd/csrc/conv_wgrad_h3d.hip b/wdno_amd/csrc/conv_wgrad_h3d.hip
--- a/wdno_amd/csrc/conv_wgrad_h3d.hip
+++ b/wdno_amd/csrc/conv_wgrad_h3d.hip
@@ -1,5 +1,9 @@
 #include "conv_common.h"
 #include <type_traits>
+#include <algorithm>
+#include <cstring>
+#include <mutex>
+#include <vector>
 
 typedef _Float16 half8 __attribute__((ext_vector_type(8)));
 typedef __bf16 bf16x8 __attribute__((ext_vector_type(8)));
@@ -696,14 +700,34 @@
 #ifndef WDNO_H3S_STAGES
 #define WDNO_H3S_STAGES 4
 #endif
+#define WD_STEM_SLOTS 1024
+struct StemItems {
+  unsigned short id[WD_STEM_SLOTS];
+  int rounds;
+};
+__device__ __forceinline__ int wd_stem_item(const StemItems& t, int i) {
+  const unsigned v = reinterpret_cast<const unsigned*>(t.id)[i >> 1];
+  return __builtin_amdgcn_readfirstlane((int)((v >> (16 * (i & 1))) & 0xffffu));
+}
+__host__ __device__ __forceinline__ int wd_stem_step_mode(int W, int H, int D, int w, int h, int d, int n, int vdz, int vdy, int zd, int zh) {
+  int mode = 0;
+  while (n > 0) {
+    const int sd = d + vdz, sh = h + vdy;
+    if ((unsigned)sd < (unsigned)D && (unsigned)sh < (unsigned)H) mode |= (sd < zd && sh < zh) ? 3 : 1;
+    n -= W - w; w = 0;
+    if (++h == H) { h = 0; if (++d == D) d = 0; }
+  }
+  return mode;
+}
 template <bool LP>
 __global__ __launch_bounds__(512) void conv_wgrad_h3s_kernel(const _Float16* __restrict__ xh, const _Float16* __restrict__ xl,
                                                               const _Float16* __restrict__ dyh, const _Float16* __restrict__ dyl,
                                                               const float* __restrict__ sx, const float* __restrict__ sdy,
-                                                              float* __restrict__ ws, WgradDP wp, unsigned x_bytes, unsigned dy_bytes) {
+                                                              float* __restrict__ ws, WgradDP wp, const StemItems items, unsigned x_bytes, unsigned dy_bytes) {
   constexpr int KW = 7, CX = 48, NS = WDNO_H3S_STAGES, TM = 2;
-  constexpr int ROWB = CX * 2, XROWS = 32 + KW - 1, X_DATA = XROWS * ROWB;
-  constexpr int A_PLANE = 4096, X_PLANE = 4096, ZADDR = X_DATA;
+  constexpr int ROWB = CX * 2, XROWS = 32 + KW - 1;
+  constexpr int XZERO = 3840;
+  constexpr int A_PLANE = 4096, X_PLANE = 4096;
   constexpr int NPL = LP ? 1 : 2;
   constexpr int A_LO = A_PLANE, B_HI = NPL * A_PLANE, B_LO = B_HI + X_PLANE;
   constexpr int STAGE = NPL * (A_PLANE + X_PLANE);
@@ -713,19 +737,13 @@
   const wdno_conv_geom& g = p.g;
   const int tid = threadIdx.x;
   const int wave = __builtin_amdgcn_readfirstlane(tid >> 6), lane = tid & 63;
-  int it_first, it_stride, my_items;
-  if (wp.xcd_chunk > 0) {
-    const int xcd = (int)blockIdx.x & 7, idx = (int)blockIdx.x >> 3;
-    const int beg = xcd * wp.xcd_chunk, end = min(beg + wp.xcd_chunk, wp.items);
-    it_stride = (int)gridDim.x >> 3;
-    it_first = beg + idx;
-    my_items = it_first < end ? (end - it_first + it_stride - 1) / it_stride : 0;
-  } else {
-    it_first = (int)blockIdx.x; it_stride = (int)gridDim.x;
-    my_items = (wp.items - it_first + it_stride - 1) / it_stride;
-  }
+  const int nblk = (int)gridDim.x, blk = (int)blockIdx.x;
+  int my_items = 0;
+  while (my_items < items.rounds && wd_stem_item(items, my_items * nblk + blk) != 0xffff) ++my_items;
   const int ntap = g.kd * g.kh;
   const int total = my_items * wp.nsteps;
+  const bool boxed = p.zb_blocks >= 2 && p.debug != WDNO_DBG_STEM_EVERY_STAGE;
+  const int zd = boxed ? min(g.D, p.zb_d) : g.D, zh = boxed ? min(g.H, p.zb_h) : g.H;
 
   if (wave >= 4) {
     const int pq = wave - 4;
@@ -735,13 +753,14 @@
     const int f = 64 * pq + lane;
     const int xr = f / (ROWB / 16), xc = f - xr * (ROWB / 16);
     const bool x_slot = xr < XROWS;
+    const int xzd = xc < 4 ? zd : g.D, xzh = xc < 4 ? zh : g.H;
     const int gi = f >> 5, du = (f >> 4) & 1, dj = (f >> 2) & 3, dc = f & 3;
     const int dpix = 16 * (gi >> 2) + 8 * ((gi >> 1) & 1) + (gi & 1) + 2 * dj;
     const bool d_slot = du * 32 + dc * 8 < g.K;
     int it = 0, st = 0;
     int q = 0, qw = 0, qh = 0, qd = 0, x_off = 0, dp = 0, d_off = 0, vdz = 0, vdy = 0;
     auto setup_item = [&]() {
-      const int id = it_first + it * it_stride;
+      const int id = wd_stem_item(items, it * nblk + blk);
       const int tap = id % ntap, split = id / ntap;
       const int dz = tap / g.kh, dy = tap - dz * g.kh;
       vdz = dz - g.pd; vdy = dy - g.ph;
@@ -759,7 +778,7 @@
     const bool no_dma = p.debug == WDNO_DBG_NO_DMA;
     auto issue_next = [&](int buf) {
       const unsigned sb = lds0 + buf * STAGE + pq * 1024;
-      const bool xv = x_slot && q >= 0 && q < (int)p.P && (unsigned)(qd + vdz) < (unsigned)g.D && (unsigned)(qh + vdy) < (unsigned)g.H;
+      const bool xv = x_slot && q >= 0 && q < (int)p.P && (unsigned)(qd + vdz) < (unsigned)xzd && (unsigned)(qh + vdy) < (unsigned)xzh;
       const int xo = xv && !no_dma ? x_off : WD_OOB;
       const int d_o = d_slot && dp < (int)p.P && !no_dma ? d_off : WD_OOB;
       wd_piece(rdh, d_o, sb);
@@ -792,21 +811,22 @@
   const int step_ow = 32 % g.W;
   const int a_base = hh * 1024 + fj * 64 + g1 * 32 + c4 * 8;
 
-  auto run = [&](auto TNC) {
-    constexpr int TN = decltype(TNC)::value;
-    const int tb0 = 3 * wave;
+  auto run = [&](auto NAC) {
+    constexpr int NA = decltype(NAC)::value, TN = NA + 1;
     int xbase[TN][4], rd[TN][4], dlo[TN], ow[4];
 #pragma unroll
     for (int b = 0; b < TN; ++b) {
-      const int r = 32 * (tb0 + b) + 16 * g1 + 4 * c4;
-      const int dx = r / CX;
+      const int dx = b < NA ? wave + 4 * b : 2 * wave + g1;
       dlo[b] = dx < KW ? g.pw - dx : (1 << 20);
 #pragma unroll
-      for (int c = 0; c < 4; ++c) xbase[b][c] = (16 * (c >> 1) + 8 * hh + (c & 1) + 2 * fj) * ROWB + 2 * r;
+      for (int c = 0; c < 4; ++c) {
+        const int row = 16 * (c >> 1) + 8 * hh + (c & 1) + 2 * fj + dx;
+        xbase[b][c] = ROWB * row + (b < NA ? 32 * g1 : 64) + 8 * c4;
+      }
     }
     auto select = [&](int c) {
 #pragma unroll
-      for (int b = 0; b < TN; ++b) rd[b][c] = (unsigned)(ow[c] - dlo[b]) < (unsigned)g.W ? xbase[b][c] : 3840 + (xbase[b][c] & 255);
+      for (int b = 0; b < TN; ++b) rd[b][c] = (unsigned)(ow[c] - dlo[b]) < (unsigned)g.W ? xbase[b][c] : XZERO + (xbase[b][c] & 255);
     };
     auto advance = [&](int c) {
       ow[c] += step_ow;
@@ -818,7 +838,7 @@
       const short4v h1 = __builtin_amdgcn_ds_read_tr16_b64_v4i16((lds_s4)a1);
       return __builtin_bit_cast(half8, (short8v)__builtin_shufflevector(h0, h1, 0, 1, 2, 3, 4, 5, 6, 7));
     };
-    auto read_frags = [&](auto SET, int stage, int ks) {
+    auto read_dy = [&](auto SET, int stage, int ks) {
       constexpr int B = decltype(SET)::value;
       const char* st = smem + stage * STAGE;
 #pragma unroll
@@ -827,32 +847,36 @@
         fah[B][a] = tr2(pa, pa + 512);
         if (!LP) fal[B][a] = tr2(pa + A_LO, pa + A_LO + 512);
       }
-#pragma unroll
-      for (int b = 0; b < TN; ++b) {
+    };
+    auto read_x = [&](auto SET, auto B0C, auto B1C, int stage, int ks) {
+      constexpr int B = decltype(SET)::value;
+      const char* st = smem + stage * STAGE;
+#pragma unroll
+      for (int b = decltype(B0C)::value; b < decltype(B1C)::value; ++b) {
         fbh[B][b] = tr2(st + B_HI + rd[b][2 * ks], st + B_HI + rd[b][2 * ks + 1]);
         if (!LP) fbl[B][b] = tr2(st + B_LO + rd[b][2 * ks], st + B_LO + rd[b][2 * ks + 1]);
       }
     };
     f32x16 acc[TM][TN];
-    auto mfma_set = [&](auto SET) {
-      constexpr int B = decltype(SET)::value;
+    auto mfma_set = [&](auto SET, auto B0C, auto B1C) {
+      constexpr int B = decltype(SET)::value, b0 = decltype(B0C)::value, b1 = decltype(B1C)::value;
       if constexpr (!LP) {
 #pragma unroll
         for (int a = 0; a < TM; ++a)
 #pragma unroll
-          for (int b = 0; b < TN; ++b) acc[a][b] = mfma_16<false>(fbh[B][b], fal[B][a], acc[a][b]);
+          for (int b = b0; b < b1; ++b) acc[a][b] = mfma_16<false>(fbh[B][b], fal[B][a], acc[a][b]);
 #pragma unroll
         for (int a = 0; a < TM; ++a)
 #pragma unroll
-          for (int b = 0; b < TN; ++b) acc[a][b] = mfma_16<false>(fbl[B][b], fah[B][a], acc[a][b]);
+          for (int b = b0; b < b1; ++b) acc[a][b] = mfma_16<false>(fbl[B][b], fah[B][a], acc[a][b]);
       }
 #pragma unroll
       for (int a = 0; a < TM; ++a)
 #pragma unroll
-        for (int b = 0; b < TN; ++b) acc[a][b] = mfma_16<LP>(fbh[B][b], fah[B][a], acc[a][b]);
-    };
-    constexpr int NRD = NPL * 2 * (TM + TN), NMF = (LP ? 1 : 3) * TM * TN, RPM = (NRD + NMF - 1) / NMF;
-    auto interleave = [&]() {
+        for (int b = b0; b < b1; ++b) acc[a][b] = mfma_16<LP>(fbh[B][b], fah[B][a], acc[a][b]);
+    };
+    auto interleave = [&](auto NRDC, auto NMFC) {
+      constexpr int NRD = decltype(NRDC)::value, NMF = decltype(NMFC)::value, RPM = (NRD + NMF - 1) / NMF;
 #pragma unroll
       for (int i = 0; i < NMF; ++i) {
         __builtin_amdgcn_sched_group_barrier(0x008, 1, 0);
@@ -861,10 +885,25 @@
     };
     using B0 = std::integral_constant<int, 0>;
     using B1 = std::integral_constant<int, 1>;
+    using TA = std::integral_constant<int, NA>;
+    using TT = std::integral_constant<int, TN>;
+    constexpr int PRD = (LP ? 1 : 2) * 2, PMF = (LP ? 1 : 3) * TM;
+    auto half_step = [&](auto RS, int stage, int ks, bool rd_a, auto MS, bool mf_a) {
+      read_dy(RS, stage, ks);
+      read_x(RS, TA{}, TT{}, stage, ks);
+      mfma_set(MS, TA{}, TT{});
+      interleave(std::integral_constant<int, PRD * (TM + 1)>{}, std::integral_constant<int, PMF>{});
+      __builtin_amdgcn_sched_barrier(0);
+      const int ra = __builtin_amdgcn_readfirstlane((int)rd_a), ma = __builtin_amdgcn_readfirstlane((int)mf_a);
+      if (ra) read_x(RS, B0{}, TA{}, stage, ks);
+      if (ma) mfma_set(MS, B0{}, TA{});
+      __builtin_amdgcn_sched_barrier(0);
+    };
     int stage = 0;
     for (int t = 0; t < my_items; ++t) {
-      const int id = it_first + t * it_stride;
+      const int id = wd_stem_item(items, t * nblk + blk);
       const int tap = id % ntap, split = id / ntap;
+      const int dz = tap / g.kh, vdz = dz - g.pd, vdy = tap - dz * g.kh - g.ph;
       const int pbeg = split * wp.pix_per_split;
 #pragma unroll
       for (int c = 0; c < 4; ++c) ow[c] = (pbeg + 16 * (c >> 1) + 8 * hh + (c & 1) + 2 * fj) % g.OW;
@@ -874,33 +913,37 @@
         for (int b = 0; b < TN; ++b)
 #pragma unroll
           for (int e = 0; e < 16; ++e) acc[a][b][e] = 0.f;
+      int sw = pbeg % g.W, sh = (pbeg / g.W) % g.H, sd = (pbeg / (g.W * g.H)) % g.D, srem = (int)p.P - pbeg;
+      auto next_box_live = [&]() {
+        const int m = __builtin_amdgcn_readfirstlane(wd_stem_step_mode(g.W, g.H, g.D, sw, sh, sd, min(srem, 32), vdz, vdy, zd, zh));
+        srem -= 32; sw += 32;
+        while (sw >= g.W) { sw -= g.W; if (++sh == g.H) { sh = 0; if (++sd == g.D) sd = 0; } }
+        return m == 3;
+      };
+      bool c3 = next_box_live();
       select(0); select(1);
       lgkm0_barrier();
-      read_frags(B0{}, stage, 0);
+      read_dy(B0{}, stage, 0);
+      read_x(B0{}, TA{}, TT{}, stage, 0);
+      if (c3) read_x(B0{}, B0{}, TA{}, stage, 0);
       advance(0); advance(1);
       for (int step = 0; step + 1 < wp.nsteps; ++step) {
+        const bool n3 = next_box_live();
         select(2); select(3);
-        read_frags(B1{}, stage, 1);
+        half_step(B1{}, stage, 1, c3, B0{}, c3);
         advance(2); advance(3);
-        mfma_set(B0{});
-        interleave();
-        __builtin_amdgcn_sched_barrier(0);
         stage = stage + 1 == NS ? 0 : stage + 1;
         select(0); select(1);
         lgkm0_barrier();
-        read_frags(B0{}, stage, 0);
+        half_step(B0{}, stage, 0, n3, B1{}, c3);
         advance(0); advance(1);
-        mfma_set(B1{});
-        interleave();
-        __builtin_amdgcn_sched_barrier(0);
+        c3 = n3;
       }
       select(2); select(3);
-      read_frags(B1{}, stage, 1);
-      mfma_set(B0{});
-      interleave();
-      __builtin_amdgcn_sched_barrier(0);
+      half_step(B1{}, stage, 1, c3, B0{}, c3);
       stage = stage + 1 == NS ? 0 : stage + 1;
-      mfma_set(B1{});
+      mfma_set(B1{}, TA{}, TT{});
+      if (c3) mfma_set(B1{}, B0{}, TA{});
       __builtin_amdgcn_sched_barrier(0);
       float* out = ws + ((int64_t)split * ntap + tap) * (int64_t)g.K * p.R;
 #pragma unroll
@@ -912,16 +955,18 @@
         for (int b = 0; b < TN; ++b) {
 #pragma unroll
           for (int e4 = 0; e4 < 4; ++e4) {
-            const int rr = 32 * (tb0 + b) + 8 * e4 + 4 * hh;
-            if (rr < p.R)
+            const int en = 8 * e4 + 4 * hh;
+            const int dx = b < NA ? wave + 4 * b : 2 * wave + (en >> 4);
+            const int rr = dx * CX + (b < NA ? en : 32 + (en & 15));
+            if (dx < KW)
               *reinterpret_cast<float4*>(orow + rr) = make_float4(acc[a][b][4 * e4] * inv, acc[a][b][4 * e4 + 1] * inv, acc[a][b][4 * e4 + 2] * inv, acc[a][b][4 * e4 + 3] * inv);
           }
         }
       }
     }
   };
-  if (wave < 3) run(std::integral_constant<int, 3>{});
-  else run(std::integral_constant<int, 2>{});
+  if (wave < 3) run(std::integral_constant<int, 2>{});
+  else run(std::integral_constant<int, 1>{});
 }
 
 static int wd_num_cus() {
@@ -951,7 +996,7 @@
   if (splitpair) *splitpair = 0;
   if (wd_stem_takes(g)) {
     *bm = 64; *bn = 352;
-    int64_t want = 256 / (g->kd * g->kh);
+    int64_t want = 512 / (g->kd * g->kh);
     int64_t max_splits = cdiv64(c.P, 16 * 32);
     if (want > max_splits) want = max_splits;
     if (want < 1) want = 1;
@@ -1044,28 +1089,119 @@
                                                        sx, sdy, (const int4v*)table, wsf, wl, x_bytes, dy_bytes, tbl_bytes);
 }
 
+static bool wd_stem_hinted(const wdno_conv_geom* g, const wdno_zero_box* zb) {
+  return zb && zb->channels >= 32 && zb->d0 >= 0 && zb->h0 >= 0 && (zb->d0 < g->D || zb->h0 < g->H);
+}
+struct StemPlan {
+  wdno_conv_geom g;
+  int hinted, zd, zh, rr, cus;
+  int splits, pps, grid;
+  int64_t grid_live, box_live;
+  StemItems items;
+};
+static const StemPlan* wd_stem_plan(const wdno_conv_geom* g, const wdno_zero_box* zb) {
+  static std::mutex mu;
+  static std::vector<StemPlan*> cache;
+  const int hinted = wd_stem_hinted(g, zb) ? 1 : 0;
+  const int zd = hinted ? std::min(g->D, zb->d0) : g->D, zh = hinted ? std::min(g->H, zb->h0) : g->H;
+  const int rr = wdno_debug_mode == WDNO_DBG_WGRAD_NO_XCD_GROUPING ? 1 : 0, cus = wd_num_cus();
+  std::lock_guard<std::mutex> lock(mu);
+  for (const StemPlan* c : cache)
+    if (!memcmp(&c->g, g, sizeof(*g)) && c->hinted == hinted && c->zd == zd && c->zh == zh && c->rr == rr && c->cus == cus) return c;
+  StemPlan* sp = new StemPlan;
+  memset(sp, 0, sizeof(*sp));
+  sp->g = *g; sp->hinted = hinted; sp->zd = zd; sp->zh = zh; sp->rr = rr; sp->cus = cus;
+  int bm, bn;
+  wdno_wgrad_h3d_plan(g, &bm, &bn, &sp->splits, &sp->pps, nullptr);
+  const int ntap = g->kd * g->kh, nsteps = sp->pps / 32, nitems = ntap * sp->splits;
+  const int64_t P = (int64_t)g->N * g->D * g->H * g->W;
+  std::vector<int64_t> cost(nitems);
+  for (int id = 0; id < nitems; ++id) {
+    const int tap = id % ntap, split = id / ntap, vdz = tap / g->kh - g->pd, vdy = tap % g->kh - g->ph;
+    int64_t q = (int64_t)split * sp->pps, n3 = 0, n1 = 0;
+    for (int step = 0; step < nsteps; ++step, q += 32) {
+      if (q >= P) break;
+      const int m = wd_stem_step_mode(g->W, g->H, g->D, (int)(q % g->W), (int)((q / g->W) % g->H), (int)((q / ((int64_t)g->W * g->H)) % g->D),
+                                      (int)std::min<int64_t>(32, P - q), vdz, vdy, zd, zh);
+      n3 += m == 3; n1 += m == 1;
+    }
+    sp->grid_live += n3 + n1; sp->box_live += n3;
+    cost[id] = 60 * n3 + 20 * (nsteps - n3) + 240;
+  }
+  std::vector<std::vector<int>> bins;
+  auto in_order = [&]() {
+    int grid = std::min(cus, nitems);
+    bins.assign(grid, {});
+    if (grid >= 64 && !rr) {
+      const int chunk = cdiv(nitems, 8);
+      grid = std::min(cus & ~7, 8 * chunk);
+      bins.assign(grid, {});
+      for (int b = 0; b < grid; ++b)
+        for (int id = (b & 7) * chunk + (b >> 3); id < std::min(((b & 7) + 1) * chunk, nitems); id += grid >> 3) bins[b].push_back(id);
+    } else {
+      for (int id = 0; id < nitems; ++id) bins[id % grid].push_back(id);
+    }
+  };
+  auto rounds_of = [&]() { size_t r = 0; for (auto& b : bins) r = std::max(r, b.size()); return (int)r; };
+  if (hinted && nitems > 1) {
+    const bool xcd = cus >= 64 && nitems >= 64 && !rr;
+    const int grid = xcd ? std::min(cus & ~7, nitems & ~7) : std::min(cus, nitems);
+    std::vector<int> order(nitems);
+    for (int i = 0; i < nitems; ++i) order[i] = i;
+    std::stable_sort(order.begin(), order.end(), [&](int a, int b) { return cost[a] > cost[b]; });
+    std::vector<int64_t> load(grid, 0);
+    bins.assign(grid, {});
+    for (int id : order) {
+      int best = 0;
+      for (int b = 1; b < grid; ++b) if (load[b] < load[best]) best = b;
+      bins[best].push_back(id); load[best] += cost[id];
+    }
+    std::stable_sort(bins.begin(), bins.end(), [](const std::vector<int>& a, const std::vector<int>& b) {
+      return !a.empty() && (b.empty() || a[0] < b[0]); });
+    if (xcd) {
+      std::vector<std::vector<int>> byx(grid);
+      const int per = grid >> 3;
+      for (int j2 = 0; j2 < grid; ++j2) byx[(j2 % per) * 8 + j2 / per] = bins[j2];
+      bins.swap(byx);
+    }
+    if ((int64_t)rounds_of() * grid > WD_STEM_SLOTS) in_order();
+  } else {
+    in_order();
+  }
+  sp->grid = (int)bins.size();
+  sp->items.rounds = rounds_of();
+  if ((int64_t)sp->items.rounds * sp->grid > WD_STEM_SLOTS || nitems >= 0xffff) sp->grid = 0;
+  else {
+    for (int i = 0; i < WD_STEM_SLOTS; ++i) sp->items.id[i] = 0xffff;
+    for (int b = 0; b < sp->grid; ++b)
+      for (size_t r = 0; r < bins[b].size(); ++r) sp->items.id[r * sp->grid + b] = (unsigned short)bins[b][r];
+  }
+  cache.push_back(sp);
+  return sp;
+}
+extern "C" int wdno_stem_wgrad_plan(const wdno_conv_geom* g, const wdno_zero_box* zb, int64_t* grid_live, int64_t* box_live, int* splits) {
+  if (check_geom(g) != WDNO_OK) return WDNO_EINVAL;
+  if (!wd_stem_takes(g)) return WDNO_EUNSUPPORTED;
+  const StemPlan* sp = wd_stem_plan(g, zb);
+  if (grid_live) *grid_live = sp->grid_live;
+  if (box_live) *box_live = wdno_debug_mode == WDNO_DBG_STEM_EVERY_STAGE ? sp->grid_live : sp->box_live;
+  if (splits) *splits = sp->splits;
+  return WDNO_OK;
+}
+
 template <bool LP>
 static void launch_ws(const void* xh, const void* xl, const void* dyh, const void* dyl, const float* sx, const float* sdy,
-                      float* wsf, const WgradDP& w, hipStream_t st) {
+                      float* wsf, const WgradDP& w, const StemPlan* sp, hipStream_t st) {
   const wdno_conv_geom& g = w.c.g;
   const unsigned x_bytes = (unsigned)((int64_t)g.N * g.D * g.H * g.W * g.C * 2);
   const unsigned dy_bytes = (unsigned)((int64_t)g.N * g.YD * g.YH * g.YW * g.K * 2);
   const size_t lds = (size_t)WDNO_H3S_STAGES * (LP ? 1 : 2) * (4096 + 4096);
-  int grid = wd_num_cus();
-  if (w.items < grid) grid = w.items;
-  WgradDP wl = w;
-  wl.xcd_chunk = 0;
-  if (grid >= 64 && wdno_debug_mode != WDNO_DBG_WGRAD_NO_XCD_GROUPING) {
-    wl.xcd_chunk = cdiv(w.items, 8);
-    grid = wd_num_cus() & ~7;
-    if (8 * wl.xcd_chunk < grid) grid = 8 * wl.xcd_chunk;
-  }
-  conv_wgrad_h3s_kernel<LP><<<grid, 512, lds, st>>>((const _Float16*)xh, (const _Float16*)xl, (const _Float16*)dyh, (const _Float16*)dyl,
-                                                   sx, sdy, wsf, wl, x_bytes, dy_bytes);
+  conv_wgrad_h3s_kernel<LP><<<sp->grid, 512, lds, st>>>((const _Float16*)xh, (const _Float16*)xl, (const _Float16*)dyh, (const _Float16*)dyl,
+                                                       sx, sdy, wsf, w, sp->items, x_bytes, dy_bytes);
 }
 
 int wdno_conv_wgrad_h3_dma(const void* xh, const void* xl, const void* dyh, const void* dyl, const float* sx, const float* sdy,
-                           const void* table, float* wsf, const wdno_conv_geom* g, hipStream_t st) {
+                           const void* table, float* wsf, const wdno_conv_geom* g, hipStream_t st, const wdno_zero_box* zb) {
   WgradDP w;
   fill_params(w.c, g);
   int bm, bn;
@@ -1078,10 +1214,13 @@
   w.items = w.tiles_k * w.tiles_r * g->kd * g->kh * w.splits;
   if (wd_stem_takes(g)) {
     if ((int64_t)g->N * g->D * g->H * g->W * g->C * 2 >= WD_OOB || w.c.P * g->K * 2 >= WD_OOB) return WDNO_EUNSUPPORTED;
+    const StemPlan* sp = wd_stem_plan(g, zb);
+    if (sp->grid == 0) return WDNO_EUNSUPPORTED;
     w.tiles_k = w.tiles_r = 1;
     w.items = g->kd * g->kh * w.splits;
-    if (xl == nullptr) launch_ws<true>(xh, xh, dyh, dyh, sx, sdy, wsf, w, st);
-    else launch_ws<false>(xh, xl, dyh, dyl, sx, sdy, wsf, w, st);
+    if (sp->hinted) { w.c.zb_blocks = zb->channels / 16; w.c.zb_d = zb->d0; w.c.zb_h = zb->h0; }
+    if (xl == nullptr) launch_ws<true>(xh, xh, dyh, dyh, sx, sdy, wsf, w, sp, st);
+    else launch_ws<false>(xh, xl, dyh, dyl, sx, sdy, wsf, w, sp, st);
     return WDNO_OK;
   }
   if (wd_window_takes(g)) {
diff --git a/wdno_amd/csrc/debug_modes.h b/wdno_amd/csrc/debug_modes.h
--- a/wdno_amd/csrc/debug_modes.h
+++ b/wdno_amd/csrc/debug_modes.h
@@ -25,7 +25,8 @@
   X(WDNO_DBG_ATTN_GENERIC_NTOK, 44)      \
   X(WDNO_DBG_DWT3_SYNTH_LDS, 45)              \
   X(WDNO_DBG_CONV_NO_RUN_SPLIT, 56)      \
-  X(WDNO_DBG_STEM_EVERY_STAGE, 57)                  \
+       \
+  X(WDNO_DBG_STEM_EVERY_STAGE, 57)                                                                                                                 \
   X(WDNO_DBG_ATTN_FWD_ROWS, 67)          \
   X(WDNO_DBG_ATTN_BWD_ROWS, 68)                                              \
   X(WDNO_DBG_WGRAD_NO_SPLIT_PAIR, 70)    \
diff --git a/wdno_amd/ops.py b/wdno_amd/ops.py
--- a/wdno_amd/ops.py
+++ b/wdno_amd/ops.py
@@ -855,7 +855,7 @@
     return v.view(shape)
 
 
-def conv_wgrad_h3(xplanes, shape4, gyplanes, osp, ks, st, pd, param_kc=None, out=None):
+def conv_wgrad_h3(xplanes, shape4, gyplanes, osp, ks, st, pd, param_kc=None, out=None, zero_box=None):
     xh, xl, sx = xplanes
     gh, gl, sg = gyplanes
     n, d, h, ww = shape4
@@ -874,13 +874,18 @@
     window = tuple(st) == (1, 1, 1) and tuple(osp) == (d, h, ww) and ks[2] == 3 and pd[2] == 1 and c8 % 64 == 0
     if tuple(st) == (1, 1, 1) and tuple(osp) == (d, h, ww) and ks[2] == 7 and pd[2] == 3 and c8 == 48 and k8 <= 64 and max(ks) <= 8:
         window = 'stem'
+    zb = _ZeroBox(*zero_box) if zero_box is not None and window == 'stem' else None
     if param_kc is not None and out is not None and _WGRAD_PENDING is not None:
         kn, cn = param_kc
         dw = out
         item = _lib.WgradReduceItem()
         with _timed(_wgrad_h3_kernel_name(k8, ks[2] * c8, window), flops):
-            _lib.check(lib.wdno_conv_wgrad_partials(_p(xh), _p(xl), _p(sx), _p(gh), _p(gl), _p(sg), _p(table), _p(dw), kn, cn, _p(ws), nb, C.byref(g),
-                                                    C.byref(item), _stream()), 'conv_wgrad_partials')
+            if zb is not None:
+                _lib.check(lib.wdno_conv_wgrad_partials_zbox(_p(xh), _p(xl), _p(sx), _p(gh), _p(gl), _p(sg), _p(table), _p(dw), kn, cn, _p(ws), nb, C.byref(g),
+                                                             C.byref(zb), C.byref(item), _stream()), 'conv_wgrad_partials_zbox')
+            else:
+                _lib.check(lib.wdno_conv_wgrad_partials(_p(xh), _p(xl), _p(sx), _p(gh), _p(gl), _p(sg), _p(table), _p(dw), kn, cn, _p(ws), nb, C.byref(g),
+                                                        C.byref(item), _stream()), 'conv_wgrad_partials')
         _WGRAD_PENDING.append((item, ws))
         if WGRAD_FLUSH_BYTES and sum(w.numel() for _, w in _WGRAD_PENDING) > WGRAD_FLUSH_BYTES:
             flush_wgrad_reduces()
@@ -890,14 +895,22 @@
         kn, cn = param_kc
         dw = out if out is not None else torch.empty((kn, cn, *ks), device=xh.device, dtype=torch.float32)
         with _timed(_wgrad_h3_kernel_name(k8, ks[2] * c8, window), flops):
-            _lib.check(lib.wdno_conv_wgrad_bf16_param(_p(xh), _p(gh), _p(table), _p(dw), kn, cn, _p(ws), nb, C.byref(g), _stream()), 'conv_wgrad_bf16_param')
+            if zb is not None:
+                _lib.check(lib.wdno_conv_wgrad_bf16_param_zbox(_p(xh), _p(gh), _p(table), _p(dw), kn, cn, _p(ws), nb, C.byref(g), C.byref(zb), _stream()),
+                           'conv_wgrad_bf16_param_zbox')
+            else:
+                _lib.check(lib.wdno_conv_wgrad_bf16_param(_p(xh), _p(gh), _p(table), _p(dw), kn, cn, _p(ws), nb, C.byref(g), _stream()), 'conv_wgrad_bf16_param')
         return dw
     if param_kc is not None:
         kn, cn = param_kc
         dw = out if out is not None else torch.empty((kn, cn, *ks), device=xh.device, dtype=torch.float32)
         with _timed(_wgrad_h3_kernel_name(k8, ks[2] * c8, window), flops):
-            _lib.check(lib.wdno_conv_wgrad_f16x3_param(_p(xh), _p(xl), _p(sx), _p(gh), _p(gl), _p(sg), _p(table), _p(dw), kn, cn, _p(ws), nb,
-                                                       C.byref(g), _stream()), 'conv_wgrad_f16x3_param')
+            if zb is not None:
+                _lib.check(lib.wdno_conv_wgrad_f16x3_param_zbox(_p(xh), _p(xl), _p(sx), _p(gh), _p(gl), _p(sg), _p(table), _p(dw), kn, cn, _p(ws), nb,
+                                                                C.byref(g), C.byref(zb), _stream()), 'conv_wgrad_f16x3_param_zbox')
+            else:
+                _lib.check(lib.wdno_conv_wgrad_f16x3_param(_p(xh), _p(xl), _p(sx), _p(gh), _p(gl), _p(sg), _p(table), _p(dw), kn, cn, _p(ws), nb,
+                                                           C.byref(g), _stream()), 'conv_wgrad_f16x3_param')
         return dw
     dwp = torch.empty((ks[0], ks[1], k8, ks[2], c8), device=xh.device, dtype=torch.float32)
     with _timed(_wgrad_h3_kernel_name(k8, ks[2] * c8, window), flops):
@@ -1097,8 +1110,9 @@
             out16 = (ACT16 and _lp() and getattr(ctx, 'to_norm', False) and GRAD_PLANES and residual is None and x.dim() in (4, 5) and kp % 8 == 0
                      and kp // 8 <= 256 and (kp // 8) & (kp // 8 - 1) == 0
                      and (not ctx.needs_input_grad[0] or (tuple(stride) == (1, 1, 1) and _use_h3(nx_ * dx_ * hx_ * wx_, kp * ks[0] * ks[1] * ks[2]))))
+            ctx.zero_box = zero_box_of(x_in) if x_in.dim() == 5 else None
             y = _leave_amax(conv_fwd_h3(planes, tuple(x5.shape[:4]), weight, pack_fwd, 'f', bias_p, res5, ks, stride, padding, kp,
-                                        amax_rec=yrec, zero_box=zero_box_of(x_in) if x_in.dim() == 5 else None, out16=out16), yrec)
+                                        amax_rec=yrec, zero_box=ctx.zero_box, out16=out16), yrec)
             ctx.save_for_backward(planes[0], planes[1], planes[2], weight)
         else:
             y = conv_fwd_raw(x5, pack_fwd(weight, cp, kp), bias_p, res5, ks, stride, padding, kp)
@@ -1197,7 +1211,7 @@
                 if gyplanes is None:
                     gyplanes = split_f16(gy5.reshape(-1, kp), grec)
                 gw = conv_wgrad_h3((xh, xl, sx), (n, d, h, w), gyplanes, osp, ks, stride, padding, param_kc=(k, c),
-                                   out=_flat_grad_out(weight, (k, c, *ks))).reshape(weight.shape)
+                                   out=_flat_grad_out(weight, (k, c, *ks)), zero_box=getattr(ctx, 'zero_box', None)).reshape(weight.shape)
             else:
                 dwp = conv_wgrad_raw(x5, gy5, ks, stride, padding)
                 gw = dwp[:, :, :k, :, :c].permute(2, 4, 0, 1, 3).reshape(weight.shape).contiguous()
```

New measurement: 33.16, median of 2. 0.99x the previous value.
